# DanHelmy/hdr-realtime-video-pipeline

Hardware: AMD Instinct MI355X
Metric: frames/sec (HDRTVNet++ AGCM+LE+HG fp16 3840x2160 + fused RGB48 post into the pinned host ring); p50 per-frame ms in p50_ms (higher is better)
Workload: dtype f16

## Files before the change

hdr-realtime-video-pipeline_amd/csrc/api.h:

```cpp
#pragma once
#include "../../include/hdrtv_mi355x.h"

#include <algorithm>
#include <array>
#include <cfloat>
#include <chrono>
#include <cmath>
#include <condition_variable>
#include <cstdarg>
#include <cstdio>
#include <cstdlib>
#include <cstring>
#include <map>
#include <mutex>
#include <string>
#include <vector>

#include "launchers.h"

namespace hdrtv_host {

struct PackEntry {
    int dtype;
    int ndim;
// ... 119 lines not shown
    bool asym = true;
    float inv() const { return 1.f / scale; }
    float zoff() const { return asym ? -zero / scale : 128.f; }
    double soff() const { return asym ? 128.0 * (double)scale + (double)zero : 0.0; }
};
struct QLayer {
    size_t wpk8 = 0, scale = 0, shift = 0;
    ActQf q;
    int cin = 0, cout = 0, coutPad = 0, ks = 0, stride = 1;
};
struct QLastLayer { size_t wq = 0, ss = 0; ActQf q; bool on = false; };
struct SftLayer {
    size_t wfrag = 0, bias = 0;
    bool q = false;
    size_t qfrag = 0, qconst = 0;
    float inv[2] = {0, 0}, zoff[2] = {0, 0}, hzoff[2] = {0, 0};
    ActQf fq[4];
};

struct Tensor {
    size_t off = 0;
    int C = 0, H = 0, W = 0, layout = 0;
    size_t bytes() const
    {
        const size_t n = (size_t)C * H * W;
        return layout == 2 || layout == 3 ? n * 4 : (layout == 4 || layout == 5 ? n : n * 2);
    }
};

struct F32Layer {
    size_t w = 0, b = 0, bn_s = 0, bn_t = 0;
    int cin = 0, cout = 0, cot = 32, ks = 1;
    bool bn = false;
};

struct RingSlot {
    uint16_t *host = nullptr, *dev = nullptr;
    hipEvent_t ev = nullptr;
    int state = 0;
    bool landed = false;
};

}

struct hdrtv_ctx {
    int device = 0;
    int n_cu = 256, dev_ncu = 256;
    bool has_hg = false;
    bool fp32 = false;
    std::map<std::string, hdrtv_host::F32Layer> conv32f;
    std::string err;
    mutable std::mutex err_mu;
    hdrtv_host::Arena wts;
    std::map<std::string, hdrtv_host::ConvLayer> conv;
    std::map<std::string, hdrtv_host::C3Layer> c3;
    std::map<std::string, hdrtv_host::ConvI8Layer> conv8;
    float mask_r = 0.75f;
    int cond_mode = 0;
    bool hg_i8 = false;
    float hg_q0_inv = 0.f, hg_q0_zero = 0.f;
    std::map<std::string, hdrtv_host::SftLayer> sft;
    bool hr_i8 = false;
    std::map<std::string, hdrtv_host::QLayer> q32, q8;
    hdrtv_host::QLastLayer q_trunk6, q_tail2;
    bool trunk_q8 = false, tail_q8 = false, agcm_q8 = false;
    size_t tq_frag = 0, tq_const = 0, tl_frag = 0, tl_const = 0, ag_frag = 0, ag_P = 0, ag_Q = 0;
    hdrtv_host::ActQf tq_q[6], tl_q[2], ag_q[3];
    FakeQ cls_q[6] = {}, lin_q[6] = {};
    std::map<std::string, size_t> f32v;
    size_t zeros_off = 0;
    size_t dump_off = 0;
    size_t trunk_wfrag = 0, trunk_bias = 0;
    size_t tail_wfrag = 0, tail_bias = 0;
    size_t hgf_wfrag = 0, hg_w10a = 0;
    int H = 0, W = 0;
    hdrtv_host::Arena ws;
    int lanes = 1;
    std::vector<unsigned char *> lane_ws;
    std::map<std::string, hdrtv_host::Tensor> t;
    int launches = 0;
    double macs = 0.0;
    bool prof_on = false;
    std::vector<hipEvent_t> prof_ev;
    struct ProfEntry { std::string layer, kernel; double macs, bytes; float ms; const int *cnt; int cnt_total; };
    bool taps_partial = false, taps_replayable = false;
    hipStream_t taps_stream = nullptr;
    std::vector<ProfEntry> prof;
    int lb_key[4] = {0, 0, 0, 0};
    LetterboxParams lb{};
    void *lb_dev = nullptr;
    size_t lb_cap = 0;
    float *pq_bnd = nullptr;
    std::map<std::array<int, 4>, int4 *> ps_tabs;
    double *mt_dev = nullptr;
    size_t mt_cap = 0;
    std::vector<hdrtv_host::RingSlot> ring;
    int ring_next = 0, ring_H = 0, ring_W = 0, ring_waiters = 0;
    std::mutex ring_mu;
    std::condition_variable ring_cv;
    std::map<std::string, int> var;
};

namespace hdrtv_host {

int fail(hdrtv_ctx *c, int code, const char *fmt, ...);
bool variant_allowed(const std::string &name, int value);
void variants_init(hdrtv_ctx *c);

#define HIPCHK(c, expr)                                                                         \
    do {                                                                                        \
        hipError_t e_ = (expr);                                                                 \
        if (e_ != hipSuccess) return hdrtv_host::fail(c, HDRTV_EHIP, "%s failed: %s", #expr, hipGetErrorString(e_)); \
    } while (0)

bool build_weights(hdrtv_ctx *c, const Pack &hr, const Pack *hg);
bool build_weights_f32(hdrtv_ctx *c, const Pack &hr, const Pack *hg);

struct Shapes {
    int H, W, h4, w4;
    int ch[6], cw[6];
    int H1, W1, H2, W2, H3, W3;
    int Hp, Wp;
};
Shapes shapes_for(int H, int W);
Tensor &ws_add(hdrtv_ctx *c, const std::string &name, int C, int H, int W, int layout);
int do_reserve(hdrtv_ctx *c, int H, int W);
void free_workspaces(hdrtv_ctx *c);
template <typename T>
T *wsp(hdrtv_ctx *c, unsigned char *base, const std::string &name)
{
    auto it = c->t.find(name);
    if (it == c->t.end()) { fprintf(stderr, "hdrtv: internal error, no workspace tensor %s\n", name.c_str()); abort(); }
    return reinterpret_cast<T *>(base + it->second.off);
}
template <typename T>
const T *wtp(hdrtv_ctx *c, size_t off) { return reinterpret_cast<const T *>(c->wts.dev + off); }

struct HgLayer {
    const char *name;
    int cout, cin, skip_cin;
    int ks, ps;
    int mode, act;
    int level;
    const char *in, *skip, *out;
    const char *bn;
    const char *consumer, *shares;
    int out_c() const { return ps ? ps : cout; }
    int out_level() const { return level + (mode == ST_POOL ? 1 : 0) - (ps ? 1 : 0); }
};
inline constexpr HgLayer hg_layers[] = {
    {"conv2", 128, 64, 0, 3, 0, ST_NHWC, ACT_RELU, 1, "p1", nullptr, "conv2", "conv2.1", "conv3_1.0", "conv9"},
    {"conv3_1", 256, 128, 0, 3, 0, ST_POOL, ACT_RELU, 1, "conv2", nullptr, "p3", "conv3_1.1", "conv3_2.0", nullptr},
    {"conv3_2", 256, 256, 0, 3, 0, ST_NHWC, ACT_RELU, 2, "p3", nullptr, "conv3_2", "conv3_2.1", "conv4_1.0", "conv8"},
    {"conv4_1", 512, 256, 0, 3, 0, ST_POOL, ACT_RELU, 2, "conv3_2", nullptr, "p4", "conv4_1.1", "conv4_2.0", nullptr},
    {"conv4_2", 512, 512, 0, 3, 0, ST_NHWC, ACT_RELU, 3, "p4", nullptr, "conv4_2", "conv4_2.1", "conv5_1.0", "conv7"},
    {"conv5_1", 512, 512, 0, 3, 0, ST_POOL, ACT_RELU, 3, "conv4_2", nullptr, "p5", "conv5_1.1", "conv5_2.0", nullptr},
    {"conv5_2", 512, 512, 0, 3, 0, ST_NHWC, ACT_RELU, 4, "p5", nullptr, "conv5_2", "conv5_2.1", "conv_code1.0", "conv6"},
    {"conv_code1", 512, 512, 0, 3, 0, ST_POOL, ACT_RELU, 4, "conv5_2", nullptr, "pc", "conv_code1.1", "conv_code2.0", nullptr},
    {"conv_code2", 512, 512, 0, 3, 0, ST_NHWC, ACT_RELU, 5, "pc", nullptr, "conv_code2", "conv_code2.1", "Up_conv1.0", nullptr},
    {"Up_conv1", 2048, 512, 0, 3, 512, ST_PS, ACT_RELU, 5, "conv_code2", nullptr, "up1", "", "conv6", nullptr},
    {"conv6", 512, 1024, 512, 1, 0, ST_NHWC, ACT_NONE, 4, "up1", "conv5_2", "conv6", "", "Up_conv2.0", nullptr},
    {"Up_conv2", 2048, 512, 0, 3, 512, ST_PS, ACT_RELU, 4, "conv6", nullptr, "up2", "", "conv7", nullptr},
    {"conv7", 256, 1024, 512, 1, 0, ST_NHWC, ACT_NONE, 3, "up2", "conv4_2", "conv7", "", "Up_conv3.0", nullptr},
    {"Up_conv3", 1024, 256, 0, 3, 256, ST_PS, ACT_RELU, 3, "conv7", nullptr, "up3", "", "conv8", nullptr},
    {"conv8", 128, 512, 256, 1, 0, ST_NHWC, ACT_NONE, 2, "up3", "conv3_2", "conv8", "", "Up_conv4.0", nullptr},
    {"Up_conv4", 512, 128, 0, 3, 128, ST_PS, ACT_RELU, 2, "conv8", nullptr, "up4", "", "conv9", nullptr},
    {"conv9", 64, 256, 128, 1, 0, ST_NHWC, ACT_NONE, 1, "up4", "conv2", "conv9", "", "Up_conv5.0", nullptr},
    {"Up_conv5", 256, 64, 0, 3, 64, ST_PS_DOT3, ACT_RELU, 1, "conv9", nullptr, nullptr, "", nullptr, nullptr},
};

struct Seq {
    hdrtv_ctx *c;
    hipStream_t s;
    unsigned char *ws;
    int rc = HDRTV_OK;
    const f16 *tail_w = nullptr;
    const float *tail_b = nullptr, *tail_s = nullptr;
    f16 *tail_out = nullptr;
    const int *need_list = nullptr;
    int need_th = 0, need_total = 0;
    bool ok() const { return rc == HDRTV_OK; }
    void mark()
    {
        if (!c->prof_on) return;
        const size_t i = c->prof.size();
        while (c->prof_ev.size() <= i) {
            hipEvent_t ev;
            if (hipEventCreate(&ev) != hipSuccess) { c->prof_on = false; return; }
            c->prof_ev.push_back(ev);
        }
        (void)hipEventRecord(c->prof_ev[i], s);
    }
    void chk(hipError_t e, const char *what, const char *kernel = "", double macs = 0.0, double bytes = 0.0, const int *cnt = nullptr, int cnt_total = 0)
    {
        ++c->launches;
        c->macs += macs;
        if (e != hipSuccess && rc == HDRTV_OK) rc = fail(c, HDRTV_EHIP, "launch %s failed: %s", what, hipGetErrorString(e));
        if (c->prof_on) {
            c->prof.push_back({what, kernel, macs, bytes, 0.f, cnt, cnt_total});
            mark();
        }
    }
    void conv(const std::string &key, const f16 *src0, int c0, const f16 *src1, int c1, int Hi, int Wi, int act, int mode, f16 *dst, int dstC, int Hd, int Wd, const f16 *res1 = nullptr, const f16 *res2 = nullptr, f16 *dst_full = nullptr, f16 *dst_planar = nullptr, const f16 *res_planar = nullptr, const float *dotw = nullptr, float *dst_dot = nullptr, int s0_stride = 0);
    void conv8(const std::string &key, const int8_t *src0, int c0, const int8_t *src1, int c1, int Hi, int Wi, int mode, void *dst, int dstC, int Hd, int Wd, const float *dotw = nullptr, float *dst_dot = nullptr);
    void convq8(const std::string &key, const void *src, bool src_i8, int src_stride, int Hi, int Wi, int act, void *dst, int dstC, const ActQf *oq);
    void c3(const std::string &key, const f16 *in, int H, int W, int act, f16 *out, f16 *out_pool, float pool_q_inv = 0.f, float pool_q_zero = 0.f, const f16 *w2frag = nullptr, float *part2 = nullptr);
    void conv32(const std::string &key, const f16 *src, const f16 *cond, const std::string &sft_key, int H, int W, int act, int mode, f16 *dst, int dstC, int Hd, int Wd, const f16 *res1 = nullptr, const f16 *res2 = nullptr, f16 *dst_planar = nullptr, const f16 *res_planar = nullptr, const f16 *c3_img = nullptr, const std::string &c3_key = "");
    template <typename T>
    T *wsp(const std::string &name) const { return hdrtv_host::wsp<T>(c, ws, name); }
    void *stamp_buf() const
    {
#ifdef HDRTV_STAMP
        static const int stamp_launch = [] { const char *e = getenv("HDRTV_STAMP_LAUNCH"); return e ? atoi(e) : -1; }();
        return (stamp_launch >= 0 && c->launches == stamp_launch) ? (void *)wsp<f16>("dbg.stamps") : nullptr;
#else
        return nullptr;
#endif
    }
    static int prw_rows(int prw_mode, int Ho, int Wo, int cout, int n_cu)
    {
        if (prw_mode != 1) return prw_mode == 0 ? 0 : (prw_mode == 3 ? 8 : 16);
        const long tx = (Wo + 15) / 16, n = n_cu;
        auto cost = [&](long tiles, double rel) { return (double)(((tiles + n - 1) / n) * n) / (double)tiles * rel; };
        const double c16 = cost(tx * ((Ho + 15) / 16) * (cout / 256), 1.0);
        const double c8 = cost(tx * ((Ho + 7) / 8) * (cout / 256), 1.09);
        const double cp = cost(tx * ((Ho + 15) / 16) * (cout / 128), 1.22);
        if (cp <= c16 && cp <= c8) return 0;
        return c8 < c16 ? 8 : 16;
    }
    static int prw_tile_rows(const hdrtv_ctx *c, int mode, int cout, int Ho, int Wo)
    {
        const int prw_mode = c->var.at("prw");
        if (prw_mode == 0) return 0;
        if (mode == ST_PS_DOT3) return cout == 256 ? 16 : 0;
        return (cout % 256) ? 0 : prw_rows(prw_mode, Ho, Wo, cout, c->n_cu);
    }
    static FqParam fqp(const ActQf &q) { return FqParam{q.inv(), q.zoff(), q.scale, q.asym ? q.zero : -128.f * q.scale}; }
    const ConvLayer *rows_conv(const std::string &key, FqParam &fq, bool &on) const
    {
        on = false;
        auto it = c->conv.find(key);
        if (it != c->conv.end()) return &it->second;
        if (!c->var.at("le_rows_fq")) return nullptr;
        it = c->conv.find(key + "#fq");
        if (it == c->conv.end()) return nullptr;
        auto iq = c->q32.find(key);
        const ActQf *q = iq != c->q32.end() ? &iq->second.q : nullptr;
        if (!q) { auto i8 = c->q8.find(key); if (i8 != c->q8.end()) q = &i8->second.q; }
        if (!q) return nullptr;
        fq = fqp(*q);
        on = true;
        return &it->second;
    }
    bool rows_sft(const SftLayer &S, FqParam (&fq)[4], bool &on) const
    {
        on = S.q;
        if (S.q && !c->var.at("le_rows_fq")) return false;
        for (int i = 0; i < 4; ++i) fq[i] = fqp(S.fq[i]);
        return true;
    }
    bool rows_on(int H, int W, bool even) const
    {
        if (!c->var.at("le_rows") || (even && ((H | W) & 1))) return false;
        const int nstrips = (W + 59) / 60, nseg = std::max(1, c->n_cu / nstrips);
        return W >= 60 && (H + nseg - 1) / nseg >= c->var.at("le_rows_min");
    }
    RowsConvI8 rows_i8(const QLayer &Q) const
    {
        return RowsConvI8{wtp<int8_t>(c, Q.wpk8), wtp<float>(c, Q.scale), wtp<float>(c, Q.shift), Q.q.inv(), Q.q.zoff()};
    }
    RowsSftI8 rows_i8(const SftLayer &S) const
    {
        return RowsSftI8{wtp<int8_t>(c, S.qfrag), wtp<float>(c, S.qconst), {S.inv[0], S.inv[1]}, {S.zoff[0], S.zoff[1]}, {S.hzoff[0], S.hzoff[1]}};
    }
    void resblock(const std::string &base, const f16 *x, const f16 *cond, int H, int W, f16 *tb, f16 *y, const f16 *extra = nullptr);
};

int run_agcm(hdrtv_ctx *c, Seq &q, const f16 *rgb, const f16 *cond, f16 *agcm_out);
int run_le(hdrtv_ctx *c, Seq &q, const f16 *img, f16 *out_planar);
int run_hg(hdrtv_ctx *c, Seq &q, const f16 *base, void *out, int out_f32, bool complete_taps = false);
size_t hg_need_plan(hdrtv_ctx *c, int Hp, int Wp, HgNeedParams &p);
int run_f32(hdrtv_ctx *c, Seq &q, bool plan, int H, int W, const float *rgb, const float *cond, float *out, float *agcm_out);
int f32_plan(hdrtv_ctx *c, int H, int W);

}
```

hdr-realtime-video-pipeline_amd/csrc/api_graph.hip:

```cpp
#include "api.h"

namespace hdrtv_host {

void Seq::conv(const std::string &key, const f16 *src0, int c0, const f16 *src1, int c1, int Hi, int Wi, int act, int mode, f16 *dst, int dstC, int Hd, int Wd, const f16 *res1, const f16 *res2, f16 *dst_full, f16 *dst_planar, const f16 *res_planar, const float *dotw, float *dst_dot, int s0_stride)
{
    if (!ok()) return;
    auto it = c->conv.find(key);
    if (it == c->conv.end()) { rc = fail(c, HDRTV_ESTATE, "no packed conv %s", key.c_str()); return; }
    const ConvLayer &L = it->second;
    ConvParams p;
    memset(&p, 0, sizeof p);
    p.src0 = src0; p.src1 = src1; p.c0 = c0; p.c1 = c1;
    p.s0_stride = s0_stride ? s0_stride : c0; p.s1_stride = c1;
    p.Hi = Hi; p.Wi = Wi;
    const int pad = L.ks / 2;
    p.Ho = (Hi + 2 * pad - L.ks) / L.stride + 1;
    p.Wo = (Wi + 2 * pad - L.ks) / L.stride + 1;
    p.wpk = wtp<f16>(c, L.wpk); p.scale = wtp<float>(c, L.scale); p.shift = wtp<float>(c, L.shift);
    p.CoutPad = L.coutPad; p.Cout = L.cout; p.act = act; p.mode = mode;
    p.dst = dst; p.dst_full = dst_full; p.dstC = dstC; p.Hd = Hd; p.Wd = Wd;
    p.res1 = res1; p.res2 = res2; p.dst_planar = dst_planar; p.res_planar = res_planar;
    p.dotw = dotw; p.dst_dot = dst_dot;
    if (c0 + c1 != L.cin) { rc = fail(c, HDRTV_ESTATE, "conv %s: channel mismatch", key.c_str()); return; }
    p.zeros = wtp<f16>(c, c->zeros_off);
    p.tail_w = tail_w; p.tail_b = tail_b; p.tail_s = tail_s; p.tail_out = tail_out;
    tail_w = nullptr; tail_b = nullptr; tail_s = nullptr; tail_out = nullptr;
    p.trash = const_cast<char *>(wtp<char>(c, c->dump_off));
    const int *const need = need_list;
    const int need_rows = need_th, need_cells = need_total;
    need_list = nullptr; need_th = 0; need_total = 0;
    const int nt_slow = c->var.at("pglds_nt_slow");
    p.nt_slow = nt_slow == 3 ? (mode == ST_PS) : (nt_slow == 2 ? (L.coutPad >= 512) : nt_slow);
    enum { T16, S2G, PRW, PGLDS, GLDS1, IGEMM } route = IGEMM;
    int prw_th = 0;
    const bool g64 = L.stride == 1 && L.cin_t == 64 && L.bn == 128 && !res1 && !res2 && !dst_full && mode != ST_PLANAR3;
    const bool no_t16 = c->var.at("no_t16") != 0;
    if (!no_t16 && L.ks == 3 && L.stride == 2 && L.cin == 32 && L.coutPad == 32 && !src1 && mode == ST_NHWC && !res1 && !res2)
        route = T16;
    else if (L.ks == 3 && L.stride == 2 && L.cin_t == 64 && L.bn == L.coutPad && (L.coutPad == 64 || L.coutPad == 192))
        route = S2G;
    else if (g64 && L.ks == 3 && L.cout == L.coutPad) {
        prw_th = prw_tile_rows(c, mode, L.coutPad, p.Ho, p.Wo);
        route = prw_th ? PRW : PGLDS;
    } else if (g64 && L.ks == 1 && mode == ST_NHWC && (c0 + c1) >= 128 && L.coutPad <= 512 && (act == ACT_RELU || act == ACT_NONE))
        route = GLDS1;
    if (p.tail_w && route != S2G) { rc = fail(c, HDRTV_ESTATE, "conv %s: a fused CondNet tail was requested but the layer does not run on conv3x3s2_preg", key.c_str()); return; }
    const char *epi = mode == ST_POOL ? "pool" : (mode == ST_PS ? "ps" : (mode == ST_PS_DOT3 ? "ps_dot3" : "nhwc"));
    char tag[64];
    hipError_t e;
    bool list_taken = false;
    switch (route) {
    case T16: snprintf(tag, sizeof tag, "conv_t16<32,3,2>"); e = conv_t16_launch(p, s, c->n_cu); break;
    case S2G:
        snprintf(tag, sizeof tag, p.tail_w ? "conv3x3s2_preg<%d>+tail" : "conv3x3s2_preg<%d>", L.coutPad);
        e = conv3x3s2_preg_launch(p, c->n_cu, s);
        break;
    case PRW:
        if (need && need_rows == prw_th) p.tile_list = need;
        snprintf(tag, sizeof tag, "%s<%s>", prw_th == 8 ? "conv_prw8" : "conv_prw", epi);
        e = conv_prw_launch(p, prw_th, c->n_cu, s, &list_taken);
        break;
    case PGLDS: snprintf(tag, sizeof tag, "conv_pglds<%s>", epi); e = conv_pglds_launch(p, c->n_cu, s); break;
    case GLDS1: snprintf(tag, sizeof tag, "conv_glds1"); e = conv_glds1_launch(p, s, c->n_cu, c->var.at("glds1_old") != 0); break;
    default:
        snprintf(tag, sizeof tag, "conv_igemm<%d,%d,%d,%d>", L.cin_t, L.bn, L.ks, L.stride);
        e = conv_igemm_launch(p, L.cin_t, L.bn, L.ks, L.stride, s);
    }
    double macs = (double)p.Ho * p.Wo * L.cin * L.ks * L.ks * L.cout;
    double bytes = 2.0 * Hi * Wi * L.cin + 2.0 * L.ks * L.ks * L.cin * L.coutPad;
    if (p.tail_w) {
        macs += (double)p.Ho * p.Wo * (p.tail_s ? 64 * 16 : 64 * 64 + 64 * 16);
        bytes -= 2.0 * p.Ho * p.Wo * (64 - 16);
    }
    const double outel = mode == ST_POOL ? (double)Hd * Wd * L.cout + (dst_full ? (double)p.Ho * p.Wo * L.cout : 0.0)
                                          : (mode == ST_PLANAR3 ? 3.0 * Hd * Wd
                                                                : (mode == ST_PS_DOT3 ? 8.0 * Hd * Wd : (double)p.Ho * p.Wo * L.cout));
    bytes += 2.0 * outel * (1 + (res1 ? 1 : 0) + (res2 ? 1 : 0) + (res_planar ? 1 : 0));
    chk(e, key.c_str(), tag, macs, bytes, list_taken ? p.tile_list : nullptr, need_cells);
}


void Seq::conv8(const std::string &key, const int8_t *src0, int c0, const int8_t *src1, int c1, int Hi, int Wi, int mode, void *dst, int dstC, int Hd, int Wd, const float *dotw, float *dst_dot)
{
    if (!ok()) return;
    auto it = c->conv8.find(key);
    if (it == c->conv8.end()) { rc = fail(c, HDRTV_ESTATE, "no packed int8 conv %s", key.c_str()); return; }
    const ConvI8Layer &L = it->second;
    if (c0 + c1 != L.cin) { rc = fail(c, HDRTV_ESTATE, "conv %s: channel mismatch", key.c_str()); return; }
    ConvI8Params p;
    memset(&p, 0, sizeof p);
    p.src0 = src0; p.src1 = src1; p.c0 = c0; p.c1 = c1; p.Hi = Hi; p.Wi = Wi; p.Ho = Hi; p.Wo = Wi;
    p.wpk = wtp<int8_t>(c, L.wpk); p.scale = wtp<float>(c, L.scale); p.shift = wtp<float>(c, L.shift);
    p.Cout = L.cout; p.mode = mode; p.out_f16 = L.out_f16; p.dst = dst; p.dstC = dstC; p.Hd = Hd; p.Wd = Wd;
    p.padline = wtp<int8_t>(c, L.padline);
    p.delta = L.has_delta ? wtp<float>(c, L.delta) : nullptr;
    p.delta_acc = L.has_delta ? wtp<int>(c, L.delta_acc) : nullptr;
    p.lo_clamp = L.lo_clamp;
    p.trash = const_cast<char *>(wtp<char>(c, c->dump_off));
    p.dotw = dotw; p.dst_dot = dst_dot;
    char tag[64];
    if (L.ks == 3) snprintf(tag, sizeof tag, "conv_pglds_i8<%s%s>", mode == ST_POOL ? "pool" : (mode == ST_PS ? "ps" : (mode == ST_PS_DOT3 ? "ps_dot3" : "nhwc")), c0 == 64 ? ",c64" : "");
    else snprintf(tag, sizeof tag, "conv1x1_i8%s", L.out_f16 ? "<f16>" : "");
    const double macs = (double)Hi * Wi * L.cin * L.ks * L.ks * L.cout_real;
    const double outel = mode == ST_POOL ? (double)Hd * Wd * L.cout_real : (double)Hi * Wi * L.cout_real;
    const double bytes = (double)Hi * Wi * L.cin + (double)L.ks * L.ks * L.cin * L.cout +
                         (mode == ST_PS_DOT3 ? 16.0 * Hd * Wd : outel * (L.out_f16 ? 2.0 : 1.0));
    const int prw_mode = c->var.at("prw");
    int prw_th = prw_mode != 0 && L.ks == 3 && c0 != 64 && (L.cout % 256) == 0 && mode != ST_PS_DOT3 && !L.out_f16
                     ? prw_rows(prw_mode, Hi, Wi, L.cout, c->n_cu) : 0;
    const int i8_mode = c->var.at("prw_i8");
    if (i8_mode == 0 || (i8_mode == 1 && prw_th != 8)) prw_th = 0;
    const bool prw = prw_th != 0;
    if (prw) snprintf(tag, sizeof tag, "conv_prw%s_i8<%s>", prw_th == 8 ? "8" : "", mode == ST_POOL ? "pool" : (mode == ST_PS ? "ps" : "nhwc"));
    chk(L.ks == 3 ? (prw ? conv_prw_i8_launch(p, prw_th, c->n_cu, s) : conv_pglds_i8_launch(p, c->n_cu, s)) : conv1x1_i8_launch(p, s),
        key.c_str(), tag, macs, bytes);
}


void Seq::convq8(const std::string &key, const void *src, bool src_i8, int src_stride, int Hi, int Wi, int act, void *dst, int dstC, const ActQf *oq)
{
    if (!ok()) return;
    auto it = c->q8.find(key);
    if (it == c->q8.end()) { rc = fail(c, HDRTV_ESTATE, "no packed W8A8 conv %s", key.c_str()); return; }
    const QLayer &L = it->second;
    ConvQ8Params p;
    memset(&p, 0, sizeof p);
    p.src = src; p.src_i8 = src_i8 ? 1 : 0; p.Cin = L.cin; p.src_stride = src_stride; p.Hi = Hi; p.Wi = Wi;
    p.ks = L.ks; p.stride = L.stride;
    const int pad = L.ks / 2;
    p.Ho = (Hi + 2 * pad - L.ks) / L.stride + 1; p.Wo = (Wi + 2 * pad - L.ks) / L.stride + 1;
    p.wpk8 = wtp<int8_t>(c, L.wpk8); p.scale = wtp<float>(c, L.scale); p.shift = wtp<float>(c, L.shift);
    p.CoutPad = L.coutPad; p.Cout = L.cout; p.act = act; p.q_inv = L.q.inv(); p.q_zoff = L.q.zoff();
    p.dst = dst; p.dst_i8 = oq ? 1 : 0; p.dstC = dstC;
    if (oq) { p.oq_inv = oq->inv(); p.oq_zoff = oq->zoff(); }
    char tag[64];
    snprintf(tag, sizeof tag, "conv_q8<%d,%d,%d>", L.cin, L.ks, L.stride);
    const double macs = (double)p.Ho * p.Wo * L.cin * L.ks * L.ks * L.cout;
    const double bytes = (double)Hi * Wi * L.cin * (src_i8 ? 1.0 : 2.0) + (double)L.ks * L.ks * L.cin * L.coutPad +
                         (double)p.Ho * p.Wo * L.cout * (oq ? 1.0 : 2.0);
    chk(conv_q8_launch(p, s, c->n_cu), key.c_str(), tag, macs, bytes);
}


void Seq::c3(const std::string &key, const f16 *in, int H, int W, int act, f16 *out, f16 *out_pool, float pool_q_inv, float pool_q_zero, const f16 *w2frag, float *part2)
{
    if (!ok()) return;
    const C3Layer &L = c->c3.at(key);
    chk(conv_c3_launch(in, H, W, wtp<f16>(c, L.wfrag), wtp<float>(c, L.scale), wtp<float>(c, L.shift), L.cout, act, out,
                       out_pool, c->n_cu, s, pool_q_inv, pool_q_zero, w2frag, part2), key.c_str(),
        part2 ? "conv_c3<64,dot3>" : (L.cout == 64 ? "conv_c3<64>" : "conv_c3<32>"), (double)H * W * (27 * L.cout + (part2 ? 192 : 0)),
        (double)H * W * (6.0 + (out ? 2.0 * L.cout : 0.0) + (out_pool ? (pool_q_inv > 0.f ? 0.25 : 0.5) * L.cout : 0.0) + (part2 ? 16.0 : 0.0)));
}


void Seq::conv32(const std::string &key, const f16 *src, const f16 *cond, const std::string &sft_key, int H, int W, int act, int mode, f16 *dst, int dstC, int Hd, int Wd, const f16 *res1, const f16 *res2, f16 *dst_planar, const f16 *res_planar, const f16 *c3_img, const std::string &c3_key)
{
    if (!ok()) return;
    auto it = c->conv.find(key);
    auto iq = c->q32.find(key);
    if (it == c->conv.end() && iq == c->q32.end()) { rc = fail(c, HDRTV_ESTATE, "no packed conv %s", key.c_str()); return; }
    const bool i8 = iq != c->q32.end();
    ConvLayer L;
    Conv32Params p;
    memset(&p, 0, sizeof p);
    if (i8) {
        const QLayer &Q = iq->second;
        L.cout = Q.cout; L.coutPad = Q.coutPad;
        p.wpk8 = wtp<int8_t>(c, Q.wpk8); p.scale = wtp<float>(c, Q.scale); p.shift = wtp<float>(c, Q.shift);
        p.q_inv = Q.q.inv(); p.q_zoff = Q.q.zoff();
    } else {
        L = it->second;
        p.wpk = wtp<f16>(c, L.wpk); p.scale = wtp<float>(c, L.scale); p.shift = wtp<float>(c, L.shift);
    }
    p.src = src; p.cond = cond; p.H = H; p.W = W;
    bool sq = false;
    if (cond) {
        const SftLayer &S = c->sft.at(sft_key);
        p.sft_wfrag = wtp<f16>(c, S.wfrag); p.sft_bias = wtp<float>(c, S.bias);
        if (S.q) {
            sq = true;
            p.sq_wfrag = wtp<int8_t>(c, S.qfrag); p.sq_const = wtp<float>(c, S.qconst);
            for (int b = 0; b < 2; ++b) { p.sq_inv[b] = S.inv[b]; p.sq_zoff[b] = S.zoff[b]; p.sq_hzoff[b] = S.hzoff[b]; }
        }
    }
    p.CoutPad = L.coutPad; p.Cout = L.cout; p.act = act; p.mode = mode;
    p.dst = dst; p.dstC = dstC; p.Hd = Hd; p.Wd = Wd; p.res1 = res1; p.res2 = res2;
    p.dst_planar = dst_planar; p.res_planar = res_planar; p.zeros = wtp<f16>(c, c->zeros_off);
    p.dump = reinterpret_cast<f16 *>(stamp_buf());
    const double npx = (double)H * W;
    const double macs = npx * 32 * 9 * L.cout + (cond ? npx * 2 * (16 * 16 + 16 * 32) : 0.0) + (c3_img ? npx * 27 * 32 : 0.0);
    const double outb = mode == ST_PLANAR3 ? 6.0 * npx : 2.0 * npx * L.cout;
    const double bytes = npx * ((c3_img ? 6 : 64) + (cond ? 32 : 0)) + outb * (1 + (res1 ? 1 : 0) + (res2 ? 1 : 0) + (res_planar ? 1 : 0)) +
                         (i8 ? 1.0 : 2.0) * 9 * 32 * L.coutPad;
    p.trash = const_cast<char *>(wtp<char>(c, c->dump_off));
    if (c3_img) {
        const C3Layer &L3 = c->c3.at(c3_key);
        p.c3_img = c3_img; p.c3_wfrag = wtp<f16>(c, L3.wfrag);
    }
    const bool old_sched = c->var.at("conv32_old") != 0;
    const bool one_barrier = L.coutPad == 32 && !old_sched;
    char tag[48];
    snprintf(tag, sizeof tag, "conv32%c<%d,%s%s%s>", one_barrier ? 's' : 'p', L.coutPad / 32, c3_img ? "c3+" : "", cond ? (sq ? "sft-i8" : "sft") : "plain", i8 ? ",i8" : "");
    if (c3_img && !one_barrier) { rc = fail(c, HDRTV_ESTATE, "conv_first fusion needs the one-barrier schedule"); return; }
    chk(one_barrier ? conv32s_launch(p, c->n_cu, s, c->var.at("conv32_nosplit") != 0) : conv32p_launch(p, c->n_cu, s, c->var.at("conv32_nw")), key.c_str(), tag, macs, bytes);
}


void Seq::resblock(const std::string &base, const f16 *x, const f16 *cond, int H, int W, f16 *tb, f16 *y, const f16 *extra)
{
    const bool rows = ok() && !extra && rows_on(H, W, false);
    if (rows && c->var.at("le_rows_i8")) {
        auto q1 = c->q32.find(base + ".conv1"), q2 = c->q32.find(base + ".conv2");
        const SftLayer &S1 = c->sft.at(base + ".sft1"), &S2 = c->sft.at(base + ".sft2");
        if (q1 != c->q32.end() && q2 != c->q32.end() && S1.q && S2.q && q1->second.coutPad == 32 && q2->second.coutPad == 32) {
            RowsRbI8Params p;
            memset(&p, 0, sizeof p);
            p.x = x; p.cond = cond; p.c1 = rows_i8(q1->second); p.c2 = rows_i8(q2->second); p.s1 = rows_i8(S1); p.s2 = rows_i8(S2);
            p.slope1 = act_slope(ACT_RELU);
            p.dst = y; p.trash = const_cast<char *>(wtp<char>(c, c->dump_off)); p.H = H; p.W = W;
            const double npx = (double)H * W;
            chk(le_rb_rows_i8_launch(p, c->n_cu, s), base.c_str(), "le_rb_rows<i8>",
                npx * (2.0 * 32 * 9 * 32 + 4.0 * (16 * 16 + 16 * 32)), npx * (64 + 32 + 64) + 2.0 * 9 * 32 * 32);
            return;
        }
    }
    if (rows) {
        RowsRbParams p;
        memset(&p, 0, sizeof p);
        bool q1, q2, qs1, qs2;
        const ConvLayer *L1 = rows_conv(base + ".conv1", p.fq_c1, q1), *L2 = rows_conv(base + ".conv2", p.fq_c2, q2);
        const SftLayer &S1 = c->sft.at(base + ".sft1"), &S2 = c->sft.at(base + ".sft2");
        if (L1 && L2 && rows_sft(S1, p.fq_s1, qs1) && rows_sft(S2, p.fq_s2, qs2)) {
            p.fq = (q1 ? 1 : 0) | (q2 ? 2 : 0) | (qs1 ? 4 : 0) | (qs2 ? 8 : 0);
            p.x = x; p.cond = cond; p.H = H; p.W = W; p.dst = y;
// ... 256 lines not shown
            q.conv32("LE.HR_conv1", f0a, cond1, "LE.SFT_layer1", H, W, ACT_RELU, ST_NHWC, fea0, 32, H, W);
        } else {
            const bool fuse = !c->var.at("no_c3fuse") && !c->var.at("conv32_old") && c->q32.find("LE.HR_conv1") == c->q32.end();
            if (fuse) {
                q.conv32("LE.HR_conv1", f0a, cond1, "LE.SFT_layer1", H, W, ACT_RELU, ST_NHWC, fea0, 32, H, W, nullptr, nullptr, nullptr, nullptr,
                         img, "le.conv_first");
            } else {
                q.c3("le.conv_first", img, H, W, ACT_RELU, f0a, nullptr);
                q.conv32("LE.HR_conv1", f0a, cond1, "LE.SFT_layer1", H, W, ACT_RELU, ST_NHWC, fea0, 32, H, W);
            }
        }
    }
    f16 *fea1a = q.wsp<f16>("le.fea1a"), *fea1 = q.wsp<f16>("le.fea1"), *l1b = q.wsp<f16>("le.l1b");
    auto down = [&](const char *key, const f16 *src, int Hi, int Wi, f16 *dst, int Ho, int Wo) {
        if (isq8(key)) q.convq8(key, src, false, 32, Hi, Wi, ACT_RELU, dst, 32, nullptr);
        else q.conv(key, src, 32, nullptr, 0, Hi, Wi, ACT_RELU, ST_NHWC, dst, 32, Ho, Wo);
    };
    if (!head_fused) down("LE.down_conv1", fea0, H, W, fea1a, s.H1, s.W1);
    q.resblock("LE.recon_trunk1.0", fea1a, cond2, s.H1, s.W1, l1b, fea1);
    f16 *fea2a = q.wsp<f16>("le.fea2a"), *fea2 = q.wsp<f16>("le.fea2"), *l2b = q.wsp<f16>("le.l2b");
    down("LE.down_conv2", fea1, s.H1, s.W1, fea2a, s.H2, s.W2);
    q.resblock("LE.recon_trunk2.0", fea2a, cond3, s.H2, s.W2, l2b, fea2);
    f16 *fea3 = q.wsp<f16>("le.fea3"), *l3b = q.wsp<f16>("le.l3b"), *t3x = q.wsp<f16>("le.t3x"), *t3y = q.wsp<f16>("le.t3y");
    down("LE.down_conv3", fea2, s.H2, s.W2, fea3, s.H3, s.W3);
    q.resblock("LE.recon_trunk3.0", fea3, cond4, s.H3, s.W3, l3b, t3x);
    q.resblock("LE.recon_trunk3.1", t3x, cond4, s.H3, s.W3, l3b, t3y);
    q.resblock("LE.recon_trunk3.2", t3y, cond4, s.H3, s.W3, l3b, t3x);
    q.resblock("LE.recon_trunk3.3", t3x, cond4, s.H3, s.W3, l3b, t3y, fea3);
    f16 *up1 = q.wsp<f16>("le.up1"), *t4 = q.wsp<f16>("le.t4");
    q.conv32("LE.up_conv1.0", t3y, nullptr, "", s.H3, s.W3, ACT_RELU, ST_PS, up1, 32, s.H2, s.W2, fea2);
    q.resblock("LE.recon_trunk4.0", up1, cond3, s.H2, s.W2, l2b, t4);
    f16 *up2 = q.wsp<f16>("le.up2"), *t5 = q.wsp<f16>("le.t5");
    q.conv32("LE.up_conv2.0", t4, nullptr, "", s.H2, s.W2, ACT_RELU, ST_PS, up2, 32, s.H1, s.W1, fea1);
    q.resblock("LE.recon_trunk5.0", up2, cond2, s.H1, s.W1, l1b, t5);
    if (q.ok() && rows && c->var.at("le_rows_i8")) {
        auto qu = c->q32.find("LE.up_conv3.0"), qh = c->q32.find("LE.HR_conv2"), ql = c->q32.find("LE.conv_last");
        const SftLayer &S2 = c->sft.at("LE.SFT_layer2");
        if (qu != c->q32.end() && qh != c->q32.end() && ql != c->q32.end() && S2.q && qu->second.coutPad == 128 &&
            qh->second.coutPad == 32 && ql->second.coutPad == 32) {
            RowsTailI8Params p;
            memset(&p, 0, sizeof p);
            p.u = t5; p.fea0 = fea0; p.cond = cond1; p.res_planar = img; p.dst_planar = out_planar; p.H = H; p.W = W;
            p.up = q.rows_i8(qu->second); p.hr = q.rows_i8(qh->second); p.last = q.rows_i8(ql->second); p.s = q.rows_i8(S2);
            p.slope_relu = act_slope(ACT_RELU);
            p.trash = const_cast<char *>(wtp<char>(c, c->dump_off));
            const double npx = (double)H * W;
            q.chk(le_tail_rows_i8_launch(p, c->n_cu, q.s), "LE.tail", "le_tail_rows<i8>",
                  npx * (32.0 * 9 * 128 / 4 + 2.0 * (16 * 16 + 16 * 32) + 32.0 * 9 * 32 + 32.0 * 9 * 3), npx * (16 + 64 + 32 + 6 + 6) + 9.0 * 32 * (128 + 32 + 32));
            return q.rc;
        }
    }
    if (q.ok() && rows) {
        RowsTailParams p;
        memset(&p, 0, sizeof p);
        bool qu, qh, ql, qs;
        const ConvLayer *Lu = q.rows_conv("LE.up_conv3.0", p.fq_u, qu), *Lh = q.rows_conv("LE.HR_conv2", p.fq_y, qh),
                        *Ll = q.rows_conv("LE.conv_last", p.fq_z, ql);
        const SftLayer &S2 = c->sft.at("LE.SFT_layer2");
        if (Lu && Lh && Ll && q.rows_sft(S2, p.fq_s, qs)) {
            p.fq = (qu ? 1 : 0) | (qh ? 2 : 0) | (ql ? 4 : 0) | (qs ? 8 : 0);
            p.u = t5; p.fea0 = fea0; p.cond = cond1; p.res_planar = img; p.dst_planar = out_planar; p.H = H; p.W = W;
            p.w_up = wtp<f16>(c, Lu->wpk); p.b_up = wtp<float>(c, Lu->shift);
            p.sft_wfrag = wtp<f16>(c, S2.wfrag); p.sft_bias = wtp<float>(c, S2.bias);
            p.w_hr = wtp<f16>(c, Lh->wpk); p.b_hr = wtp<float>(c, Lh->shift); p.w_last = wtp<f16>(c, Ll->wpk); p.b_last = wtp<float>(c, Ll->shift);
            p.trash = const_cast<char *>(wtp<char>(c, c->dump_off));
            p.dump = q.stamp_buf();
            const double npx = (double)H * W;
            q.chk(le_tail_rows_launch(p, c->n_cu, q.s), "LE.tail", p.fq ? "le_tail_rows<fq>" : "le_tail_rows",
                  npx * (32.0 * 9 * 128 / 4 + 2.0 * (16 * 16 + 16 * 32) + 32.0 * 9 * 32 + 32.0 * 9 * 3), npx * (16 + 64 + 32 + 6 + 6) + 2.0 * 9 * 32 * (128 + 32 + 32));
            return q.rc;
        }
    }
    q.conv32("LE.up_conv3.0", t5, nullptr, "", s.H1, s.W1, ACT_RELU, ST_PS, up3, 32, H, W, fea0);
    q.conv32("LE.HR_conv2", up3, cond1, "LE.SFT_layer2", H, W, ACT_RELU, ST_NHWC, f0b, 32, H, W);
    q.conv32("LE.conv_last", f0b, nullptr, "", H, W, ACT_NONE, ST_PLANAR3, nullptr, 0, H, W, nullptr, nullptr, out_planar, img);
    return q.rc;
}

size_t hg_need_plan(hdrtv_ctx *c, int Hp, int Wp, HgNeedParams &p)
{
    memset(&p, 0, sizeof p);
    p.Hp = Hp; p.Wp = Wp;
    constexpr int n_layers = (int)(sizeof hg_layers / sizeof hg_layers[0]);
    static_assert(n_layers <= HG_NEED_MAX_LAYERS && n_layers + 2 <= HG_NEED_MAX_TENSORS, "hg_need's tables are too small");
    constexpr int max_level = [] { int m = 0; for (const HgLayer &L : hg_layers) m = L.level > m ? L.level : m; return m; }();
    static_assert(max_level < HG_NEED_LEVELS, "hg_need's unit tables have too few levels");
    memcpy(p.lu, hg_need_unit_log2[c->var.at("hg_sparse") == 1 ? 1 : 2], sizeof p.lu);
    auto ncell = [&](int level) { return (((Hp >> level) + 15) / 16) * (((Wp >> level) + 15) / 16); };
    auto nwords = [&](int level) {
        size_t m = 0;
        for (const auto &tab : hg_need_unit_log2) {
            const int u = 1 << tab[level], rows = std::max(((Hp >> level) + u - 1) / u, ((Hp >> level) + 7) / 8);
            m = std::max(m, (size_t)rows * ((((Wp >> level) + u - 1) / u + 63) / 64));
        }
        return m;
    };
    const char *names[HG_NEED_MAX_TENSORS];
    int level[HG_NEED_MAX_TENSORS], nt = 0;
    auto tensor = [&](const char *name, int lev) {
        if (!name) name = "part";
        for (int i = 0; i < nt; ++i)
            if (!strcmp(names[i], name)) return i;
        names[nt] = name; level[nt] = lev;
        return nt++;
    };
    for (int i = 0; i < n_layers; ++i) {
        const HgLayer &L = hg_layers[i];
        HgNeedLayer &N = p.L[i];
        N.level = L.level; N.ks = L.ks;
        N.mode = L.mode == ST_POOL ? 1 : (L.ps ? 2 : 0);
        N.in = tensor(L.in, L.level);
        N.skip = L.skip ? tensor(L.skip, L.level) : -1;
        N.out = tensor(L.out, L.out_level());
        N.th = L.ks == 3 && Seq::prw_tile_rows(c, L.mode, L.cout, Hp >> L.level, Wp >> L.level) == 8 ? 8 : 16;
    }
    p.n_layers = n_layers;
    bool seen[HG_NEED_MAX_TENSORS] = {};
    for (int i = n_layers - 1; i >= 0; --i) {
        HgNeedLayer &N = p.L[i];
        N.in_first = !seen[N.in];
        seen[N.in] = true;
        if (N.skip >= 0) { N.skip_first = !seen[N.skip]; seen[N.skip] = true; }
    }
    size_t off = 0;
    auto take = [&](size_t bytes) { const size_t o = off; off = (off + bytes + 15) & ~(size_t)15; return (int)o; };
    p.flags_off = take((size_t)ncell(0));
    take((size_t)ncell(0));
    for (int t = 0; t < nt; ++t)
        if (strcmp(names[t], "part")) take((size_t)ncell(level[t]));
    for (int i = 0; i < n_layers; ++i) p.L[i].list_off = take(4 * (2 * (size_t)ncell(p.L[i].level) + 4));
    size_t scratch = 0;
    for (int t = 0; t < nt; ++t) {
        p.map_off[t] = take(8 * nwords(level[t]));
        scratch = std::max(scratch, nwords(level[t]));
        if (!strcmp(names[t], "part")) p.flags_map = t;
    }
    for (int i = 0; i < n_layers; ++i) {
        p.L[i].out_chained = i + 1 < n_layers ? p.L[i + 1].in == p.L[i].out : p.L[i].out == p.flags_map;
        p.L[i].in_chained = i > 0 && p.L[i - 1].out == p.L[i].in;
    }
    p.scratch_words = (int)scratch;
    p.kbits_off = take(8 * scratch);
    p.tbits_off = take(8 * scratch);
    return off;
}

int run_hg(hdrtv_ctx *c, Seq &q, const f16 *base, void *out, int out_f32, bool complete_taps)
{
    const Shapes s = shapes_for(c->H, c->W);
    const int Hp = s.Hp, Wp = s.Wp;
    f16 *img = q.wsp<f16>("hg.img");
    uint8_t *mask = q.wsp<uint8_t>("hg.mask");
    const bool sparse = !complete_taps && c->var.at("hg_sparse") != 0 && !c->hg_i8 && !c->var.at("final_recompute");
    HgNeedParams np;
    if (sparse) {
        hg_need_plan(c, Hp, Wp, np);
        np.base = q.wsp<unsigned char>("hg.need");
    }
    if (q.ws == c->lane_ws[0] && !complete_taps) {
        hipStreamCaptureStatus cap = hipStreamCaptureStatusNone;
        c->taps_partial = sparse;
        c->taps_replayable = sparse && hipStreamIsCapturing(q.s, &cap) == hipSuccess && cap != hipStreamCaptureStatusNone;
        c->taps_stream = q.s;
    }
    if (!complete_taps)
        q.chk(hg_prep_launch(base, s.H, s.W, Hp, Wp, img, mask, c->mask_r, 0.1f, q.s, sparse ? np.base + np.flags_off : nullptr), "hg_prep",
              "hg_prep", 0.0, 13.0 * Hp * Wp);
    if (sparse) q.chk(hg_need_launch(np, q.s), "hg_need", "hg_need", 0.0, 0.0);
    float *part = q.wsp<float>("hg.part");
    const bool light = !c->var.at("final_recompute");
    float *part2 = light ? q.wsp<float>("hg.part2") : nullptr;
    const f16 *w2frag = light ? wtp<f16>(c, c->hgf_wfrag) + 6 * 64 * 8 : nullptr;
    constexpr int n_layers = (int)(sizeof hg_layers / sizeof hg_layers[0]);
    const char *tn[3 * n_layers];
    void *tp[3 * n_layers];
    int nt = 0;
    auto tensor = [&](const char *name) -> void * {
        if (!name) return nullptr;
        for (int i = 0; i < nt; ++i)
            if (!strcmp(tn[i], name)) return tp[i];
        char key[32];
        snprintf(key, sizeof key, "%s%s", c->hg_i8 ? "hg8." : "hg.", name);
        tn[nt] = name;
        tp[nt] = q.wsp<void>(key);
        return tp[nt++];
    };
    q.c3("hg.conv1", img, Hp, Wp, ACT_RELU, nullptr, (f16 *)tensor(hg_layers[0].in), c->hg_q0_inv, c->hg_q0_zero, w2frag, part2);
    char key[32];
    for (const HgLayer &L : hg_layers) {
        snprintf(key, sizeof key, "hg.%s", L.name);
        if (sparse) {
            const HgNeedLayer &N = np.L[&L - hg_layers];
            q.need_list = reinterpret_cast<const int *>(np.base + N.list_off);
            q.need_th = N.th;
            q.need_total = (((Hp >> L.level) + N.th - 1) / N.th) * (((Wp >> L.level) + 15) / 16);
        }
        const int c1 = L.skip_cin, c0 = L.cin - c1, Hi = Hp >> L.level, Wi = Wp >> L.level;
        const int Ho = Hp >> L.out_level(), Wo = Wp >> L.out_level();
        const bool dot3 = L.mode == ST_PS_DOT3;
        const float *dotw = dot3 ? wtp<float>(c, c->hg_w10a) : nullptr;
        float *dst_dot = dot3 ? part : nullptr;
        if (c->hg_i8)
            q.conv8(key, (const int8_t *)tensor(L.in), c0, (const int8_t *)tensor(L.skip), c1, Hi, Wi, L.mode, tensor(L.out), L.out_c(), Ho, Wo, dotw, dst_dot);
        else
            q.conv(key, (const f16 *)tensor(L.in), c0, (const f16 *)tensor(L.skip), c1, Hi, Wi, L.act, L.mode, (f16 *)tensor(L.out), L.out_c(), Ho, Wo,
                   nullptr, nullptr, nullptr, nullptr, nullptr, dotw, dst_dot);
    }
    if (!q.ok() || complete_taps) return q.rc;
    const C3Layer &L1 = c->c3.at("hg.conv1");
    HgFinalFusedArgs fa;
    fa.img = img; fa.mask = mask; fa.part = part; fa.wfrag = wtp<f16>(c, c->hgf_wfrag);
    fa.scale = wtp<float>(c, L1.scale); fa.shift = wtp<float>(c, L1.shift);
    fa.b10 = wtp<float>(c, c->f32v.at("hg.b10"));
    fa.wl = wtp<float>(c, c->f32v.at("hg.wl")); fa.bl = wtp<float>(c, c->f32v.at("hg.bl"));
    fa.out = out; fa.out_f32 = out_f32; fa.H = s.H; fa.W = s.W; fa.Hp = Hp; fa.Wp = Wp;
    if (light)
        q.chk(hg_final_light_launch(fa, part2, q.s), "hg_final", "hg_final_light", (double)s.H * s.W * 6 * 3,
              (double)s.H * s.W * (6 + 1 + 32 + 3 * (out_f32 ? 4 : 2)));
#ifdef HDRTV_AB
    else
        q.chk(hg_final_fused_launch(fa, c->n_cu, q.s), "hg_final", "hg_final_fused", (double)Hp * Wp * (128 * 3 + 6 * 3),
              (double)s.H * s.W * (6 + 1 + 16 + 3 * (out_f32 ? 4 : 2)));
#endif
    return q.rc;
}

}
```

hdr-realtime-video-pipeline_amd/csrc/conv1x1_glds.hip:

```cpp
#include <cstdlib>

#include "launchers.h"

namespace {

constexpr int TH = 16, TW = 16, NPIX = TH * TW;
constexpr int CT = 64, PIXB = CT * 2;
constexpr int A_PIECES_PER_WAVE = 4, A_BYTES = 8 * A_PIECES_PER_WAVE * 1024;
constexpr int BN = 128;
constexpr int B_BYTES = BN * PIXB;
constexpr int B_PIECES_PER_WAVE = 2;
constexpr int SMEM = 3 * A_BYTES + 3 * B_BYTES;
constexpr int OUT_ROWB = BN * 2 + 16;
static_assert(NPIX * OUT_ROWB <= SMEM, "epilogue tile must fit");

__device__ __forceinline__ int swz64(int row) { return (row >> 1) & 7; }


#ifdef HDRTV_AB
__global__ __launch_bounds__(512) void conv_glds1_kernel(ConvParams p)
{
    extern __shared__ __attribute__((aligned(16))) char smem[];
    char *sA = smem;
    char *sB = smem + 3 * A_BYTES;
// ... 58 lines not shown
    for (int i = 0; i < 2; ++i)
#pragma unroll
        for (int j = 0; j < 2; ++j)
#pragma unroll
            for (int k = 0; k < 16; ++k) acc[i][j][k] = 0.f;

    issue_A(0, 0);
    issue_B(0, 0);
    if (nchunk > 1) {
        issue_A(1, 1);
        issue_B(1, 1);
        asm volatile("s_waitcnt vmcnt(6)" ::: "memory");
    } else {
        asm volatile("s_waitcnt vmcnt(0)" ::: "memory");
    }
    __builtin_amdgcn_s_barrier();
    int slot = 0;
#pragma unroll 1
    for (int cc = 0; cc < nchunk; ++cc) {
        const bool pf = cc + 2 < nchunk;
        const int s2 = slot == 0 ? 2 : slot - 1;
        if (pf) { issue_A(cc + 2, s2); issue_B(cc + 2, s2); }
        const char *a = sA + slot * A_BYTES;
        const char *b = sB + slot * B_BYTES;
#pragma unroll
        for (int ks = 0; ks < CT / 16; ++ks) {
            const int chunk = ks * 2 + lh;
            f16x8 wf[2], xf[2];
#pragma unroll
            for (int i = 0; i < 2; ++i)
                wf[i] = *reinterpret_cast<const f16x8 *>(b + wrow[i] * PIXB + ((chunk ^ swz64(wrow[i])) << 4));
#pragma unroll
            for (int j = 0; j < 2; ++j)
                xf[j] = *reinterpret_cast<const f16x8 *>(a + hp_base[j] * PIXB + ((chunk ^ swz64(hx_base[j])) << 4));
#pragma unroll
            for (int i = 0; i < 2; ++i)
#pragma unroll
                for (int j = 0; j < 2; ++j)
                    acc[i][j] = __builtin_amdgcn_mfma_f32_32x32x16_f16(wf[i], xf[j], acc[i][j], 0, 0, 0);
        }
        if (pf) asm volatile("s_waitcnt vmcnt(6)" ::: "memory");
        else asm volatile("s_waitcnt vmcnt(0)" ::: "memory");
        __builtin_amdgcn_s_barrier();
        slot = slot == 2 ? 0 : slot + 1;
    }

    const float aslope = act_slope(p.act);
    char *so = smem;
#pragma unroll
    for (int i = 0; i < 2; ++i) {
#pragma unroll
        for (int qd = 0; qd < 4; ++qd) {
            const int cl = (wc * 2 + i) * 32 + 8 * qd + 4 * lh;
            const float4 sc = *reinterpret_cast<const float4 *>(p.scale + n0 + cl);
            const float4 sh = *reinterpret_cast<const float4 *>(p.shift + n0 + cl);
#pragma unroll
            for (int j = 0; j < 2; ++j) {
                const int q = (wp * 2 + j) * 32 + l31;
                f16x4 o;
                o[0] = (f16)act_fast(acc[i][j][4 * qd + 0] * sc.x + sh.x, aslope);
                o[1] = (f16)act_fast(acc[i][j][4 * qd + 1] * sc.y + sh.y, aslope);
                o[2] = (f16)act_fast(acc[i][j][4 * qd + 2] * sc.z + sh.z, aslope);
                o[3] = (f16)act_fast(acc[i][j][4 * qd + 3] * sc.w + sh.w, aslope);
                *reinterpret_cast<f16x4 *>(so + q * OUT_ROWB + cl * 2) = o;
            }
        }
    }
    __syncthreads();
    constexpr int CPP = BN / 8;
    for (int e = tid; e < NPIX * CPP; e += 512) {
        const int q = e / CPP, c8 = e % CPP;
        const int oy = oy0 + q / TW, ox = ox0 + q % TW;
        const int ch = n0 + c8 * 8;
        if (oy < p.Ho && ox < p.Wo && ch < p.Cout)
            *reinterpret_cast<f16x8 *>(p.dst + ((size_t)oy * p.Wo + ox) * p.dstC + ch) =
                *reinterpret_cast<const f16x8 *>(so + q * OUT_ROWB + c8 * 16);
    }
}
#endif

constexpr int P_NST = 8;
constexpr int P_SP = 144;
constexpr int P_MAXC = 512;

__global__ __launch_bounds__(512) void conv_glds1p_kernel(ConvParams p)
{
    extern __shared__ __attribute__((aligned(16))) char smem[];
    char *sA = smem;
    char *sB = smem + 3 * A_BYTES;
    const int tid = threadIdx.x, lane = tid & 63;
    const int wave = __builtin_amdgcn_readfirstlane(tid >> 6);
    const int l31 = lane & 31, lh = lane >> 5;

    const int ntn = p.CoutPad / BN;
    const int total = p.tiles_x * p.tiles_y * ntn;
    int t_first, t_step, ntile;
    {
        const int G = gridDim.x, b = blockIdx.x, xcd = b & 7, slot = b >> 3;
        const int nslots = (G - xcd + 7) >> 3;
        const int q = total >> 3, r = total & 7;
        const int base = xcd < r ? xcd * (q + 1) : r * (q + 1) + (xcd - r) * q;
        const int len = q + (xcd < r ? 1 : 0);
        t_first = base + slot;
        t_step = nslots;
        ntile = slot < len ? (len - slot + nslots - 1) / nslots : 0;
    }
    if (ntile == 0) return;
    struct Tile { int n0, oy0, ox0; };
    auto decode = [&](int t) {
        Tile o;
        const int nt_i = t % ntn, sp = t / ntn;
        const int ty = sp / p.tiles_x, tx = sp - ty * p.tiles_x;
        o.n0 = nt_i * BN; o.oy0 = ty * TH; o.ox0 = tx * TW;
        return o;
    };
    const int nchunk = (p.c0 + p.c1) / CT, nchunk0 = p.c0 / CT;

    const int l_row = lane >> 3, l_slot = lane & 7;
    auto issue = [&](const Tile &T, int cc, int slot) {
        const f16 *src;
        int cs, coff;
        if (cc < nchunk0) { src = p.src0; cs = p.s0_stride; coff = cc * CT; }
        else { src = p.src1; cs = p.s1_stride; coff = (cc - nchunk0) * CT; }
        const dma_rsrc_t ra = dma_rsrc(src, (unsigned)p.Hi * (unsigned)p.Wi * (unsigned)cs * 2u);
#pragma unroll
        for (int it = 0; it < A_PIECES_PER_WAVE; ++it) {
            const int piece = wave + it * 8;
            const int hp = piece * 8 + l_row;
            const int hy = hp / TW, hx = hp - hy * TW;
            const int iy = T.oy0 + hy, ix = T.ox0 + hx;
            const bool ok = (iy < p.Hi) & (ix < p.Wi);
            const unsigned off = ((unsigned)(iy * p.Wi + ix) * (unsigned)cs + (unsigned)(coff + ((l_slot ^ swz64(hx)) << 3))) * 2u;
            dma16(ra, sA + slot * A_BYTES + piece * 1024, ok ? off : DMA_OOB);
        }
        const dma_rsrc_t rb = dma_rsrc(p.wpk, (unsigned)nchunk * (unsigned)p.CoutPad * (unsigned)(CT * 2));
        const unsigned so = (unsigned)(cc * p.CoutPad + T.n0) * (unsigned)(CT * 2);
#pragma unroll
        for (int k = 0; k < B_PIECES_PER_WAVE; ++k) {
            const int piece = wave * B_PIECES_PER_WAVE + k;
            const int n = piece * 8 + l_row;
            dma16(rb, sB + slot * B_BYTES + piece * 1024, (unsigned)(n * CT + ((l_slot ^ swz64(n)) << 3)) * 2u, so);
        }
    };

    const int wc = wave & 1, wp = wave >> 1;
    int hp_base[2], hx_base[2], wrow[2];
#pragma unroll
    for (int j = 0; j < 2; ++j) {
        const int q = (wp * 2 + j) * 32 + l31;
        hp_base[j] = q;
        hx_base[j] = q % TW;
        wrow[j] = (wc * 2 + j) * 32 + l31;
    }
    f32x16 acc[2][2];
#pragma unroll
    for (int i = 0; i < 2; ++i)
#pragma unroll
        for (int j = 0; j < 2; ++j)
#pragma unroll
            for (int k = 0; k < 16; ++k) acc[i][j][k] = 0.f;
    const float act_lb = p.act == ACT_RELU ? 0.f : -__builtin_inff();
    char *trash = reinterpret_cast<char *>(p.trash) + lane * 16;
    __shared__ __attribute__((aligned(16))) float s_ss[2 * P_MAXC];
    for (int e = tid; e < p.CoutPad; e += 512) { s_ss[e] = p.scale[e]; s_ss[P_MAXC + e] = p.shift[e]; }
    __syncthreads();

    Tile cur = decode(t_first), nxt = cur;
    issue(cur, 0, 0);
    issue(cur, 1, 1);
    asm volatile("s_waitcnt vmcnt(6)" ::: "memory");
    __builtin_amdgcn_s_barrier();
    int slot = 0;
    for (int k = 0; k < ntile; ++k) {
        const bool has_next = k + 1 < ntile;
        if (has_next) nxt = decode(t_first + (k + 1) * t_step);
#pragma unroll 1
        for (int cc = 0; cc < nchunk; ++cc) {
            const int s2 = slot == 0 ? 2 : slot - 1;
            bool pf = true;
            if (cc + 2 < nchunk) issue(cur, cc + 2, s2);
            else if (has_next) issue(nxt, cc + 2 - nchunk, s2);
            else pf = false;
            const char *a = sA + slot * A_BYTES;
            const char *b = sB + slot * B_BYTES;
#pragma unroll
            for (int ks = 0; ks < CT / 16; ++ks) {
                const int chunk = ks * 2 + lh;
                f16x8 wf[2], xf[2];
#pragma unroll
                for (int i = 0; i < 2; ++i)
                    wf[i] = *reinterpret_cast<const f16x8 *>(b + wrow[i] * PIXB + ((chunk ^ swz64(wrow[i])) << 4));
#pragma unroll
                for (int j = 0; j < 2; ++j)
                    xf[j] = *reinterpret_cast<const f16x8 *>(a + hp_base[j] * PIXB + ((chunk ^ swz64(hx_base[j])) << 4));
#pragma unroll
                for (int i = 0; i < 2; ++i)
#pragma unroll
                    for (int j = 0; j < 2; ++j)
                        acc[i][j] = __builtin_amdgcn_mfma_f32_32x32x16_f16(wf[i], xf[j], acc[i][j], 0, 0, 0);
            }
            if (!pf) asm volatile("s_waitcnt vmcnt(0)" ::: "memory");
            else if (cc == 0 && k > 0) asm volatile("s_waitcnt vmcnt(%0)" ::"n"(6 + P_NST) : "memory");
            else asm volatile("s_waitcnt vmcnt(6)" ::: "memory");
            __builtin_amdgcn_s_barrier();
            if (cc + 1 < nchunk) slot = slot == 2 ? 0 : slot + 1;
        }
        char *stg = wave < 6 ? sA + slot * A_BYTES + wave * (32 * P_SP) : sB + slot * B_BYTES + (wave - 6) * (32 * P_SP);
        const int s_row = lane >> 3, s_chunk = lane & 7;
        const int chb = cur.n0 + wc * 64 + s_chunk * 8;
#pragma unroll
        for (int j = 0; j < 2; ++j) {
#pragma unroll
            for (int i = 0; i < 2; ++i)
#pragma unroll
                for (int qd = 0; qd < 4; ++qd) {
                    const int cl = (wc * 2 + i) * 32 + 8 * qd + 4 * lh;
                    const float4 sc = *reinterpret_cast<const float4 *>(s_ss + cur.n0 + cl);
                    const float4 sh = *reinterpret_cast<const float4 *>(s_ss + P_MAXC + cur.n0 + cl);
                    f16x4 o;
                    o[0] = (f16)fmaxf(acc[i][j][4 * qd + 0] * sc.x + sh.x, act_lb);
                    o[1] = (f16)fmaxf(acc[i][j][4 * qd + 1] * sc.y + sh.y, act_lb);
                    o[2] = (f16)fmaxf(acc[i][j][4 * qd + 2] * sc.z + sh.z, act_lb);
                    o[3] = (f16)fmaxf(acc[i][j][4 * qd + 3] * sc.w + sh.w, act_lb);
                    *reinterpret_cast<f16x4 *>(stg + l31 * P_SP + (i * 32 + 8 * qd + 4 * lh) * 2) = o;
#pragma unroll
                    for (int r = 0; r < 4; ++r) acc[i][j][4 * qd + r] = 0.f;
                }
#pragma unroll
            for (int rr = 0; rr < 4; ++rr) {
                const int px = rr * 8 + s_row;
                const f16x8 v = *reinterpret_cast<const f16x8 *>(stg + px * P_SP + s_chunk * 16);
                const int oy = cur.oy0 + (wp * 2 + j) * 2 + (px >> 4), ox = cur.ox0 + (px & 15);
                const bool ok = oy < p.Ho && ox < p.Wo && chb < p.Cout;
                f16 *d = ok ? p.dst + ((size_t)oy * p.Wo + ox) * p.dstC + chb : reinterpret_cast<f16 *>(trash);
                *reinterpret_cast<f16x8 *>(d) = v;
            }
        }
        asm volatile("s_waitcnt lgkmcnt(0)" ::: "memory");
        __builtin_amdgcn_s_barrier();
        slot = slot == 2 ? 0 : slot + 1;
        cur = nxt;
    }
}

}

hipError_t conv_glds1_launch(ConvParams p, hipStream_t stream, int n_cu, bool old_form)
{
    if ((p.c0 % CT) || (p.c1 % CT) || p.c0 + p.c1 < CT || (p.CoutPad % BN) || p.res1 || p.res2 || p.dst_full ||
        p.mode != ST_NHWC || !p.zeros)
        return hipErrorInvalidValue;
#ifdef HDRTV_AB
    static DevOnce attr_once;
    if (attr_once.need()) {
        hipError_t e = hipFuncSetAttribute(reinterpret_cast<const void *>(conv_glds1_kernel),
                                           hipFuncAttributeMaxDynamicSharedMemorySize, SMEM);
        if (e != hipSuccess) return e;
        attr_once.done();
    }
#endif
    p.tiles_x = (p.Wo + TW - 1) / TW;
    p.tiles_y = (p.Ho + TH - 1) / TH;
    const int grid = p.tiles_x * p.tiles_y * (p.CoutPad / BN);
    const int nchunk = (p.c0 + p.c1) / CT;
    if (!old_form && n_cu >= 8 && nchunk >= 2 && p.trash && p.CoutPad <= P_MAXC && (p.act == ACT_RELU || p.act == ACT_NONE)) {
        static DevOnce attr_p;
        if (attr_p.need()) {
            hipError_t e = hipFuncSetAttribute(reinterpret_cast<const void *>(conv_glds1p_kernel),
                                               hipFuncAttributeMaxDynamicSharedMemorySize, SMEM);
            if (e != hipSuccess) return e;
            attr_p.done();
        }
        hipLaunchKernelGGL(conv_glds1p_kernel, dim3(grid < n_cu ? grid : n_cu), dim3(512), SMEM, stream, p);
        return hipGetLastError();
    }
#ifdef HDRTV_AB
    hipLaunchKernelGGL(conv_glds1_kernel, dim3(grid), dim3(512), SMEM, stream, p);
    return hipGetLastError();
#else
    return hipErrorNotSupported;
#endif
}
```

hdr-realtime-video-pipeline_amd/csrc/conv3x3_pglds.hip:

```cpp
#include "launchers.h"

namespace {

constexpr int TH = 16, TW = 16, HW = 18, NPIX = HW * HW;
constexpr int CT = 64, PIXB = CT * 2;
constexpr int BN = 128;
constexpr int A_PIECES_PER_WAVE = 6, A_BYTES = 8 * A_PIECES_PER_WAVE * 1024;
constexpr int B_BYTES = BN * PIXB, B_PIECES_PER_WAVE = 2;
constexpr int SS_OFF = 2 * A_BYTES + 3 * B_BYTES;
constexpr int DOTW_OFF = SS_OFF + 2048;
constexpr int SMEM = DOTW_OFF + 1024;

template <int MODE> struct NStores { static constexpr int N = MODE == ST_POOL ? 2 : (MODE == ST_PS_DOT3 ? 1 : 8); };

typedef __amdgpu_buffer_rsrc_t rsrc_t;
__device__ __forceinline__ rsrc_t make_rsrc(const void *base, unsigned bytes)
{
    return __builtin_amdgcn_make_buffer_rsrc(const_cast<void *>(base), (short)0, (int)bytes, 0x00020000);
}
__device__ __forceinline__ void bdma16(rsrc_t r, void *lds, unsigned voff, unsigned soff)
{
    __builtin_amdgcn_raw_ptr_buffer_load_lds(r, (__attribute__((address_space(3))) void *)lds, 16, voff, soff, 0, 0);
}
constexpr unsigned OOB = 0x80000000u;

template <int N> __device__ __forceinline__ void wait_vm()
{
    asm volatile("s_waitcnt vmcnt(%0)" ::"n"(N) : "memory");
}
template <int N> __device__ __forceinline__ void wait_tap()
{
    asm volatile("s_waitcnt vmcnt(%0) lgkmcnt(0)" ::"n"(N) : "memory");
}

struct Tile { int n0, oy0, ox0; };

template <int MODE>
__global__ __launch_bounds__(512) void conv_pglds_kernel(ConvParams p)
{
    extern __shared__ __attribute__((aligned(16))) char smem[];
    char *sA = smem;
    char *sB = smem + 2 * A_BYTES;

    const int tid = threadIdx.x, lane = tid & 63;
    const int wave = __builtin_amdgcn_readfirstlane(tid >> 6);
    const int l15 = lane & 15, kg = lane >> 4;

    const int ntn = p.CoutPad / BN;
    const int total = p.tiles_x * p.tiles_y * ntn;
    int t_first, t_step, ntile;
    {
        const int G = gridDim.x, b = blockIdx.x, xcd = b & 7, slot = b >> 3;
        const int nslots = (G - xcd + 7) >> 3;
        const int q = total >> 3, r = total & 7;
        const int base = xcd < r ? xcd * (q + 1) : r * (q + 1) + (xcd - r) * q;
        const int len = q + (xcd < r ? 1 : 0);
        t_first = base + slot;
        t_step = nslots;
        ntile = slot < len ? (len - slot + nslots - 1) / nslots : 0;
    }
    if (ntile == 0) return;
    auto decode = [&](int t) {
        Tile o;
        const int nsp = p.tiles_x * p.tiles_y;
        const int nt_i = p.nt_slow ? t / nsp : t % ntn, sp = p.nt_slow ? t - nt_i * nsp : t / ntn;
        const int ty = sp / p.tiles_x, tx = sp - ty * p.tiles_x;
        o.n0 = nt_i * BN; o.oy0 = ty * TH; o.ox0 = tx * TW;
        return o;
    };

    const int nchunk = (p.c0 + p.c1) / CT, nchunk0 = p.c0 / CT;
    const int nit = nchunk * 9;

    const int l_row = lane >> 3, l_slot = lane & 7;
    auto issue_A = [&](int cc, int buf, const Tile &T) {
        const f16 *src;
        int cs, coff;
        if (cc < nchunk0) { src = p.src0; cs = p.s0_stride; coff = cc * CT; }
        else { src = p.src1; cs = p.s1_stride; coff = (cc - nchunk0) * CT; }
        const rsrc_t rs = make_rsrc(src, (unsigned)p.Hi * (unsigned)p.Wi * (unsigned)cs * 2u);
#pragma unroll
        for (int it = 0; it < A_PIECES_PER_WAVE; ++it) {
            const int piece = wave + it * 8;
            const int hp = piece * 8 + l_row;
            const int hy = hp / HW, hx = hp - hy * HW;
            const int iy = T.oy0 - 1 + hy, ix = T.ox0 - 1 + hx;
            const bool ok = (hp < NPIX) & ((unsigned)iy < (unsigned)p.Hi) & ((unsigned)ix < (unsigned)p.Wi);
            const unsigned off = ((unsigned)(iy * p.Wi + ix) * (unsigned)cs + (unsigned)(coff + ((l_slot ^ (hx & 7)) << 3))) * 2u;
            bdma16(rs, sA + buf * A_BYTES + piece * 1024, ok ? off : OOB, 0);
        }
    };
    auto issue_B = [&](int it_i, int n0, int slot) {
        const int cc = it_i / 9, tap = it_i - cc * 9;
        const rsrc_t rs = make_rsrc(p.wpk, 9u * (unsigned)nchunk * (unsigned)p.CoutPad * (unsigned)PIXB);
        const unsigned so = (unsigned)((tap * nchunk + cc) * p.CoutPad + n0) * (unsigned)PIXB;
#pragma unroll
        for (int k = 0; k < B_PIECES_PER_WAVE; ++k) {
            const int piece = wave * B_PIECES_PER_WAVE + k;
            const int n = piece * 8 + l_row;
            bdma16(rs, sB + slot * B_BYTES + piece * 1024, (unsigned)(n * CT + ((l_slot ^ (n & 7)) << 3)) * 2u, so);
        }
    };
    auto issue_SS = [&](int n0, int slot) {
        const char *sc = reinterpret_cast<const char *>(p.scale), *sh = reinterpret_cast<const char *>(p.shift);
        const char *lo = sc < sh ? sc : sh;
        const rsrc_t rs = make_rsrc(lo, 0xffffffffu);
        bdma16(rs, smem + SS_OFF + slot * 1024, (unsigned)((lane < 32 ? sc : sh) - lo) + (unsigned)(lane & 31) * 16u, (unsigned)n0 * 4u);
    };

    if constexpr (MODE == ST_PS_DOT3) {
        if (tid < 24) {
            const int kgq = tid & 3, o = (tid >> 2) % 3, half = tid / 12;
            f16x8 hi, lo;
#pragma unroll
            for (int e = 0; e < 8; ++e) {
                const float w = p.dotw[o * 64 + half * 32 + (e < 4 ? 4 * kgq + e : 16 + 4 * kgq + e - 4)];
                hi[e] = (f16)w;
                lo[e] = (f16)((w - (float)hi[e]) * 1024.f);
            }
            *reinterpret_cast<f16x8 *>(smem + DOTW_OFF + tid * 32) = hi;
            *reinterpret_cast<f16x8 *>(smem + DOTW_OFF + tid * 32 + 16) = lo;
        }
        __syncthreads();
    }

    const int wc = wave & 1, wp = wave >> 1;
    f32x4 acc[4][4];
#pragma unroll
    for (int i = 0; i < 4; ++i)
#pragma unroll
        for (int j = 0; j < 4; ++j) acc[i][j] = f32x4{0.f, 0.f, 0.f, 0.f};
    const float act_lb = p.act == ACT_RELU ? 0.f : -__builtin_inff();
    const int kw = l15 & 7;
    const int b_lane = (wc * 64 + l15) * PIXB;
    const int a_lane = (wp * 4 * HW + l15) * PIXB;

    Tile cur = decode(t_first), nxt = cur;
    issue_A(0, 0, cur);
    issue_SS(cur.n0, 0);
    issue_B(0, cur.n0, 0);
    issue_B(1, cur.n0, 1);
    issue_B(2, cur.n0, 2);
    wait_vm<4>();
    __builtin_amdgcn_s_barrier();

    int gch = 0;
    for (int k = 0; k < ntile; ++k) {
        const bool has_next = k + 1 < ntile;
        if (has_next) nxt = decode(t_first + (k + 1) * t_step);
        for (int cc = 0; cc < nchunk; ++cc, ++gch) {
            const char *a = sA + (gch & 1) * A_BYTES;
            const bool last_chunk = cc + 1 == nchunk;
            const bool pfA = !last_chunk || has_next;
#pragma unroll
            for (int tap = 0; tap < 9; ++tap) {
                const int it_i = cc * 9 + tap;
                bool pfB = true;
                if (tap == 0 && cc == 0) {}
                else if (it_i + 2 < nit) issue_B(it_i + 2, cur.n0, (tap + 2) % 3);
                else if (has_next) issue_B(it_i + 2 - nit, nxt.n0, (tap + 2) % 3);
                else pfB = false;
                if (tap == 6 && pfA) {
                    if (!last_chunk) issue_A(cc + 1, (gch + 1) & 1, cur);
                    else { issue_A(0, (gch + 1) & 1, nxt); issue_SS(nxt.n0, (k + 1) & 1); }
                }

                const char *bw = sB + (tap % 3) * B_BYTES + b_lane;
                const char *ax = a + a_lane + ((tap / 3) * HW + tap % 3) * PIXB;
                const int kx = (l15 + tap % 3) & 7;
                f16x8 wf[2][4], xf[2][4];
                auto ldw = [&](int ks, int i) {
                    wf[ks][i] = *reinterpret_cast<const f16x8 *>(bw + i * 16 * PIXB + (((ks * 4 + kg) ^ kw) << 4));
                };
                auto ldx = [&](int ks, int j) {
                    xf[ks][j] = *reinterpret_cast<const f16x8 *>(ax + j * HW * PIXB + (((ks * 4 + kg) ^ kx) << 4));
                };
#pragma unroll
                for (int i = 0; i < 4; ++i) { ldw(0, i); ldx(0, i); }
                __builtin_amdgcn_sched_barrier(0);
#pragma unroll
                for (int g = 0; g < 8; ++g) {
                    acc[g >> 2][g & 3] = __builtin_amdgcn_mfma_f32_16x16x32_f16(wf[0][g >> 2], xf[0][g & 3], acc[g >> 2][g & 3], 0, 0, 0);
                    __builtin_amdgcn_sched_barrier(0);
                    if (g == 0) ldw(1, 0); else if (g < 5) ldx(1, g - 1); else ldw(1, g - 4);
                    __builtin_amdgcn_sched_barrier(0);
                }
#pragma unroll
                for (int m = 8; m < 16; ++m)
                    acc[m >> 2][m & 3] = __builtin_amdgcn_mfma_f32_16x16x32_f16(wf[0][m >> 2], xf[0][m & 3], acc[m >> 2][m & 3], 0, 0, 0);
                __builtin_amdgcn_sched_barrier(0);
#pragma unroll
                for (int m = 0; m < 16; ++m)
                    acc[m >> 2][m & 3] = __builtin_amdgcn_mfma_f32_16x16x32_f16(wf[1][m >> 2], xf[1][m & 3], acc[m >> 2][m & 3], 0, 0, 0);

                if (!pfB) {
                    wait_tap<0>();
                } else if ((tap == 6 || tap == 7) && pfA) {
                    if (last_chunk) wait_tap<9>();
                    else wait_tap<8>();
                } else if (tap <= 1 && cc == 0 && k > 0) {
                    wait_tap<NStores<MODE>::N + 2>();
                } else {
                    wait_tap<2>();
                }
                __builtin_amdgcn_s_barrier();
            }
        }

        if (has_next) issue_B(2, nxt.n0, 2);
        const float *ss = reinterpret_cast<const float *>(smem + SS_OFF + (k & 1) * 1024);
        char *trash = reinterpret_cast<char *>(p.trash) + lane * 16;
        const int cw = wc * 64 + 4 * kg;
        f16x4 o[4][4];
#pragma unroll
        for (int i = 0; i < 4; ++i) {
            const float4 sc = *reinterpret_cast<const float4 *>(ss + cw + i * 16);
            const float4 sh = *reinterpret_cast<const float4 *>(ss + 128 + cw + i * 16);
#pragma unroll
            for (int j = 0; j < 4; ++j) {
                o[i][j][0] = (f16)fmaxf(acc[i][j][0] * sc.x + sh.x, act_lb);
                o[i][j][1] = (f16)fmaxf(acc[i][j][1] * sc.y + sh.y, act_lb);
                o[i][j][2] = (f16)fmaxf(acc[i][j][2] * sc.z + sh.z, act_lb);
                o[i][j][3] = (f16)fmaxf(acc[i][j][3] * sc.w + sh.w, act_lb);
                acc[i][j] = f32x4{0.f, 0.f, 0.f, 0.f};
            }
        }
        const int ox = cur.ox0 + l15;
        constexpr int SP = 144;
        char *stg = sA + ((gch - 1) & 1) * A_BYTES + wave * (32 * SP);
        const int s_row = lane >> 3, s_chunk = lane & 7;
        if constexpr (MODE == ST_NHWC || MODE == ST_PS) {
            const int cps = p.dstC;
// ... 15 lines not shown
                    f16 *d;
                    if constexpr (MODE == ST_NHWC) {
                        const bool ok = oy < p.Ho && oxx < p.Wo;
                        d = ok ? p.dst + ((size_t)oy * p.Wo + oxx) * p.dstC + cbase : reinterpret_cast<f16 *>(trash);
                    } else {
                        const int Y = 2 * oy + (sub >> 1), X = 2 * oxx + (sub & 1);
                        const bool ok = oy < p.Ho && oxx < p.Wo && Y < p.Hd && X < p.Wd;
                        d = ok ? p.dst + ((size_t)Y * p.Wd + X) * cps + cbase : reinterpret_cast<f16 *>(trash);
                    }
                    *reinterpret_cast<f16x8 *>(d) = v;
                }
            }
        } else if constexpr (MODE == ST_POOL) {
#pragma unroll
            for (int jj = 0; jj < 2; ++jj)
#pragma unroll
                for (int i = 0; i < 4; ++i) {
                    f16x4 m;
#pragma unroll
                    for (int r = 0; r < 4; ++r) m[r] = o[i][2 * jj][r] > o[i][2 * jj + 1][r] ? o[i][2 * jj][r] : o[i][2 * jj + 1][r];
                    *reinterpret_cast<f16x4 *>(stg + (jj * 16 + l15) * SP + (i * 16 + 4 * kg) * 2) = m;
                }
#pragma unroll
            for (int jj = 0; jj < 2; ++jj) {
                f16x8 v = *reinterpret_cast<const f16x8 *>(stg + (jj * 16 + 2 * s_row) * SP + s_chunk * 16);
                const f16x8 v1 = *reinterpret_cast<const f16x8 *>(stg + (jj * 16 + 2 * s_row + 1) * SP + s_chunk * 16);
#pragma unroll
                for (int r = 0; r < 8; ++r) v[r] = v[r] > v1[r] ? v[r] : v1[r];
                const int py = (cur.oy0 >> 1) + wp * 2 + jj, px = (cur.ox0 >> 1) + s_row;
                const bool ok = py < p.Hd && px < p.Wd;
                f16 *d = ok ? p.dst + ((size_t)py * p.Wd + px) * p.dstC + cur.n0 + wc * 64 + s_chunk * 8 : reinterpret_cast<f16 *>(trash);
                *reinterpret_cast<f16x8 *>(d) = v;
            }
        } else {
            const int orow = l15 & 3, qrow = l15 >> 2;
            const f16x8 zero8 = {(f16)0.f, (f16)0.f, (f16)0.f, (f16)0.f, (f16)0.f, (f16)0.f, (f16)0.f, (f16)0.f};
            float4 r = make_float4(0.f, 0.f, 0.f, 0.f);
#pragma unroll
            for (int half = 0; half < 2; ++half) {
                const char *tb = smem + DOTW_OFF + (((half * 3 + (orow < 3 ? orow : 0)) * 4 + kg) << 5);
                f16x8 fh = *reinterpret_cast<const f16x8 *>(tb), fl = *reinterpret_cast<const f16x8 *>(tb + 16);
                if (orow == 3) { fh = zero8; fl = zero8; }
                f32x4 ah = {0.f, 0.f, 0.f, 0.f}, al = {0.f, 0.f, 0.f, 0.f};
#pragma unroll
                for (int jj = 0; jj < 4; ++jj) {
                    const f16x4 o0 = o[2 * half][jj], o1 = o[2 * half + 1][jj];
                    const f16x8 bq = {o0[0], o0[1], o0[2], o0[3], o1[0], o1[1], o1[2], o1[3]};
                    const bool mine = qrow == jj;
                    ah = __builtin_amdgcn_mfma_f32_16x16x32_f16(mine ? fh : zero8, bq, ah, 0, 0, 0);
                    al = __builtin_amdgcn_mfma_f32_16x16x32_f16(mine ? fl : zero8, bq, al, 0, 0, 0);
                }
                constexpr float k = 1.f / 1024.f;
                const float4 v = make_float4(ah[0] + al[0] * k, ah[1] + al[1] * k, ah[2] + al[2] * k, 0.f);
                if (half == 0) r = v;
                else { r.x += v.x; r.y += v.y; r.z += v.z; }
            }
            const int sub = cur.n0 / 64 + wc;
            const int oy = cur.oy0 + wp * 4 + kg;
            const int Y = 2 * oy + (sub >> 1), X = 2 * ox + (sub & 1);
            const bool ok = oy < p.Ho && ox < p.Wo && Y < p.Hd && X < p.Wd;
            float4 *d = ok ? reinterpret_cast<float4 *>(p.dst_dot + ((size_t)Y * p.Wd + X) * 4) : reinterpret_cast<float4 *>(trash);
            *d = make_float4(r.x, r.y, r.z, 0.f);
        }
        cur = nxt;
    }
}

template <int MODE>
hipError_t launch_mode(const ConvParams &p, int grid, hipStream_t stream)
{
    static DevOnce attr_once;
    auto kern = conv_pglds_kernel<MODE>;
    if (attr_once.need()) {
        hipError_t e = hipFuncSetAttribute(reinterpret_cast<const void *>(kern), hipFuncAttributeMaxDynamicSharedMemorySize, SMEM);
        if (e != hipSuccess) return e;
        attr_once.done();
    }
    hipLaunchKernelGGL(kern, dim3(grid), dim3(512), SMEM, stream, p);
    return hipGetLastError();
}

}

hipError_t conv_pglds_launch(ConvParams p, int n_cu, hipStream_t stream)
{
    if ((p.c0 % CT) || (p.c1 % CT) || p.c0 + p.c1 < CT || (p.CoutPad % BN) || p.Cout != p.CoutPad || p.res1 || p.res2 ||
        p.dst_full || !p.zeros || !p.trash || n_cu < 8 || (p.act != ACT_RELU && p.act != ACT_NONE) ||
        (p.mode != ST_NHWC && p.mode != ST_PS && p.mode != ST_POOL && p.mode != ST_PS_DOT3) ||
        (p.mode == ST_PS && (p.dstC % 64)) || (p.mode == ST_PS_DOT3 && (p.dstC != 64 || !p.dotw || !p.dst_dot)))
        return hipErrorInvalidValue;
    p.tiles_x = (p.Wo + TW - 1) / TW;
    p.tiles_y = (p.Ho + TH - 1) / TH;
    const int total = p.tiles_x * p.tiles_y * (p.CoutPad / BN);
    const int grid = total < n_cu ? total : n_cu;
    switch (p.mode) {
    case ST_NHWC: return launch_mode<ST_NHWC>(p, grid, stream);
    case ST_PS: return launch_mode<ST_PS>(p, grid, stream);
    case ST_POOL: return launch_mode<ST_POOL>(p, grid, stream);
    default: return launch_mode<ST_PS_DOT3>(p, grid, stream);
    }
}
```

hdr-realtime-video-pipeline_amd/csrc/hdrtv_api.hip:

```cpp
#include "api.h"
#include "yuv420.h"

using namespace hdrtv_host;
extern "C" {

static int launched(hdrtv_ctx *c, const char *what, hipError_t e)
{
    return e == hipSuccess ? HDRTV_OK : fail(c, HDRTV_EHIP, "%s: %s", what, hipGetErrorString(e));
}

#ifndef HDRTV_BUILD_ID
#define HDRTV_BUILD_ID "unstamped"
#endif
const char *hdrtv_version(void) { return "hdrtv_mi355x 0.1 gfx950 (MFMA f16 implicit-GEMM, hand-written HIP) build " HDRTV_BUILD_ID; }

int hdrtv_create(const void *hr_pack, size_t hr_bytes, const void *hg_pack, size_t hg_bytes, int device_id, hdrtv_ctx **out)
{
    return hdrtv_create_ex(hr_pack, hr_bytes, hg_pack, hg_bytes, device_id, HDRTV_PREC_F16, out);
}

int hdrtv_create_ex(const void *hr_pack, size_t hr_bytes, const void *hg_pack, size_t hg_bytes, int device_id, int precision,
                    hdrtv_ctx **out)
{
    if (!out) return HDRTV_EINVAL;
// ... 637 lines not shown
    {
        std::unique_lock<std::mutex> lk(c->ring_mu);
        if (slot < 0 || slot >= (int)c->ring.size()) return fail(c, HDRTV_EINVAL, "bad ring slot");
        if (c->ring[slot].state == 0) return fail(c, HDRTV_ESTATE, "ring slot %d is already free", slot);
        if (c->ring[slot].state == 2 && !c->ring[slot].landed) {
            const hipEvent_t ev = c->ring[slot].ev;
            if (int rc = ring_sync_slot(c, slot, lk, "release")) return rc;
            if (slot >= (int)c->ring.size() || c->ring[slot].ev != ev) return fail(c, HDRTV_ESTATE, "ring destroyed during release");
        }
        c->ring[slot].state = 0;
        c->ring[slot].landed = false;
    }
    c->ring_cv.notify_all();
    return HDRTV_OK;
}

int hdrtv_ring_destroy(hdrtv_ctx *c)
{
    if (!c) return HDRTV_OK;
    std::unique_lock<std::mutex> lk(c->ring_mu);
    c->ring_cv.wait(lk, [&] { return c->ring_waiters == 0; });
    for (auto &sl : c->ring) {
        if (sl.ev) (void)hipEventDestroy(sl.ev);
        if (sl.host) (void)hipHostFree(sl.host);
        if (sl.dev) (void)hipFree(sl.dev);
    }
    c->ring.clear();
    lk.unlock();
    c->ring_cv.notify_all();
    return HDRTV_OK;
}

int hdrtv_get_tap(hdrtv_ctx *c, const char *name, void **dev_ptr, int *C, int *H, int *W, int *layout)
{
    if (!c || !name) return HDRTV_EINVAL;
    auto it = c->t.find(name);
    if (it == c->t.end() || c->lane_ws.empty()) return fail(c, HDRTV_EINVAL, "no tap named %s", name);
    if (c->taps_partial && !strncmp(name, "hg.", 3) && strcmp(name, "hg.img") && strcmp(name, "hg.mask") && strcmp(name, "hg.need")) {
        HIPCHK(c, hipSetDevice(c->device));
        const int launches = c->launches;
        const double macs = c->macs;
        const bool prof_on = c->prof_on;
        c->prof_on = false;
        Seq q{c, c->taps_stream, c->lane_ws[0]};
        const int rc = run_hg(c, q, nullptr, nullptr, 0, true);
        c->launches = launches; c->macs = macs; c->prof_on = prof_on;
        c->taps_partial = c->taps_replayable;
        if (rc != HDRTV_OK) return rc;
    }
    if (dev_ptr) *dev_ptr = c->lane_ws[0] + it->second.off;
    if (C) *C = it->second.C;
    if (H) *H = it->second.H;
    if (W) *W = it->second.W;
    if (layout) *layout = it->second.layout;
    return HDRTV_OK;
}

int hdrtv_infer_stats(hdrtv_ctx *c, int *launches, double *macs)
{
    if (!c) return HDRTV_EINVAL;
    if (launches) *launches = c->launches;
    if (macs) *macs = c->macs;
    return HDRTV_OK;
}

int hdrtv_profile_enable(hdrtv_ctx *c, int on)
{
    if (!c) return HDRTV_EINVAL;
    c->prof_on = on != 0;
    c->prof.clear();
    return HDRTV_OK;
}

int hdrtv_profile_get(hdrtv_ctx *c, int i, const char **layer, const char **kernel, float *ms, double *macs, double *bytes)
{
    if (!c) return HDRTV_EINVAL;
    const int n = (int)c->prof.size();
    if (i < 0) return n;
    if (i >= n || (size_t)i + 1 >= c->prof_ev.size()) return fail(c, HDRTV_EINVAL, "profile index out of range");
    hdrtv_ctx::ProfEntry &e = c->prof[i];
    HIPCHK(c, hipEventSynchronize(c->prof_ev[i + 1]));
    HIPCHK(c, hipEventElapsedTime(&e.ms, c->prof_ev[i], c->prof_ev[i + 1]));
    double done = 1.0;
    if (e.cnt && e.cnt_total > 0) {
        int n = 0;
        HIPCHK(c, hipMemcpy(&n, e.cnt, sizeof n, hipMemcpyDeviceToHost));
        done = (double)n / (double)e.cnt_total;
    }
    if (layer) *layer = e.layer.c_str();
    if (kernel) *kernel = e.kernel.c_str();
    if (ms) *ms = e.ms;
    if (macs) *macs = e.macs * done;
    if (bytes) *bytes = e.bytes * done;
    return HDRTV_OK;
}

const char *hdrtv_last_error(const hdrtv_ctx *c)
{
    if (!c) return "null context";
    static thread_local std::string copy;
    std::lock_guard<std::mutex> lk(c->err_mu);
    copy = c->err;
    return copy.c_str();
}

}
```

hdr-realtime-video-pipeline_amd/csrc/hg_need.hip:

```cpp
#include "launchers.h"

namespace {

constexpr int NT = 1024, LDS_WORDS = 2304;
using u64 = unsigned long long;

__constant__ u64 k_tile_bits[5] = {~0ull, 0x5555555555555555ull, 0x1111111111111111ull, 0x0101010101010101ull, 0x0001000100010001ull};

struct Map {
    int h, w, nw;
};
__device__ __forceinline__ Map map_of(const HgNeedParams &p, int level)
{
    const int lu = p.lu[level], r = (1 << lu) - 1;
    Map m;
    m.h = ((p.Hp >> level) + r) >> lu;
    m.w = ((p.Wp >> level) + r) >> lu;
    m.nw = (m.w + 63) >> 6;
    return m;
}
__device__ __forceinline__ u64 word(const u64 *b, const Map &m, int y, int wi)
{
    return (unsigned)y < (unsigned)m.h && (unsigned)wi < (unsigned)m.nw ? b[y * m.nw + wi] : 0;
}
__device__ __forceinline__ u64 row_mask(int w, int wi)
{
    const int n = w - 64 * wi;
    return n >= 64 ? ~0ull : (n <= 0 ? 0ull : (1ull << n) - 1);
}
__device__ __forceinline__ u64 spread2(unsigned v)
{
    u64 x = v;
    x = (x | x << 16) & 0x0000FFFF0000FFFFull;
    x = (x | x << 8) & 0x00FF00FF00FF00FFull;
    x = (x | x << 4) & 0x0F0F0F0F0F0F0F0Full;
    x = (x | x << 2) & 0x3333333333333333ull;
    x = (x | x << 1) & 0x5555555555555555ull;
    return x | x << 1;
}
__device__ __forceinline__ unsigned pairs_any(u64 v)
{
    u64 x = (v | v >> 1) & 0x5555555555555555ull;
    x = (x | x >> 1) & 0x3333333333333333ull;
    x = (x | x >> 2) & 0x0F0F0F0F0F0F0F0Full;
    x = (x | x >> 4) & 0x00FF00FF00FF00FFull;
    x = (x | x >> 8) & 0x0000FFFF0000FFFFull;
    x = (x | x >> 16) & 0x00000000FFFFFFFFull;
    return (unsigned)x;
}

__global__ __launch_bounds__(NT) void hg_need_kernel(HgNeedParams p)
{
    __shared__ u64 s_k[LDS_WORDS], s_t[LDS_WORDS], s_n[LDS_WORDS];
    __shared__ int s_wave[NT / 64];
    const int tid = threadIdx.x;
    {
        const Map m = map_of(p, 0);
        const HgNeedLayer &L = p.L[p.n_layers - 1];
        u64 *fb = L.out_chained && m.h * m.nw <= LDS_WORDS ? s_n : reinterpret_cast<u64 *>(p.base + p.map_off[p.flags_map]);
        unsigned char *fl = p.base + p.flags_off;
        constexpr int NW = NT / 64, B = 8;
        const int lane = tid & 63, n0 = m.h * m.nw;
        for (int i0 = tid >> 6; i0 < n0; i0 += B * NW) {
            int at[B];
            unsigned char c[B];
#pragma unroll
            for (int j = 0; j < B; ++j) {
                const int i = i0 + j * NW, y = i / m.nw, x = 64 * (i - y * m.nw) + lane;
                at[j] = i < n0 && x < m.w ? y * m.w + x : -1;
                c[j] = at[j] >= 0 ? fl[at[j]] : 0;
            }
#pragma unroll
            for (int j = 0; j < B; ++j) {
                const u64 v = __ballot(c[j] != 0);
                if (at[j] >= 0) fl[at[j]] = 0;
                if (lane == 0 && i0 + j * NW < n0) fb[i0 + j * NW] = v;
            }
        }
    }
    __syncthreads();
    for (int li = p.n_layers - 1; li >= 0; --li) {
        const HgNeedLayer L = p.L[li];
        const int olev = L.level + (L.mode == 1 ? 1 : 0) - (L.mode == 2 ? 1 : 0);
        const Map mk = map_of(p, L.level), mo = map_of(p, olev);
        const int lu = p.lu[L.level], nk = mk.h * mk.nw;
        const int sh = p.lu[olev] - lu + olev - L.level;
        const int lth = L.th == 8 ? 3 : 4, lbw = 4 - lu;
        const int ty_n = ((p.Hp >> L.level) + L.th - 1) >> lth, tx_n = ((p.Wp >> L.level) + 15) >> 4, nt = ty_n * mk.nw;
        const bool lds = max(nk, nt) <= LDS_WORDS;
        u64 *km = lds ? s_k : reinterpret_cast<u64 *>(p.base + p.kbits_off);
        u64 *tm = lds ? s_t : reinterpret_cast<u64 *>(p.base + p.tbits_off);
        const u64 *om = L.out_chained && mo.h * mo.nw <= LDS_WORDS ? s_n : reinterpret_cast<const u64 *>(p.base + p.map_off[L.out]);
        for (int i = tid; i < nk; i += NT) {
            const int y = i / mk.nw, wi = i - y * mk.nw;
            u64 k;
            if (sh == 0) {
                k = word(om, mo, y, wi);
            } else if (sh > 0) {
                k = spread2((unsigned)(word(om, mo, y >> 1, wi >> 1) >> (32 * (wi & 1))));
            } else {
                k = 0;
                for (int dy = 0; dy < 2; ++dy)
                    k |= (u64)pairs_any(word(om, mo, 2 * y + dy, 2 * wi)) | (u64)pairs_any(word(om, mo, 2 * y + dy, 2 * wi + 1)) << 32;
            }
            km[i] = k & row_mask(mk.w, wi);
        }
        __syncthreads();
        u64 *ig = reinterpret_cast<u64 *>(p.base + p.map_off[L.in]), *im = L.in_chained && nk <= LDS_WORDS ? s_n : ig;
        u64 *sm = L.skip >= 0 ? reinterpret_cast<u64 *>(p.base + p.map_off[L.skip]) : nullptr;
        for (int i = tid; i < nk; i += NT) {
            const int y = i / mk.nw, wi = i - y * mk.nw;
            u64 v = km[i];
            if (L.ks == 3) {
                for (int dy = -1; dy <= 1; ++dy) {
                    const u64 c = word(km, mk, y + dy, wi);
                    v |= c | c << 1 | c >> 1 | word(km, mk, y + dy, wi - 1) >> 63 | word(km, mk, y + dy, wi + 1) << 63;
                }
                v &= row_mask(mk.w, wi);
            }
            im[i] = L.in_first ? v : (ig[i] | v);
            if (sm) sm[i] = L.skip_first ? v : (sm[i] | v);
        }
        const int r_sh = lth - lu;
        for (int i = tid; i < nt; i += NT) {
            const int ty = i / mk.nw, wi = i - ty * mk.nw;
            const int r0 = r_sh >= 0 ? ty << r_sh : ty >> -r_sh, nr = r_sh >= 0 ? 1 << r_sh : 1;
            u64 v = 0;
            for (int r = r0; r < min(r0 + nr, mk.h); ++r) v |= km[r * mk.nw + wi];
            for (int s = 1; s < (1 << lbw); s <<= 1) v |= v >> s;
            tm[i] = v & k_tile_bits[lbw];
        }
        __syncthreads();
        const int per = (nt + NT - 1) / NT, c0 = tid * per, c1 = min(nt, c0 + per);
        int cnt = 0;
        for (int i = c0; i < c1; ++i) cnt += __popcll(tm[i]);
        int incl = cnt;
        for (int d = 1; d < 64; d <<= 1) {
            const int v = __shfl_up(incl, d, 64);
            if ((tid & 63) >= d) incl += v;
        }
        if ((tid & 63) == 63) s_wave[tid >> 6] = incl;
        __syncthreads();
        int o = incl - cnt, total = 0;
        for (int w = 0; w < NT / 64; ++w) {
            const int v = s_wave[w];
            if (w < (tid >> 6)) o += v;
            total += v;
        }
        int *lst = reinterpret_cast<int *>(p.base + L.list_off);
        if (tid == 0) lst[0] = total;
        for (int i = c0; i < c1; ++i) {
            const int ty = i / mk.nw, wi = i - ty * mk.nw;
            for (u64 v = tm[i]; v; v &= v - 1) lst[1 + o++] = ty * tx_n + ((64 * wi + __ffsll(v) - 1) >> lbw);
        }
    }
}

}

hipError_t hg_need_launch(const HgNeedParams &p, hipStream_t s)
{
    if (!p.base || p.n_layers < 1 || p.n_layers > HG_NEED_MAX_LAYERS) return hipErrorInvalidValue;
    for (int i = 0; i < p.n_layers; ++i) {
        const HgNeedLayer &L = p.L[i];
        const int olev = L.level + (L.mode == 1 ? 1 : 0) - (L.mode == 2 ? 1 : 0);
        if (L.level < 0 || L.level >= HG_NEED_LEVELS || olev < 0 || olev >= HG_NEED_LEVELS) return hipErrorInvalidValue;
        const int sh = p.lu[olev] - p.lu[L.level] + olev - L.level;
        if (p.lu[L.level] < 0 || p.lu[L.level] > 4 || sh < -1 || sh > 1 || (L.th != 8 && L.th != 16)) return hipErrorInvalidValue;
    }
    if (p.lu[0] != 4) return hipErrorInvalidValue;
    hipLaunchKernelGGL(hg_need_kernel, dim3(1), dim3(NT), 0, s, p);
    return hipGetLastError();
}
```

hdr-realtime-video-pipeline_amd/csrc/launchers.h:

```cpp
#pragma once
#include "common.h"

struct DevOnce {
    unsigned char set[64] = {};
    static int cur() { int d = 0; return hipGetDevice(&d) == hipSuccess && d >= 0 && d < 64 ? d : 0; }
    bool need() const { return !set[cur()]; }
    void done() { set[cur()] = 1; }
};

hipError_t conv_igemm_launch(ConvParams p, int cin_t, int bn, int ks, int stride, hipStream_t stream);
hipError_t conv_glds1_launch(ConvParams p, hipStream_t stream, int n_cu = 0, bool old_form = false);
hipError_t conv_pglds_launch(ConvParams p, int n_cu, hipStream_t stream);
hipError_t conv_prw_launch(ConvParams p, int th, int n_cu, hipStream_t stream, bool *list_taken = nullptr);
hipError_t conv_pglds_i8_launch(ConvI8Params p, int n_cu, hipStream_t stream);
hipError_t conv_prw_i8_launch(ConvI8Params p, int th, int n_cu, hipStream_t stream);
hipError_t conv1x1_i8_launch(ConvI8Params p, hipStream_t stream);
hipError_t conv32p_launch(Conv32Params p, int n_cu, hipStream_t stream, int nw = 0);
hipError_t conv32s_launch(Conv32Params p, int n_cu, hipStream_t stream, bool nosplit = false);
hipError_t le_rb_rows_launch(RowsRbParams p, int n_cu, hipStream_t stream);
hipError_t le_rb_rows_i8_launch(RowsRbI8Params p, int n_cu, hipStream_t stream);
hipError_t le_tail_rows_i8_launch(RowsTailI8Params p, int n_cu, hipStream_t stream);
hipError_t le_head_rows_i8_launch(RowsHeadI8Params p, int n_cu, hipStream_t stream);
hipError_t le_tail_rows_launch(RowsTailParams p, int n_cu, hipStream_t stream);
hipError_t le_head_rows_launch(RowsHeadParams p, int n_cu, hipStream_t stream);
hipError_t conv_t16_launch(ConvParams p, hipStream_t stream, int n_cu);
hipError_t conv_q8_launch(ConvQ8Params p, hipStream_t stream, int n_cu);
hipError_t conv_q8_multi_launch(ConvQ8MultiParams p, int n_cu, hipStream_t stream);
hipError_t conv3x3s2_preg_launch(ConvParams p, int n_cu, hipStream_t stream);

hipError_t pre_unpack_launch(const uint8_t *bgr, f16 *out, int H, int W, hipStream_t s);
hipError_t cond_resize_launch(const f16 *in, f16 *out, int H, int W, int Ho, int Wo, const float *wx, const int *xmn,
                              const int *xns, const float *wy, const int *ymn, const int *yns, hipStream_t s);
hipError_t pre_fused_launch(const uint8_t *bgr, f16 *out, f16 *cond, int H, int W, int Ho, int Wo, const float *wx, const int *xmn,
                            const int *xns, const float *wy, const int *ymn, const int *yns, int mode, hipStream_t s);
hipError_t post_u8_launch(const void *in, int is_f32, int H, int W, uint8_t *bgr, hipStream_t s);
hipError_t post_rgb48_launch(const void *in, int is_f32, int H, int W, uint16_t *rgb, int pq, float peak, hipStream_t s,
                             const float *pq_bnd = nullptr);

struct FakeQ { int on; float inv, zoff, scale, zero; };
hipError_t cls_block_launch(const void *in, int in_f16, int Ci, int Hi, int Wi, const float *nmean, const float *nrstd,
                            const float *ngamma, const float *nbeta, const float *Wt, const float *bias, int Co, float *out,
                            int Ho, int Wo, float *part, hipStream_t s, const FakeQ *qin = nullptr, const FakeQ *qstat = nullptr,
                            int *nblk = nullptr);
hipError_t cls_stats_launch(const float *part, int C, int nblk, int n, float eps, float *mean, float *rstd, hipStream_t s);
struct AgcmFoldArgs {
    const float *mean5;
    const float *w20, *b20;
    const float *ws[3], *bs[3], *wt[3], *bt[3];
    const float *w1, *b1, *w2, *b2, *w3, *b3;
};
hipError_t agcm_fold_launch(const AgcmFoldArgs &a, f16 *frags, float *biasbuf, hipStream_t s);
hipError_t agcm_mlp_launch(const f16 *in, f16 *out, size_t npix, const f16 *frags, const float *biasbuf, hipStream_t s);

hipError_t conv_c3_launch(const f16 *in, int H, int W, const f16 *wfrag, const float *scale, const float *shift, int cout,
                          int act, f16 *out, f16 *out_pool, int n_cu, hipStream_t s, float pool_q_inv = 0.f, float pool_q_zero = 0.f,
                          const f16 *w2frag = nullptr, float *part2 = nullptr);
hipError_t conv_c3_q8_launch(const f16 *in, int H, int W, const int8_t *wq, const float *scale, const float *shift, float q_inv,
                             float q_zoff, int act, f16 *out, int n_cu, hipStream_t s);
struct QLastArgs {
    const int8_t *wq;
    const float *ss;
    float q_inv, q_zoff;
};
hipError_t le_cond_trunk_launch(const f16 *img, int H, int W, const f16 *wfrag, const float *bias, f16 *cond, f16 *cond1,
                                int n_cu, hipStream_t s, const QLastArgs *q6 = nullptr);
hipError_t cond_tail_launch(const f16 *x, int x_stride, size_t npx, const f16 *wfrag, const float *bias, f16 *out, int n_cu,
                            hipStream_t s, const QLastArgs *q2 = nullptr);
struct TrunkQ8Args {
    const int8_t *wfrag;
    const float *consts;
    float q1_inv, q1_zoff, q4_inv;
    float zoff[5];
};
hipError_t le_cond_trunk_q8_launch(const f16 *img, int H, int W, const TrunkQ8Args &a, f16 *cond, f16 *cond1, int n_cu, hipStream_t s);
hipError_t cond_tail_q8_launch(const int8_t *x, size_t npx, const int8_t *wfrag, const float *consts, float zoff2, f16 *out, int n_cu,
                               hipStream_t s);
hipError_t agcm_mlp_q8_launch(const f16 *in, f16 *out, size_t npix, const int8_t *wfrag, const float *consts, float q1_inv, float q1_zoff,
                              float zoff2, float zoff3, hipStream_t s);
hipError_t planar3_to_q8_launch(const f16 *in, size_t npix, float inv, float zoff, int8_t *out, hipStream_t s);
struct AgcmFoldQ8Args {
    FakeQ q20, qlin[6];
    const float *P, *Q;
    float inv2, inv3;
    float *consts;
};
hipError_t agcm_fold_q8_launch(const AgcmFoldArgs &a, const AgcmFoldQ8Args &q, float *biasbuf, hipStream_t s);
hipError_t hg_prep_launch(const f16 *base, int H, int W, int Hp, int Wp, f16 *img_pad, uint8_t *mask, float r, float thresh,
                          hipStream_t s, uint8_t *flags = nullptr);
constexpr int HG_NEED_MAX_LAYERS = 24, HG_NEED_MAX_TENSORS = 32, HG_NEED_LEVELS = 6;
constexpr int hg_need_unit_log2[3][HG_NEED_LEVELS] = {{4, 4, 4, 4, 4, 4}, {4, 4, 4, 4, 4, 4}, {4, 2, 1, 0, 0, 0}};
struct HgNeedLayer {
    int level, mode, ks;
    int in, skip, out;
    int in_first, skip_first;
    int out_chained;
    int in_chained;
    int th;
    int list_off;
};
struct HgNeedParams {
    unsigned char *base;
    int Hp, Wp, n_layers;
    int lu[HG_NEED_LEVELS];
    int flags_off;
    int flags_map;
    int kbits_off, tbits_off, scratch_words;
    int map_off[HG_NEED_MAX_TENSORS];
    HgNeedLayer L[HG_NEED_MAX_LAYERS];
};
hipError_t hg_need_launch(const HgNeedParams &p, hipStream_t s);
struct HgFinalFusedArgs {
    const f16 *img;
    const uint8_t *mask;
    const float *part;
    const f16 *wfrag;
    const float *scale, *shift, *b10, *wl, *bl;
    void *out;
    int out_f32, H, W, Hp, Wp;
};
hipError_t hg_final_fused_launch(const HgFinalFusedArgs &a, int n_cu, hipStream_t s);
hipError_t hg_final_light_launch(const HgFinalFusedArgs &a, const float *part2, hipStream_t s);
hipError_t letterbox_launch(const LetterboxParams &p, hipStream_t s);
hipError_t post_scale_launch(const PostScaleParams &p, int is_f32, int pq, hipStream_t s);
hipError_t post_ycbcr10_launch(const Ycbcr10Params &p, int is_f32, int pq, hipStream_t s);
hipError_t rgb48_to_ycbcr10_launch(const Ycbcr10Params &p, hipStream_t s);
hipError_t metrics_launch(const MetricsParams &p, hipStream_t s);
int metrics_blocks(int H, int W);

hipError_t conv_f32_launch(const F32ConvParams &p, int ks, int stride, int n_cu, hipStream_t s);
bool conv_f32_on_mfma(const F32ConvParams &p, int ks, int n_cu);
hipError_t ew_f32_launch(int op, const float *a, const float *b, const float *c, float *y, size_t n, hipStream_t s);
hipError_t avgpool3s2_leaky_f32_launch(const float *x, float *y, int C, int H, int W, float slope, hipStream_t s);
hipError_t instnorm_f32_launch(float *x, const float *gamma, const float *beta, int C, int n, float eps, hipStream_t s);
hipError_t plane_mean_f32_launch(const float *x, float *y, int C, int n, hipStream_t s);
hipError_t gfm_heads_f32_launch(const F32GfmParams &p, hipStream_t s);
hipError_t maxpool2_f32_launch(const float *x, float *y, int C, int H, int W, hipStream_t s);
hipError_t window_f32_launch(const float *x, float *y, int C, int H, int W, int Ho, int Wo, int mode, hipStream_t s);
hipError_t hg_mask_f32_launch(const float *base, float *mask, size_t npix, float r, hipStream_t s);
hipError_t hg_blend_f32_launch(const float *t, const float *img, const float *mask, float *out, int H, int W, int Hp, int Wp,
                               hipStream_t s);
hipError_t pre_f32_launch(const uint8_t *bgr, float *rgb, float *cond, int H, int W, int Ho, int Wo, const float *wx,
                          const int *xmn, const int *xns, const float *wy, const int *ymn, const int *yns, int mode, hipStream_t s);
```

hdr-realtime-video-pipeline_amd/csrc/le_hg_misc.hip:

```cpp
#include "launchers.h"

namespace {

constexpr int C3_TH = 8, C3_TW = 32;
constexpr int C3_HH = C3_TH + 2, C3_HW = C3_TW + 2;
constexpr int C3_PW = C3_HW + 2;
constexpr int C3_NP = (C3_HH * C3_HW + 255) / 256;

__device__ __forceinline__ f16x8 c3_frag(const f16x4 *s_px, int row, int ky, int l31, int lh)
{
    const f16x4 *q = s_px + (row + ky) * C3_PW + l31 + 2 * lh;
    const f16x4 a = q[0], b = q[1];
    return f16x8{a[0], a[1], a[2], a[3], b[0], b[1], b[2], b[3]};
}

struct C3Pre { f16 v[C3_NP][3]; bool ok[C3_NP]; };
__device__ __forceinline__ void c3_fetch(C3Pre &pre, const f16 *__restrict__ in, int H, int W, int oy0, int ox0, int tid)
{
#pragma unroll
    for (int i = 0; i < C3_NP; ++i) {
        const int e = tid + 256 * i;
        const int r = e / C3_HW, q = e % C3_HW;
        const int iy = oy0 - 1 + r, ix = ox0 - 1 + q;
        const bool ok = e < C3_HH * C3_HW && iy >= 0 && iy < H && ix >= 0 && ix < W;
        const size_t o = ok ? (size_t)iy * W + ix : 0;
        pre.ok[i] = ok;
#pragma unroll
        for (int c = 0; c < 3; ++c) {
            pre.v[i][c] = in[(size_t)c * H * W + o];
            if (!ok) pre.v[i][c] = (f16)0.f;
        }
    }
}
__device__ __forceinline__ void c3_stage(const C3Pre &pre, f16x4 *s_px, int tid)
{
#pragma unroll
    for (int i = 0; i < C3_NP; ++i) {
        const int e = tid + 256 * i;
        if (e < C3_HH * C3_HW) s_px[(e / C3_HW) * C3_PW + e % C3_HW] = f16x4{pre.v[i][0], pre.v[i][1], pre.v[i][2], (f16)1.f};
    }
}

template <int COUT, bool DOT = false>
__global__ __launch_bounds__(256) void conv_c3_kernel(const f16 *__restrict__ in, int H, int W, const f16 *__restrict__ wfrag,
                                                      const float *__restrict__ scale, const float *__restrict__ shift,
                                                      int act, f16 *__restrict__ out, f16 *__restrict__ out_pool, float pool_q_inv,
                                                      float pool_q_zero, const f16 *__restrict__ w2frag = nullptr,
                                                      float *__restrict__ part2 = nullptr)
{
    static_assert(!DOT || COUT == 64, "the fused conv10 half belongs to HG.conv1");
    constexpr int MT = COUT / 32;
    constexpr int ROWB = COUT * 2 + 16;
    __shared__ __attribute__((aligned(16))) f16x4 s_px_all[(DOT ? 2 : 1) * C3_HH * C3_PW];
    f16x4 *s_px = s_px_all;
    __shared__ __attribute__((aligned(16))) char s_out[C3_TH * C3_TW * ROWB];
    __shared__ __attribute__((aligned(16))) float s_ss[2 * COUT];
    const int tid = threadIdx.x, lane = tid & 63, wave = tid >> 6, l31 = lane & 31, lh = lane >> 5;
    const int tiles_x = (W + C3_TW - 1) / C3_TW, ntiles = tiles_x * ((H + C3_TH - 1) / C3_TH);
    if (tid < COUT) { s_ss[tid] = scale[tid]; s_ss[COUT + tid] = shift[tid]; }
    __shared__ __attribute__((aligned(16))) f16x8 s_w2[DOT ? 4 * 64 : 1];
    if constexpr (DOT) s_w2[tid] = reinterpret_cast<const f16x8 *>(w2frag)[tid];
    f16x8 wf[MT][3];
#pragma unroll
    for (int i = 0; i < MT; ++i)
#pragma unroll
        for (int ky = 0; ky < 3; ++ky) wf[i][ky] = reinterpret_cast<const f16x8 *>(wfrag)[(i * 3 + ky) * 64 + lane];
    for (int e = tid; e < C3_HH * 2 * (DOT ? 2 : 1); e += 256)
        s_px_all[(e / (C3_HH * 2)) * (C3_HH * C3_PW) + ((e % (C3_HH * 2)) >> 1) * C3_PW + C3_HW + (e & 1)] = f16x4{(f16)0.f, (f16)0.f, (f16)0.f, (f16)0.f};
    C3Pre pre;
    auto fetch = [&](int t) { c3_fetch(pre, in, H, W, (t / tiles_x) * C3_TH, (t % tiles_x) * C3_TW, tid); };
    const float aslope = act_slope(act);
    int t = blockIdx.x;
    if (t < ntiles) fetch(t);
    int pbuf = 0;
    if constexpr (DOT) {
        if (t < ntiles) c3_stage(pre, s_px_all, tid);
        if (t + (int)gridDim.x < ntiles) fetch(t + gridDim.x);
    }
    for (; t < ntiles; t += gridDim.x) {
    const int ox0 = (t % tiles_x) * C3_TW, oy0 = (t / tiles_x) * C3_TH;
    if constexpr (DOT) {
        __syncthreads();
        s_px = s_px_all + pbuf * (C3_HH * C3_PW);
        if (t + (int)gridDim.x < ntiles) c3_stage(pre, s_px_all + (pbuf ^ 1) * (C3_HH * C3_PW), tid);
        if (t + 2 * (int)gridDim.x < ntiles) fetch(t + 2 * gridDim.x);
        pbuf ^= 1;
    } else {
        __syncthreads();
        c3_stage(pre, s_px, tid);
        __syncthreads();
        if (t + (int)gridDim.x < ntiles) fetch(t + gridDim.x);
    }
    f32x16 acc[MT][2];
    auto dot_row = [&](int j) __attribute__((always_inline)) {
        const int q = (2 * wave + j) * C3_TW + l31;
        f16x8 bf[4];
#pragma unroll
        for (int i = 0; i < MT; ++i)
#pragma unroll
            for (int qd = 0; qd < 4; ++qd) {
                const int cl = i * 32 + 8 * qd + 4 * lh;
                const float4 sc = *reinterpret_cast<const float4 *>(s_ss + cl);
                const float4 sh = *reinterpret_cast<const float4 *>(s_ss + COUT + cl);
                f16x4 o;
                o[0] = (f16)act_fast(acc[i][j][4 * qd + 0] * sc.x + sh.x, aslope);
                o[1] = (f16)act_fast(acc[i][j][4 * qd + 1] * sc.y + sh.y, aslope);
                o[2] = (f16)act_fast(acc[i][j][4 * qd + 2] * sc.z + sh.z, aslope);
                o[3] = (f16)act_fast(acc[i][j][4 * qd + 3] * sc.w + sh.w, aslope);
                *reinterpret_cast<f16x4 *>(s_out + q * ROWB + cl * 2) = o;
#pragma unroll
                for (int k = 0; k < 4; ++k) bf[2 * i + (qd >> 1)][4 * (qd & 1) + k] = o[k];
            }
        f32x16 o3;
#pragma unroll
        for (int k = 0; k < 16; ++k) o3[k] = 0.f;
#pragma unroll
        for (int s4 = 0; s4 < 4; ++s4) o3 = __builtin_amdgcn_mfma_f32_32x32x16_f16(s_w2[s4 * 64 + lane], bf[s4], o3, 0, 0, 0);
        const int y = oy0 + 2 * wave + j, x = ox0 + l31;
        if (lh == 0 && y < H && x < W) *reinterpret_cast<float4 *>(part2 + ((size_t)y * W + x) * 4) = make_float4(o3[0], o3[1], o3[2], 0.f);
    };
#pragma unroll
    for (int j = 0; j < 2; ++j) {
        const int row = 2 * wave + j;
        f16x8 xf[3];
#pragma unroll
        for (int ky = 0; ky < 3; ++ky) xf[ky] = c3_frag(s_px, row, ky, l31, lh);
#pragma unroll
        for (int i = 0; i < MT; ++i) {
#pragma unroll
            for (int k = 0; k < 16; ++k) acc[i][j][k] = 0.f;
#pragma unroll
            for (int ky = 0; ky < 3; ++ky) acc[i][j] = __builtin_amdgcn_mfma_f32_32x32x16_f16(wf[i][ky], xf[ky], acc[i][j], 0, 0, 0);
        }
        if constexpr (DOT) {
            dot_row(j);
            __builtin_amdgcn_sched_barrier(0);
        }
    }
    if constexpr (!DOT) {
#pragma unroll
        for (int i = 0; i < MT; ++i)
#pragma unroll
            for (int qd = 0; qd < 4; ++qd) {
                const int cl = i * 32 + 8 * qd + 4 * lh;
                const float4 sc = *reinterpret_cast<const float4 *>(s_ss + cl);
                const float4 sh = *reinterpret_cast<const float4 *>(s_ss + COUT + cl);
#pragma unroll
                for (int j = 0; j < 2; ++j) {
                    const int q = (2 * wave + j) * C3_TW + l31;
                    f16x4 o;
                    o[0] = (f16)act_fast(acc[i][j][4 * qd + 0] * sc.x + sh.x, aslope);
                    o[1] = (f16)act_fast(acc[i][j][4 * qd + 1] * sc.y + sh.y, aslope);
                    o[2] = (f16)act_fast(acc[i][j][4 * qd + 2] * sc.z + sh.z, aslope);
                    o[3] = (f16)act_fast(acc[i][j][4 * qd + 3] * sc.w + sh.w, aslope);
                    *reinterpret_cast<f16x4 *>(s_out + q * ROWB + cl * 2) = o;
                }
            }
    }
    constexpr int CPP = COUT / 8;
    if constexpr (DOT) {
        const int Hq = H / 2, Wq = W / 2;
#pragma unroll
        for (int it = 0; it < 2; ++it) {
            const int e = lane + 64 * it;
            const int px = e / CPP, c8 = e % CPP;
            const int oy = oy0 / 2 + wave, ox = ox0 / 2 + px;
            const int q00 = 2 * wave * C3_TW + 2 * px;
            f16x8 v = *reinterpret_cast<const f16x8 *>(s_out + q00 * ROWB + c8 * 16);
            const f16x8 v1 = *reinterpret_cast<const f16x8 *>(s_out + (q00 + 1) * ROWB + c8 * 16);
            const f16x8 v2 = *reinterpret_cast<const f16x8 *>(s_out + (q00 + C3_TW) * ROWB + c8 * 16);
            const f16x8 v3 = *reinterpret_cast<const f16x8 *>(s_out + (q00 + C3_TW + 1) * ROWB + c8 * 16);
#pragma unroll
            for (int k = 0; k < 8; ++k) {
                const f16 m = v[k] > v1[k] ? v[k] : v1[k];
                const f16 m2 = v2[k] > v3[k] ? v2[k] : v3[k];
                v[k] = m > m2 ? m : m2;
            }
            if (oy < Hq && ox < Wq) {
                if (pool_q_inv > 0.f) {
                    unsigned lo = 0, hi = 0;
                    const float z128 = pool_q_zero + 128.f;
                    lo = __builtin_amdgcn_cvt_pk_u8_f32((float)v[0] * pool_q_inv + z128, 0, lo);
                    lo = __builtin_amdgcn_cvt_pk_u8_f32((float)v[1] * pool_q_inv + z128, 1, lo);
                    lo = __builtin_amdgcn_cvt_pk_u8_f32((float)v[2] * pool_q_inv + z128, 2, lo);
                    lo = __builtin_amdgcn_cvt_pk_u8_f32((float)v[3] * pool_q_inv + z128, 3, lo);
                    hi = __builtin_amdgcn_cvt_pk_u8_f32((float)v[4] * pool_q_inv + z128, 0, hi);
                    hi = __builtin_amdgcn_cvt_pk_u8_f32((float)v[5] * pool_q_inv + z128, 1, hi);
                    hi = __builtin_amdgcn_cvt_pk_u8_f32((float)v[6] * pool_q_inv + z128, 2, hi);
                    hi = __builtin_amdgcn_cvt_pk_u8_f32((float)v[7] * pool_q_inv + z128, 3, hi);
                    lo ^= 0x80808080u; hi ^= 0x80808080u;
                    *reinterpret_cast<uint2 *>(reinterpret_cast<int8_t *>(out_pool) + ((size_t)oy * Wq + ox) * COUT + c8 * 8) = make_uint2(lo, hi);
                } else {
                    *reinterpret_cast<f16x8 *>(out_pool + ((size_t)oy * Wq + ox) * COUT + c8 * 8) = v;
                }
            }
        }
        continue;
    }
    __syncthreads();
    for (int e = tid; e < C3_TH * C3_TW * CPP; e += 256) {
        const int q = e / CPP, c8 = e % CPP;
        const int oy = oy0 + q / C3_TW, ox = ox0 + q % C3_TW;
        if (out && oy < H && ox < W)
            *reinterpret_cast<f16x8 *>(out + ((size_t)oy * W + ox) * COUT + c8 * 8) =
                *reinterpret_cast<const f16x8 *>(s_out + q * ROWB + c8 * 16);
    }
    if (out_pool) {
        const int Hp = H / 2, Wp = W / 2;
        for (int e = tid; e < (C3_TH / 2) * (C3_TW / 2) * CPP; e += 256) {
            const int pq = e / CPP, c8 = e % CPP;
            const int py = pq / (C3_TW / 2), px = pq % (C3_TW / 2);
            const int oy = oy0 / 2 + py, ox = ox0 / 2 + px;
            if (oy < Hp && ox < Wp) {
                const int q00 = 2 * py * C3_TW + 2 * px;
                f16x8 v = *reinterpret_cast<const f16x8 *>(s_out + q00 * ROWB + c8 * 16);
                const f16x8 v1 = *reinterpret_cast<const f16x8 *>(s_out + (q00 + 1) * ROWB + c8 * 16);
                const f16x8 v2 = *reinterpret_cast<const f16x8 *>(s_out + (q00 + C3_TW) * ROWB + c8 * 16);
                const f16x8 v3 = *reinterpret_cast<const f16x8 *>(s_out + (q00 + C3_TW + 1) * ROWB + c8 * 16);
#pragma unroll
                for (int k = 0; k < 8; ++k) {
                    const f16 m = v[k] > v1[k] ? v[k] : v1[k];
                    const f16 m2 = v2[k] > v3[k] ? v2[k] : v3[k];
                    v[k] = m > m2 ? m : m2;
                }
                if (pool_q_inv > 0.f) {
                    unsigned lo = 0, hi = 0;
                    const float z128 = pool_q_zero + 128.f;
                    lo = __builtin_amdgcn_cvt_pk_u8_f32((float)v[0] * pool_q_inv + z128, 0, lo);
                    lo = __builtin_amdgcn_cvt_pk_u8_f32((float)v[1] * pool_q_inv + z128, 1, lo);
                    lo = __builtin_amdgcn_cvt_pk_u8_f32((float)v[2] * pool_q_inv + z128, 2, lo);
                    lo = __builtin_amdgcn_cvt_pk_u8_f32((float)v[3] * pool_q_inv + z128, 3, lo);
                    hi = __builtin_amdgcn_cvt_pk_u8_f32((float)v[4] * pool_q_inv + z128, 0, hi);
                    hi = __builtin_amdgcn_cvt_pk_u8_f32((float)v[5] * pool_q_inv + z128, 1, hi);
                    hi = __builtin_amdgcn_cvt_pk_u8_f32((float)v[6] * pool_q_inv + z128, 2, hi);
                    hi = __builtin_amdgcn_cvt_pk_u8_f32((float)v[7] * pool_q_inv + z128, 3, hi);
                    lo ^= 0x80808080u; hi ^= 0x80808080u;
                    *reinterpret_cast<uint2 *>(reinterpret_cast<int8_t *>(out_pool) + ((size_t)oy * Wp + ox) * COUT + c8 * 8) = make_uint2(lo, hi);
                } else {
                    *reinterpret_cast<f16x8 *>(out_pool + ((size_t)oy * Wp + ox) * COUT + c8 * 8) = v;
                }
            }
        }
    }
    }
}

__global__ __launch_bounds__(256) void conv_c3_q8_kernel(const f16 *__restrict__ in, int H, int W, const i32x4 *__restrict__ wq,
                                                         const float *__restrict__ scale, const float *__restrict__ shift,
                                                         float q_inv, float q_zoff, int act, f16 *__restrict__ out)
{
    constexpr int COUT = 32, ROWB = COUT * 2 + 16;
    __shared__ __attribute__((aligned(16))) int s_px[C3_HH * C3_PW];
    __shared__ __attribute__((aligned(16))) char s_out[C3_TH * C3_TW * ROWB];
    __shared__ __attribute__((aligned(16))) float s_ss[17 * COUT];
    const int tid = threadIdx.x, lane = tid & 63, wave = tid >> 6, l31 = lane & 31, lh = lane >> 5;
    const int tiles_x = (W + C3_TW - 1) / C3_TW, ntiles = tiles_x * ((H + C3_TH - 1) / C3_TH);
    for (int e = tid; e < 17 * COUT; e += 256) s_ss[e] = e < COUT ? scale[e] : shift[e - COUT];
    const i32x4 w0 = wq[lane], w1 = wq[64 + lane];
    for (int e = tid; e < C3_HH * 2; e += 256) s_px[(e >> 1) * C3_PW + C3_HW + (e & 1)] = 0;
    C3Pre pre;
    auto fetch = [&](int t) { c3_fetch(pre, in, H, W, (t / tiles_x) * C3_TH, (t % tiles_x) * C3_TW, tid); };
    const float aslope = act_slope(act);
    int t = blockIdx.x;
    if (t < ntiles) fetch(t);
    for (; t < ntiles; t += gridDim.x) {
        const int ox0 = (t % tiles_x) * C3_TW, oy0 = (t / tiles_x) * C3_TH;
        __syncthreads();
#pragma unroll
        for (int i = 0; i < C3_NP; ++i) {
            const int e = tid + 256 * i;
            if (e < C3_HH * C3_HW)
                s_px[(e / C3_HW) * C3_PW + e % C3_HW] =
                    pre.ok[i] ? (int)quant4((float)pre.v[i][0], (float)pre.v[i][1], (float)pre.v[i][2], 0.f, q_inv, q_zoff) : 0;
        }
        __syncthreads();
        if (t + (int)gridDim.x < ntiles) fetch(t + gridDim.x);
#pragma unroll
        for (int j = 0; j < 2; ++j) {
            const int row = 2 * wave + j;
// ... 161 lines not shown
            }
        }
    }
    }
}
#endif

struct HgFinalLightParams {
    const f16 *img;
    const uint8_t *mask;
    const float *part, *part2;
    const float *b10, *wl, *bl;
    void *out;
    int out_f32, H, W, Hp, Wp;
};

__global__ __launch_bounds__(256) void hg_final_light_kernel(HgFinalLightParams p)
{
    const int nx = (p.W + 3) >> 2;
    const size_t total = (size_t)p.H * nx, plane_i = (size_t)p.Hp * p.Wp, plane_o = (size_t)p.H * p.W;
    float b10[3], wl[18], bl[3];
#pragma unroll
    for (int k = 0; k < 3; ++k) { b10[k] = p.b10[k]; bl[k] = p.bl[k]; }
#pragma unroll
    for (int k = 0; k < 18; ++k) wl[k] = p.wl[k];
    for (size_t e = (size_t)blockIdx.x * 256 + threadIdx.x; e < total; e += (size_t)gridDim.x * 256) {
        const int y = (int)(e / nx), x0 = (int)(e - (size_t)y * nx) * 4;
        const size_t pix = (size_t)y * p.Wp + x0;
        const uint32_t m4 = *reinterpret_cast<const uint32_t *>(p.mask + pix);
        float4 pt[4], p2[4];
#pragma unroll
        for (int k = 0; k < 4; ++k) {
            pt[k] = p2[k] = make_float4(0.f, 0.f, 0.f, 0.f);
            if ((m4 >> (8 * k)) & 0xff) { pt[k] = reinterpret_cast<const float4 *>(p.part)[pix + k]; p2[k] = reinterpret_cast<const float4 *>(p.part2)[pix + k]; }
        }
        f16x4 iv[3];
#pragma unroll
        for (int ch = 0; ch < 3; ++ch) iv[ch] = *reinterpret_cast<const f16x4 *>(p.img + ch * plane_i + pix);
        float res[3][4];
#pragma unroll
        for (int k = 0; k < 4; ++k) {
            const float c10[3] = {(float)(f16)(p2[k].x + pt[k].x + b10[0]), (float)(f16)(p2[k].y + pt[k].y + b10[1]),
                                  (float)(f16)(p2[k].z + pt[k].z + b10[2])};
            const float im[3] = {(float)iv[0][k], (float)iv[1][k], (float)iv[2][k]};
            const float m = (float)((m4 >> (8 * k)) & 0xff);
#pragma unroll
            for (int ch = 0; ch < 3; ++ch) {
                float v = bl[ch];
#pragma unroll
                for (int t = 0; t < 3; ++t) v += wl[ch * 6 + t] * c10[t] + wl[ch * 6 + 3 + t] * im[t];
                v = (float)(f16)v;
                res[ch][k] = m != 0.f ? m * v + im[ch] : im[ch];
            }
        }
        const size_t oo = (size_t)y * p.W + x0;
        const bool vec = (p.W & 3) == 0;
#pragma unroll
        for (int ch = 0; ch < 3; ++ch) {
            if (p.out_f32) {
                float *d = reinterpret_cast<float *>(p.out) + ch * plane_o + oo;
                if (vec) *reinterpret_cast<float4 *>(d) = make_float4(res[ch][0], res[ch][1], res[ch][2], res[ch][3]);
                else for (int k = 0; k < 4 && x0 + k < p.W; ++k) d[k] = res[ch][k];
            } else {
                f16 *d = reinterpret_cast<f16 *>(p.out) + ch * plane_o + oo;
                if (vec) *reinterpret_cast<f16x4 *>(d) = f16x4{(f16)res[ch][0], (f16)res[ch][1], (f16)res[ch][2], (f16)res[ch][3]};
                else for (int k = 0; k < 4 && x0 + k < p.W; ++k) d[k] = (f16)res[ch][k];
            }
        }
    }
}

inline int grid_for(size_t n, int per_block)
{
    size_t g = (n + per_block - 1) / per_block;
    if (g > 4096) g = 4096;
    if (g < 1) g = 1;
    return (int)g;
}

}

hipError_t conv_c3_launch(const f16 *in, int H, int W, const f16 *wfrag, const float *scale, const float *shift, int cout,
                          int act, f16 *out, f16 *out_pool, int n_cu, hipStream_t s, float pool_q_inv, float pool_q_zero,
                          const f16 *w2frag, float *part2)
{
    if ((w2frag != nullptr) != (part2 != nullptr) || (part2 && (cout != 64 || out || !out_pool))) return hipErrorInvalidValue;
    const int ntiles = ((W + C3_TW - 1) / C3_TW) * ((H + C3_TH - 1) / C3_TH);
    static int occ[3] = {0, 0, 0};
    int &per_cu = occ[part2 ? 2 : (cout == 64)];
    if (per_cu == 0) {
        int nb = 0;
        const hipError_t e = cout == 32 ? hipOccupancyMaxActiveBlocksPerMultiprocessor(&nb, conv_c3_kernel<32>, 256, 0)
                           : part2 ? hipOccupancyMaxActiveBlocksPerMultiprocessor(&nb, conv_c3_kernel<64, true>, 256, 0)
                                   : hipOccupancyMaxActiveBlocksPerMultiprocessor(&nb, conv_c3_kernel<64>, 256, 0);
        per_cu = (e == hipSuccess && nb >= 1) ? nb : 2;
    }
    const dim3 grid(ntiles < per_cu * n_cu ? ntiles : per_cu * n_cu);
    if (cout == 32)
        hipLaunchKernelGGL(conv_c3_kernel<32>, grid, dim3(256), 0, s, in, H, W, wfrag, scale, shift, act, out, out_pool, pool_q_inv, pool_q_zero,
                           (const f16 *)nullptr, (float *)nullptr);
    else if (cout == 64 && part2)
        hipLaunchKernelGGL((conv_c3_kernel<64, true>), grid, dim3(256), 0, s, in, H, W, wfrag, scale, shift, act, out, out_pool, pool_q_inv, pool_q_zero,
                           w2frag, part2);
    else if (cout == 64)
        hipLaunchKernelGGL(conv_c3_kernel<64>, grid, dim3(256), 0, s, in, H, W, wfrag, scale, shift, act, out, out_pool, pool_q_inv, pool_q_zero,
                           (const f16 *)nullptr, (float *)nullptr);
    else
        return hipErrorInvalidValue;
    return hipGetLastError();
}

hipError_t conv_c3_q8_launch(const f16 *in, int H, int W, const int8_t *wq, const float *scale, const float *shift, float q_inv,
                             float q_zoff, int act, f16 *out, int n_cu, hipStream_t s)
{
    const int ntiles = ((W + C3_TW - 1) / C3_TW) * ((H + C3_TH - 1) / C3_TH);
    static int per_cu = 0;
    if (per_cu == 0) {
        int nb = 0;
        per_cu = (hipOccupancyMaxActiveBlocksPerMultiprocessor(&nb, conv_c3_q8_kernel, 256, 0) == hipSuccess && nb >= 1) ? nb : 2;
    }
    const dim3 grid(ntiles < per_cu * n_cu ? ntiles : per_cu * n_cu);
    hipLaunchKernelGGL(conv_c3_q8_kernel, grid, dim3(256), 0, s, in, H, W, reinterpret_cast<const i32x4 *>(wq), scale, shift, q_inv, q_zoff,
                       act, out);
    return hipGetLastError();
}

hipError_t hg_prep_launch(const f16 *base, int H, int W, int Hp, int Wp, f16 *img_pad, uint8_t *mask, float r, float thresh,
                          hipStream_t s, uint8_t *flags)
{
    hipLaunchKernelGGL(hg_prep_kernel, dim3(grid_for((size_t)Hp * Wp, 256)), dim3(256), 0, s, base, H, W, Hp, Wp, img_pad,
                       mask, r, thresh, flags);
    return hipGetLastError();
}

hipError_t hg_final_light_launch(const HgFinalFusedArgs &a, const float *part2, hipStream_t s)
{
    if (!part2 || (a.Wp & 31) || a.W > a.Wp || a.H > a.Hp) return hipErrorInvalidValue;
    HgFinalLightParams p;
    p.img = a.img; p.mask = a.mask; p.part = a.part; p.part2 = part2; p.b10 = a.b10; p.wl = a.wl; p.bl = a.bl;
    p.out = a.out; p.out_f32 = a.out_f32; p.H = a.H; p.W = a.W; p.Hp = a.Hp; p.Wp = a.Wp;
    hipLaunchKernelGGL(hg_final_light_kernel, dim3(grid_for((size_t)a.H * ((a.W + 3) / 4), 256)), dim3(256), 0, s, p);
    return hipGetLastError();
}

#ifdef HDRTV_AB
hipError_t hg_final_fused_launch(const HgFinalFusedArgs &a, int n_cu, hipStream_t s)
{
    HgFinalFusedParams p;
    p.img = a.img; p.mask = a.mask; p.part = a.part; p.wfrag = a.wfrag; p.scale = a.scale; p.shift = a.shift;
    p.b10 = a.b10; p.wl = a.wl; p.bl = a.bl; p.out = a.out; p.out_f32 = a.out_f32; p.H = a.H; p.W = a.W; p.Hp = a.Hp; p.Wp = a.Wp;
    const int ntiles = ((a.W + C3_TW - 1) / C3_TW) * ((a.H + C3_TH - 1) / C3_TH);
    static int per_cu = 0;
    if (per_cu == 0) {
        int nb = 0;
        if (hipOccupancyMaxActiveBlocksPerMultiprocessor(&nb, hg_final_fused_kernel, 256, 0) != hipSuccess || nb < 1) nb = 3;
        per_cu = nb;
    }
    const int grid = ntiles < per_cu * n_cu ? ntiles : per_cu * n_cu;
    hipLaunchKernelGGL(hg_final_fused_kernel, dim3(grid), dim3(256), 0, s, p);
    return hipGetLastError();
}
#endif
```

hdr-realtime-video-pipeline_amd/hdrtv_mi355x/lib.py:

```python
from __future__ import annotations

import ctypes as C
import os
from typing import NamedTuple

_PKG = os.path.dirname(os.path.abspath(__file__))
LIB_PATH = os.path.join(os.path.dirname(_PKG), "lib", "libhdrtv_mi355x.so")
LIB_PATH_AB = os.path.join(os.path.dirname(_PKG), "lib", "libhdrtv_mi355x_ab.so")

OK, EINVAL, EWEIGHTS, EHIP, ENOMEM, ESTATE = 0, -1, -2, -3, -4, -5
F16, F32 = 0, 1
PREC_F16, PREC_F32 = 0, 1
YUV_I420, YUV_NV12 = 0, 1
YCC_P010, YCC_YUV420P10, YCC_YUV422P10 = 0, 1, 2
SITING_LEFT, SITING_TOPLEFT = 0, 1

_VP, _I, _SZ = C.c_void_p, C.c_int, C.c_size_t
SYMBOLS = [
    ("hdrtv_version", C.c_char_p, []),
    ("hdrtv_create", _I, [_VP, _SZ, _VP, _SZ, _I, C.POINTER(_VP)]),
    ("hdrtv_create_ex", _I, [_VP, _SZ, _VP, _SZ, _I, _I, C.POINTER(_VP)]),
    ("hdrtv_destroy", _I, [_VP]),
    ("hdrtv_has_hg", _I, [_VP]),
    ("hdrtv_set_hg_mask_r", _I, [_VP, C.c_float]),
    ("hdrtv_set_cond_mode", _I, [_VP, _I]),
    ("hdrtv_reserve", _I, [_VP, _I, _I]),
    ("hdrtv_preprocess", _I, [_VP, _VP, _VP, _I, _I, _VP, _VP]),
    ("hdrtv_infer", _I, [_VP, _VP, _VP, _VP, _I, _I, _VP, _I, _VP]),
    ("hdrtv_set_lanes", _I, [_VP, _I]),
    ("hdrtv_get_lanes", _I, [_VP]),
    ("hdrtv_infer_lane", _I, [_VP, _I, _VP, _VP, _VP, _I, _I, _VP, _I, _VP]),
    ("hdrtv_post_u8", _I, [_VP, _VP, _VP, _I, _I, _I, _VP]),
    ("hdrtv_post_rgb48", _I, [_VP, _VP, _VP, _I, _I, _I, _VP]),
    ("hdrtv_post_pq_rgb48", _I, [_VP, _VP, _VP, _I, _I, _I, C.c_float, _VP]),
    ("hdrtv_post_rgb48_scaled", _I, [_VP, _VP, _VP, _I, _I, _I, _I, C.c_float, _VP, _I, _I]),
    ("hdrtv_post_ycbcr10", _I, [_VP, _VP, _VP, _I, _I, _I, _I, C.c_float, _I, _I, _VP, _I, _VP, _VP, _I]),
    ("hdrtv_rgb48_to_ycbcr10", _I, [_VP, _VP, _VP, _I, _I, _I, _I, _VP, _I, _VP, _VP, _I]),
    ("hdrtv_ycbcr10_bytes", C.c_int64, [_I, _I, _I]),
    ("hdrtv_letterbox_u8", _I, [_VP, _VP, _VP, _I, _I, _VP, _I, _I]),
    ("hdrtv_yuv420_to_bgr_u8", _I, [_VP, _VP, _VP, _I, _VP, _VP, _I, _I, _I, _I, _I, _I, _VP]),
    ("hdrtv_preprocess_yuv420", _I, [_VP, _VP, _VP, _I, _VP, _VP, _I, _I, _I, _I, _I, _I, _VP, _VP]),
    ("hdrtv_metrics", _I, [_VP, _VP, _VP, _VP, _I, _I, _I, C.c_float, C.POINTER(C.c_double)]),
    ("hdrtv_ring_create", _I, [_VP, _I, _I, _I]),
    ("hdrtv_ring_acquire", _I, [_VP, _I, C.POINTER(_VP), C.POINTER(_VP)]),
    ("hdrtv_ring_commit", _I, [_VP, _I, _VP]),
    ("hdrtv_ring_commit_bytes", _I, [_VP, _I, _VP, _SZ]),
    ("hdrtv_ring_wait", _I, [_VP, _I]),
    ("hdrtv_ring_release", _I, [_VP, _I]),
    ("hdrtv_ring_destroy", _I, [_VP]),
    ("hdrtv_get_tap", _I, [_VP, C.c_char_p, C.POINTER(_VP), C.POINTER(_I), C.POINTER(_I), C.POINTER(_I), C.POINTER(_I)]),
    ("hdrtv_infer_stats", _I, [_VP, C.POINTER(_I), C.POINTER(C.c_double)]),
    ("hdrtv_profile_enable", _I, [_VP, _I]),
    ("hdrtv_profile_get", _I, [_VP, _I, C.POINTER(C.c_char_p), C.POINTER(C.c_char_p), C.POINTER(C.c_float),
                               C.POINTER(C.c_double), C.POINTER(C.c_double)]),
    ("hdrtv_set_variant", _I, [_VP, C.c_char_p, _I]),
    ("hdrtv_get_variant", _I, [_VP, C.c_char_p, C.POINTER(_I)]),
    ("hdrtv_last_error", C.c_char_p, [_VP]),
]

YCC_FORMATS = {"p010le": YCC_P010, "yuv420p10le": YCC_YUV420P10, "yuv422p10le": YCC_YUV422P10}
YCC_SITINGS = {"left": SITING_LEFT, "topleft": SITING_TOPLEFT}
OUT_PIX_FMTS = ("rgb48le",) + tuple(YCC_FORMATS)


def check_out_format(pix_fmt, siting="left"):
    pix_fmt, siting = str(pix_fmt).lower(), str(siting).lower()
    if pix_fmt not in OUT_PIX_FMTS:
        raise ValueError(f"out_pix_fmt must be one of {list(OUT_PIX_FMTS)}")
    if siting not in YCC_SITINGS:
        raise ValueError(f"out_siting must be one of {sorted(YCC_SITINGS)}")
    if pix_fmt == "yuv422p10le" and siting != "left":
        raise ValueError("4:2:2 chroma is horizontally co-sited: out_siting must be 'left'")
    return pix_fmt, siting


class OutputFormat(NamedTuple):
    pix_fmt: str
    siting: str
    h: int
    w: int

    @property
    def is_rgb48(self):
        return self.pix_fmt == "rgb48le"

    @property
    def nbytes(self):
        return self.h * self.w * (6 if self.is_rgb48 else 4 if self.pix_fmt == "yuv422p10le" else 3)

    @property
    def shape(self):
        return (self.h, self.w, 3) if self.is_rgb48 else (self.nbytes // 2,)

    def at(self, h, w):
        return self if (h, w) == (self.h, self.w) else output_format(self.pix_fmt, self.siting, h, w)

    def planes(self, ptr):
        if self.is_rgb48:
            raise ValueError("rgb48le has no Y'CbCr planes")
        fmt, sit, h, w = YCC_FORMATS[self.pix_fmt], YCC_SITINGS[self.siting], self.h, self.w
        u = ptr + h * w * 2
        if fmt == YCC_P010:
            return fmt, sit, ptr, 2 * w, u, None, 2 * w
        ch = h if fmt == YCC_YUV422P10 else h // 2
        return fmt, sit, ptr, 2 * w, u, u + ch * w, w


def output_format(pix_fmt, siting, h, w):
    pix_fmt, siting = check_out_format(pix_fmt, siting)
    h, w = int(h), int(w)
    if pix_fmt != "rgb48le" and (h <= 0 or w <= 0 or w % 2 or (pix_fmt != "yuv422p10le" and h % 2)):
        raise ValueError(f"{pix_fmt} needs an even width{'' if pix_fmt == 'yuv422p10le' else ' and height'} (got {w}x{h})")
    return OutputFormat(pix_fmt, siting, h, w)


def out_frame_bytes(pix_fmt, h, w):
    return output_format(pix_fmt, "left", h, w).nbytes


def ycbcr10_planes(ptr, h, w, pix_fmt, siting="left"):
    return output_format(pix_fmt, siting, h, w).planes(ptr)


_libs = {}


def load(ab=False):
    path = LIB_PATH_AB if ab else LIB_PATH
    if path in _libs:
        return _libs[path]
    if not os.path.exists(path):
        raise RuntimeError(
            f"{path} not found: the MI355X HIP extension is not built and there is no "
            "fallback path (run __graft_entry__.build())")
    import torch
    lib = C.CDLL(path)
    for name, res, args in SYMBOLS:
# ... 28 lines not shown
```

hdr-realtime-video-pipeline_amd/hdrtv_mi355x/processor.py:

```python
from __future__ import annotations

import ctypes as C
import os
import time

import numpy as np
import torch

from . import lib as _L
from . import weights as _W


def _split_composite(state):
    if not any(k.startswith("base.") for k in state):
        return state, None
    hr = {k[5:]: v for k, v in state.items() if k.startswith("base.")}
    hg = {k[3:]: v for k, v in state.items() if k.startswith("hg.")}
    return hr, (hg or None)


def _load_state(path_or_state, what):
    if isinstance(path_or_state, dict):
        return path_or_state
    path = str(path_or_state)
# ... 512 lines not shown

    def tap(self, name):
        p, c, h, w, lay = C.c_void_p(), C.c_int(), C.c_int(), C.c_int(), C.c_int()
        self._chk(self._lib.hdrtv_get_tap(self._ctx, name.encode(), C.byref(p), C.byref(c), C.byref(h), C.byref(w),
                                          C.byref(lay)), "hdrtv_get_tap")
        n = c.value * h.value * w.value
        torch.cuda.synchronize(self.device)
        if lay.value in (0, 1):
            buf = torch.empty(n, dtype=torch.float16, device=self.device)
        elif lay.value == 4:
            buf = torch.empty(n, dtype=torch.uint8, device=self.device)
        elif lay.value == 5:
            buf = torch.empty(n, dtype=torch.int8, device=self.device)
        else:
            buf = torch.empty(n, dtype=torch.float32, device=self.device)
        _hip_memcpy_d2d(buf.data_ptr(), p.value, buf.numel() * buf.element_size())
        torch.cuda.synchronize(self.device)
        if lay.value in (0, 5):
            return buf.view(h.value, w.value, c.value).permute(2, 0, 1).float().cpu()
        return buf.view(c.value, h.value, w.value).float().cpu()

    def _tap_device(self, name):
        p, c, h, w, lay = C.c_void_p(), C.c_int(), C.c_int(), C.c_int(), C.c_int()
        self._chk(self._lib.hdrtv_get_tap(self._ctx, name.encode(), C.byref(p), C.byref(c), C.byref(h), C.byref(w),
                                          C.byref(lay)), "hdrtv_get_tap")
        dt = {0: torch.float16, 1: torch.float16, 4: torch.uint8, 5: torch.int8}.get(lay.value, torch.float32)
        buf = torch.empty(c.value * h.value * w.value, dtype=dt, device=self.device)
        torch.cuda.synchronize(self.device)
        _hip_memcpy_d2d(buf.data_ptr(), p.value, buf.numel() * buf.element_size())
        torch.cuda.synchronize(self.device)
        return buf

    @torch.inference_mode()
    def calibrate_hg_w8a8(self, frames):
        if self._hg_state_fp is None:
            raise RuntimeError("calibrate_hg_w8a8 needs a model loaded with floating-point HG weights")
        members = {"p1": ("hg.p1",), "conv2+up4": ("hg.conv2", "hg.up4"), "p3": ("hg.p3",), "conv3_2+up3": ("hg.conv3_2", "hg.up3"), "p4": ("hg.p4",),
                   "conv4_2+up2": ("hg.conv4_2", "hg.up2"), "p5": ("hg.p5",), "conv5_2+up1": ("hg.conv5_2", "hg.up1"),
                   "pc": ("hg.pc",), "conv_code2": ("hg.conv_code2",), "conv6": ("hg.conv6",), "conv7": ("hg.conv7",),
                   "conv8": ("hg.conv8",), "conv9": ("hg.conv9",)}
        assert list(members) == list(_W.HG_W8A8_GROUPS)
        ranges = {g: [0.0, 0.0] for g in members}
        for f in frames:
            self.infer(self.preprocess(f))
            for g, taps in members.items():
                for t in taps:
                    v = self._tap_device(t)
                    ranges[g][0] = min(ranges[g][0], float(v.amin()))
                    ranges[g][1] = max(ranges[g][1], float(v.amax()))
        return {g: (lo, hi) for g, (lo, hi) in ranges.items()}

    def hg_w8a8_checkpoint(self, ranges):
        if self._hg_state_fp is None:
            raise RuntimeError("hg_w8a8_checkpoint needs a model loaded with floating-point HG weights")
        return _W.hg_w8a8_state(self._hg_state_fp, ranges)

    def set_hg_mask_r(self, r=0.75):
        self._chk(self._lib.hdrtv_set_hg_mask_r(self._ctx, float(r)), "hdrtv_set_hg_mask_r")
        self._graphs.clear()

    def set_variant(self, name, value):
        self._chk(self._lib.hdrtv_set_variant(self._ctx, name.encode(), int(value)), "hdrtv_set_variant")
        self._graphs.clear()

    def get_variant(self, name):
        v = C.c_int()
        self._chk(self._lib.hdrtv_get_variant(self._ctx, name.encode(), C.byref(v)), "hdrtv_get_variant")
        return v.value

    def profile_enable(self, on=True):
        self._chk(self._lib.hdrtv_profile_enable(self._ctx, 1 if on else 0), "hdrtv_profile_enable")
        self._profiling = bool(on)

    def profile_read(self):
        n = self._lib.hdrtv_profile_get(self._ctx, -1, None, None, None, None, None)
        out = []
        for i in range(max(n, 0)):
            layer, kern, ms, macs, nbytes = C.c_char_p(), C.c_char_p(), C.c_float(), C.c_double(), C.c_double()
            self._chk(self._lib.hdrtv_profile_get(self._ctx, i, C.byref(layer), C.byref(kern), C.byref(ms),
                                                  C.byref(macs), C.byref(nbytes)), "hdrtv_profile_get")
            out.append((layer.value.decode(), kern.value.decode(), ms.value, macs.value, nbytes.value))
        return out

    def execution_summary(self, profile=None):
        return summarize_profile(profile if profile is not None else self.profile_read())

    def infer_stats(self):
        n, m = C.c_int(), C.c_double()
        self._lib.hdrtv_infer_stats(self._ctx, C.byref(n), C.byref(m))
        return n.value, m.value

    def close(self):
        if getattr(self, "_ctx", None) and self._ctx.value:
            self._lib.hdrtv_destroy(self._ctx)
            self._ctx = C.c_void_p()

    def __del__(self):
        try:
            self.close()
        except Exception:
            pass


def _arch_hr():
    from . import arch
    return arch.hr_params()


_hip = None


YUV_LAYOUTS = {"i420": _L.YUV_I420, "yuv420p": _L.YUV_I420, "nv12": _L.YUV_NV12}


def _yuv_frame_hw(frame):
    if frame.ndim != 2 or frame.dtype != np.uint8 or frame.shape[0] % 3:
        raise ValueError("a 4:2:0 frame must be uint8 [H*3//2, W]")
    h, w = frame.shape[0] // 3 * 2, frame.shape[1]
    if h % 2 or w % 2 or h <= 0:
        raise ValueError(f"4:2:0 frames have even sizes (got {w}x{h})")
    return h, w


def _yuv_planes(ptr, h, w, layout, matrix, full_range):
    code = YUV_LAYOUTS.get(str(layout).lower())
    if code is None:
        raise ValueError(f"layout must be one of {sorted(YUV_LAYOUTS)}")
    u = ptr + h * w
    if code == _L.YUV_NV12:
        return ptr, w, u, None, w, code, int(matrix), int(bool(full_range))
    return ptr, w, u, u + (h // 2) * (w // 2), w // 2, code, int(matrix), int(bool(full_range))


def _hip_memcpy_d2d(dst, src, nbytes):
    global _hip
    if _hip is None:
        _hip = C.CDLL("libamdhip64.so")
        _hip.hipMemcpy.argtypes = [C.c_void_p, C.c_void_p, C.c_size_t, C.c_int]
        _hip.hipMemcpy.restype = C.c_int
    rc = _hip.hipMemcpy(dst, src, nbytes, 3)
    if rc != 0:
        raise RuntimeError(f"hipMemcpy failed: {rc}")
```

include/hdrtv_mi355x.h:

```cpp
#ifndef HDRTV_MI355X_H
#define HDRTV_MI355X_H

#include <stddef.h>
#include <stdint.h>

#ifdef __cplusplus
extern "C" {
#endif

#define HDRTV_OK 0
#define HDRTV_EINVAL (-1)
#define HDRTV_EWEIGHTS (-2)
#define HDRTV_EHIP (-3)
#define HDRTV_ENOMEM (-4)
#define HDRTV_ESTATE (-5)

typedef struct hdrtv_ctx hdrtv_ctx;

#define HDRTV_F16 0
#define HDRTV_F32 1

const char *hdrtv_version(void);

int hdrtv_create(const void *hr_pack, size_t hr_bytes, const void *hg_pack, size_t hg_bytes,
                 int device_id, hdrtv_ctx **out);

#define HDRTV_PREC_F16 0
#define HDRTV_PREC_F32 1
int hdrtv_create_ex(const void *hr_pack, size_t hr_bytes, const void *hg_pack, size_t hg_bytes,
                    int device_id, int precision, hdrtv_ctx **out);
int hdrtv_destroy(hdrtv_ctx *ctx);

int hdrtv_has_hg(const hdrtv_ctx *ctx);

int hdrtv_set_cond_mode(hdrtv_ctx *ctx, int mode);

int hdrtv_set_hg_mask_r(hdrtv_ctx *ctx, float r);

int hdrtv_reserve(hdrtv_ctx *ctx, int H, int W);

int hdrtv_preprocess(hdrtv_ctx *ctx, void *stream, const uint8_t *dev_bgr_hwc, int H, int W,
                     void *dev_rgb_chw, void *dev_cond);

int hdrtv_infer(hdrtv_ctx *ctx, void *stream, const void *dev_rgb_chw, const void *dev_cond, int H,
                int W, void *dev_out, int out_dtype, void *dev_agcm_out);

int hdrtv_set_lanes(hdrtv_ctx *ctx, int lanes);
int hdrtv_get_lanes(const hdrtv_ctx *ctx);
int hdrtv_infer_lane(hdrtv_ctx *ctx, int lane, void *stream, const void *dev_rgb_chw, const void *dev_cond, int H,
                     int W, void *dev_out, int out_dtype, void *dev_agcm_out);

int hdrtv_post_u8(hdrtv_ctx *ctx, void *stream, const void *dev_out, int dtype, int H, int W,
                  uint8_t *dev_bgr_hwc);

int hdrtv_post_rgb48(hdrtv_ctx *ctx, void *stream, const void *dev_out, int dtype, int H, int W,
                     uint16_t *dst);

int hdrtv_post_pq_rgb48(hdrtv_ctx *ctx, void *stream, const void *dev_out, int dtype, int H, int W,
                        float peak_nits, uint16_t *dst);

int hdrtv_post_rgb48_scaled(hdrtv_ctx *ctx, void *stream, const void *dev_out, int dtype, int H, int W,
                            int pq, float peak_nits, uint16_t *dst, int dH, int dW);

#define HDRTV_YCC_P010 0
#define HDRTV_YCC_YUV420P10 1
#define HDRTV_YCC_YUV422P10 2
#define HDRTV_SITING_LEFT 0
#define HDRTV_SITING_TOPLEFT 1
int hdrtv_post_ycbcr10(hdrtv_ctx *ctx, void *stream, const void *dev_out, int dtype, int H, int W, int pq, float peak_nits,
                       int fmt, int siting, uint16_t *dst_y, int y_pitch, uint16_t *dst_u, uint16_t *dst_v, int c_pitch);
int hdrtv_rgb48_to_ycbcr10(hdrtv_ctx *ctx, void *stream, const uint16_t *src_rgb48, int H, int W, int fmt, int siting,
                           uint16_t *dst_y, int y_pitch, uint16_t *dst_u, uint16_t *dst_v, int c_pitch);
int64_t hdrtv_ycbcr10_bytes(int fmt, int H, int W);

int hdrtv_letterbox_u8(hdrtv_ctx *ctx, void *stream, const uint8_t *dev_src_bgr, int sh, int sw,
                       uint8_t *dev_dst_bgr, int dh, int dw);

#define HDRTV_YUV_I420 0
#define HDRTV_YUV_NV12 1
int hdrtv_yuv420_to_bgr_u8(hdrtv_ctx *ctx, void *stream, const uint8_t *dev_y, int y_pitch,
                           const uint8_t *dev_u, const uint8_t *dev_v, int c_pitch, int layout,
                           int matrix, int full_range, int H, int W, uint8_t *dev_bgr_hwc);
int hdrtv_preprocess_yuv420(hdrtv_ctx *ctx, void *stream, const uint8_t *dev_y, int y_pitch,
                            const uint8_t *dev_u, const uint8_t *dev_v, int c_pitch, int layout,
                            int matrix, int full_range, int H, int W, void *dev_rgb_chw, void *dev_cond);

int hdrtv_metrics(hdrtv_ctx *ctx, void *stream, const void *dev_a, const void *dev_b, int dtype, int H, int W,
                  float peak_nits, double *out3);

int hdrtv_ring_create(hdrtv_ctx *ctx, int slots, int H, int W);
int hdrtv_ring_acquire(hdrtv_ctx *ctx, int timeout_ms, uint16_t **host_ptr, uint16_t **dev_ptr);
int hdrtv_ring_commit(hdrtv_ctx *ctx, int slot, void *stream);
int hdrtv_ring_commit_bytes(hdrtv_ctx *ctx, int slot, void *stream, size_t bytes);
int hdrtv_ring_wait(hdrtv_ctx *ctx, int slot);
int hdrtv_ring_release(hdrtv_ctx *ctx, int slot);
int hdrtv_ring_destroy(hdrtv_ctx *ctx);

int hdrtv_get_tap(hdrtv_ctx *ctx, const char *name, void **dev_ptr, int *C, int *H, int *W,
                  int *layout);
int hdrtv_infer_stats(hdrtv_ctx *ctx, int *launches, double *macs);

int hdrtv_profile_enable(hdrtv_ctx *ctx, int on);
int hdrtv_profile_get(hdrtv_ctx *ctx, int i, const char **layer, const char **kernel, float *ms, double *macs,
                      double *bytes);

int hdrtv_set_variant(hdrtv_ctx *ctx, const char *name, int value);
int hdrtv_get_variant(hdrtv_ctx *ctx, const char *name, int *value);

const char *hdrtv_last_error(const hdrtv_ctx *ctx);

#ifdef __cplusplus
}
#endif
#endif
```

Before: 137.5.

## Extend sparse tile lists to HG conv1, pglds and glds1 convolutions

New measurement: 146.9, median of 6. +6.8%, better.

```diff
diff --git a/hdr-realtime-video-pipeline_amd/csrc/api.h b/hdr-realtime-video-pipeline_amd/csrc/api.h
--- a/hdr-realtime-video-pipeline_amd/csrc/api.h
+++ b/hdr-realtime-video-pipeline_amd/csrc/api.h
@@ -225,7 +225,7 @@
     double macs = 0.0;
     bool prof_on = false;
     std::vector<hipEvent_t> prof_ev;
-    struct ProfEntry { std::string layer, kernel; double macs, bytes; float ms; const int *cnt; int cnt_total; };
+    struct ProfEntry { std::string layer, kernel; double macs, bytes; float ms; const int *cnt; int cnt_total; bool cnt_scales; };
     bool taps_partial = false, taps_replayable = false;
     hipStream_t taps_stream = nullptr;
     std::vector<ProfEntry> prof;
@@ -334,20 +334,20 @@
         }
         (void)hipEventRecord(c->prof_ev[i], s);
     }
-    void chk(hipError_t e, const char *what, const char *kernel = "", double macs = 0.0, double bytes = 0.0, const int *cnt = nullptr, int cnt_total = 0)
+    void chk(hipError_t e, const char *what, const char *kernel = "", double macs = 0.0, double bytes = 0.0, const int *cnt = nullptr, int cnt_total = 0, bool cnt_scales = true)
     {
         ++c->launches;
         c->macs += macs;
         if (e != hipSuccess && rc == HDRTV_OK) rc = fail(c, HDRTV_EHIP, "launch %s failed: %s", what, hipGetErrorString(e));
         if (c->prof_on) {
-            c->prof.push_back({what, kernel, macs, bytes, 0.f, cnt, cnt_total});
+            c->prof.push_back({what, kernel, macs, bytes, 0.f, cnt, cnt_total, cnt_scales});
             mark();
         }
     }
     void conv(const std::string &key, const f16 *src0, int c0, const f16 *src1, int c1, int Hi, int Wi, int act, int mode, f16 *dst, int dstC, int Hd, int Wd, const f16 *res1 = nullptr, const f16 *res2 = nullptr, f16 *dst_full = nullptr, f16 *dst_planar = nullptr, const f16 *res_planar = nullptr, const float *dotw = nullptr, float *dst_dot = nullptr, int s0_stride = 0);
     void conv8(const std::string &key, const int8_t *src0, int c0, const int8_t *src1, int c1, int Hi, int Wi, int mode, void *dst, int dstC, int Hd, int Wd, const float *dotw = nullptr, float *dst_dot = nullptr);
     void convq8(const std::string &key, const void *src, bool src_i8, int src_stride, int Hi, int Wi, int act, void *dst, int dstC, const ActQf *oq);
-    void c3(const std::string &key, const f16 *in, int H, int W, int act, f16 *out, f16 *out_pool, float pool_q_inv = 0.f, float pool_q_zero = 0.f, const f16 *w2frag = nullptr, float *part2 = nullptr);
+    void c3(const std::string &key, const f16 *in, int H, int W, int act, f16 *out, f16 *out_pool, float pool_q_inv = 0.f, float pool_q_zero = 0.f, const f16 *w2frag = nullptr, float *part2 = nullptr, const int *need = nullptr, int need_tiles = 0);
     void conv32(const std::string &key, const f16 *src, const f16 *cond, const std::string &sft_key, int H, int W, int act, int mode, f16 *dst, int dstC, int Hd, int Wd, const f16 *res1 = nullptr, const f16 *res2 = nullptr, f16 *dst_planar = nullptr, const f16 *res_planar = nullptr, const f16 *c3_img = nullptr, const std::string &c3_key = "");
     template <typename T>
     T *wsp(const std::string &name) const { return hdrtv_host::wsp<T>(c, ws, name); }
diff --git a/hdr-realtime-video-pipeline_amd/csrc/api_graph.hip b/hdr-realtime-video-pipeline_amd/csrc/api_graph.hip
--- a/hdr-realtime-video-pipeline_amd/csrc/api_graph.hip
+++ b/hdr-realtime-video-pipeline_amd/csrc/api_graph.hip
@@ -60,8 +60,16 @@
         snprintf(tag, sizeof tag, "%s<%s>", prw_th == 8 ? "conv_prw8" : "conv_prw", epi);
         e = conv_prw_launch(p, prw_th, c->n_cu, s, &list_taken);
         break;
-    case PGLDS: snprintf(tag, sizeof tag, "conv_pglds<%s>", epi); e = conv_pglds_launch(p, c->n_cu, s); break;
-    case GLDS1: snprintf(tag, sizeof tag, "conv_glds1"); e = conv_glds1_launch(p, s, c->n_cu, c->var.at("glds1_old") != 0); break;
+    case PGLDS:
+        if (need && need_rows == 16) p.tile_list = need;
+        snprintf(tag, sizeof tag, "conv_pglds<%s>", epi);
+        e = conv_pglds_launch(p, c->n_cu, s, &list_taken);
+        break;
+    case GLDS1:
+        if (need && need_rows == 16) p.tile_list = need;
+        snprintf(tag, sizeof tag, "conv_glds1");
+        e = conv_glds1_launch(p, s, c->n_cu, c->var.at("glds1_old") != 0, &list_taken);
+        break;
     default:
         snprintf(tag, sizeof tag, "conv_igemm<%d,%d,%d,%d>", L.cin_t, L.bn, L.ks, L.stride);
         e = conv_igemm_launch(p, L.cin_t, L.bn, L.ks, L.stride, s);
@@ -76,7 +84,7 @@
                                           : (mode == ST_PLANAR3 ? 3.0 * Hd * Wd
                                                                 : (mode == ST_PS_DOT3 ? 8.0 * Hd * Wd : (double)p.Ho * p.Wo * L.cout));
     bytes += 2.0 * outel * (1 + (res1 ? 1 : 0) + (res2 ? 1 : 0) + (res_planar ? 1 : 0));
-    chk(e, key.c_str(), tag, macs, bytes, list_taken ? p.tile_list : nullptr, need_cells);
+    chk(e, key.c_str(), tag, macs, bytes, list_taken ? p.tile_list : nullptr, need_cells, route == PRW);
 }
 
 
@@ -142,14 +150,17 @@
 }
 
 
-void Seq::c3(const std::string &key, const f16 *in, int H, int W, int act, f16 *out, f16 *out_pool, float pool_q_inv, float pool_q_zero, const f16 *w2frag, float *part2)
+void Seq::c3(const std::string &key, const f16 *in, int H, int W, int act, f16 *out, f16 *out_pool, float pool_q_inv, float pool_q_zero, const f16 *w2frag, float *part2, const int *need, int need_tiles)
 {
     if (!ok()) return;
     const C3Layer &L = c->c3.at(key);
-    chk(conv_c3_launch(in, H, W, wtp<f16>(c, L.wfrag), wtp<float>(c, L.scale), wtp<float>(c, L.shift), L.cout, act, out,
-                       out_pool, c->n_cu, s, pool_q_inv, pool_q_zero, w2frag, part2), key.c_str(),
+    bool list_taken = false;
+    const hipError_t e = conv_c3_launch(in, H, W, wtp<f16>(c, L.wfrag), wtp<float>(c, L.scale), wtp<float>(c, L.shift), L.cout, act, out,
+                                        out_pool, c->n_cu, s, pool_q_inv, pool_q_zero, w2frag, part2, need, &list_taken);
+    chk(e, key.c_str(),
         part2 ? "conv_c3<64,dot3>" : (L.cout == 64 ? "conv_c3<64>" : "conv_c3<32>"), (double)H * W * (27 * L.cout + (part2 ? 192 : 0)),
-        (double)H * W * (6.0 + (out ? 2.0 * L.cout : 0.0) + (out_pool ? (pool_q_inv > 0.f ? 0.25 : 0.5) * L.cout : 0.0) + (part2 ? 16.0 : 0.0)));
+        (double)H * W * (6.0 + (out ? 2.0 * L.cout : 0.0) + (out_pool ? (pool_q_inv > 0.f ? 0.25 : 0.5) * L.cout : 0.0) + (part2 ? 16.0 : 0.0)),
+        list_taken ? need : nullptr, need_tiles, false);
 }
 
 
@@ -572,7 +583,7 @@
     memset(&p, 0, sizeof p);
     p.Hp = Hp; p.Wp = Wp;
     constexpr int n_layers = (int)(sizeof hg_layers / sizeof hg_layers[0]);
-    static_assert(n_layers <= HG_NEED_MAX_LAYERS && n_layers + 2 <= HG_NEED_MAX_TENSORS, "hg_need's tables are too small");
+    static_assert(n_layers + 1 <= HG_NEED_MAX_LAYERS && n_layers + 3 <= HG_NEED_MAX_TENSORS, "hg_need's tables are too small");
     constexpr int max_level = [] { int m = 0; for (const HgLayer &L : hg_layers) m = L.level > m ? L.level : m; return m; }();
     static_assert(max_level < HG_NEED_LEVELS, "hg_need's unit tables have too few levels");
     memcpy(p.lu, hg_need_unit_log2[c->var.at("hg_sparse") == 1 ? 1 : 2], sizeof p.lu);
@@ -596,17 +607,26 @@
     };
     for (int i = 0; i < n_layers; ++i) {
         const HgLayer &L = hg_layers[i];
-        HgNeedLayer &N = p.L[i];
-        N.level = L.level; N.ks = L.ks;
+        HgNeedLayer &N = p.L[i + 1];
+        N.level = L.level; N.ks = L.ks; N.tw = 16;
         N.mode = L.mode == ST_POOL ? 1 : (L.ps ? 2 : 0);
         N.in = tensor(L.in, L.level);
         N.skip = L.skip ? tensor(L.skip, L.level) : -1;
         N.out = tensor(L.out, L.out_level());
         N.th = L.ks == 3 && Seq::prw_tile_rows(c, L.mode, L.cout, Hp >> L.level, Wp >> L.level) == 8 ? 8 : 16;
     }
-    p.n_layers = n_layers;
+    const int nt_table = nt;
+    {
+        HgNeedLayer &N = p.L[0];
+        N.level = 0; N.ks = 3; N.mode = 1;
+        N.out = tensor(hg_layers[0].in, 1);
+        N.in = tensor("img", 0);
+        N.skip = -1;
+        N.th = 8; N.tw = 32;
+    }
+    p.n_layers = n_layers + 1;
     bool seen[HG_NEED_MAX_TENSORS] = {};
-    for (int i = n_layers - 1; i >= 0; --i) {
+    for (int i = p.n_layers - 1; i >= 0; --i) {
         HgNeedLayer &N = p.L[i];
         N.in_first = !seen[N.in];
         seen[N.in] = true;
@@ -616,22 +636,24 @@
     auto take = [&](size_t bytes) { const size_t o = off; off = (off + bytes + 15) & ~(size_t)15; return (int)o; };
     p.flags_off = take((size_t)ncell(0));
     take((size_t)ncell(0));
-    for (int t = 0; t < nt; ++t)
+    for (int t = 0; t < nt_table; ++t)
         if (strcmp(names[t], "part")) take((size_t)ncell(level[t]));
-    for (int i = 0; i < n_layers; ++i) p.L[i].list_off = take(4 * (2 * (size_t)ncell(p.L[i].level) + 4));
+    for (int i = 1; i <= n_layers; ++i) p.L[i].list_off = take(4 * (2 * (size_t)ncell(p.L[i].level) + 4));
     size_t scratch = 0;
-    for (int t = 0; t < nt; ++t) {
+    for (int t = 0; t < nt; ++t) scratch = std::max(scratch, nwords(level[t]));
+    for (int t = 0; t < nt_table; ++t) {
         p.map_off[t] = take(8 * nwords(level[t]));
-        scratch = std::max(scratch, nwords(level[t]));
         if (!strcmp(names[t], "part")) p.flags_map = t;
     }
-    for (int i = 0; i < n_layers; ++i) {
-        p.L[i].out_chained = i + 1 < n_layers ? p.L[i + 1].in == p.L[i].out : p.L[i].out == p.flags_map;
+    for (int i = 0; i < p.n_layers; ++i) {
+        p.L[i].out_chained = i + 1 < p.n_layers ? p.L[i + 1].in == p.L[i].out : p.L[i].out == p.flags_map;
         p.L[i].in_chained = i > 0 && p.L[i - 1].out == p.L[i].in;
     }
     p.scratch_words = (int)scratch;
     p.kbits_off = take(8 * scratch);
     p.tbits_off = take(8 * scratch);
+    p.L[0].list_off = take(4 * (2 * (size_t)ncell(0) + 4));
+    p.map_off[nt_table] = take(8 * nwords(0));
     return off;
 }
 
@@ -675,12 +697,14 @@
         tp[nt] = q.wsp<void>(key);
         return tp[nt++];
     };
-    q.c3("hg.conv1", img, Hp, Wp, ACT_RELU, nullptr, (f16 *)tensor(hg_layers[0].in), c->hg_q0_inv, c->hg_q0_zero, w2frag, part2);
+    const bool c1_list = sparse && light;
+    q.c3("hg.conv1", img, Hp, Wp, ACT_RELU, nullptr, (f16 *)tensor(hg_layers[0].in), c->hg_q0_inv, c->hg_q0_zero, w2frag, part2,
+         c1_list ? reinterpret_cast<const int *>(np.base + np.L[0].list_off) : nullptr, c1_list ? ((Hp + 7) / 8) * ((Wp + 31) / 32) : 0);
     char key[32];
     for (const HgLayer &L : hg_layers) {
         snprintf(key, sizeof key, "hg.%s", L.name);
         if (sparse) {
-            const HgNeedLayer &N = np.L[&L - hg_layers];
+            const HgNeedLayer &N = np.L[&L - hg_layers + 1];
             q.need_list = reinterpret_cast<const int *>(np.base + N.list_off);
             q.need_th = N.th;
             q.need_total = (((Hp >> L.level) + N.th - 1) / N.th) * (((Wp >> L.level) + 15) / 16);
diff --git a/hdr-realtime-video-pipeline_amd/csrc/conv1x1_glds.hip b/hdr-realtime-video-pipeline_amd/csrc/conv1x1_glds.hip
--- a/hdr-realtime-video-pipeline_amd/csrc/conv1x1_glds.hip
+++ b/hdr-realtime-video-pipeline_amd/csrc/conv1x1_glds.hip
@@ -164,6 +164,7 @@
 constexpr int P_NST = 8;
 constexpr int P_SP = 144;
 constexpr int P_MAXC = 512;
+constexpr int P_LIST_N = 512;
 
 __global__ __launch_bounds__(512) void conv_glds1p_kernel(ConvParams p)
 {
@@ -174,8 +175,10 @@
     const int wave = __builtin_amdgcn_readfirstlane(tid >> 6);
     const int l31 = lane & 31, lh = lane >> 5;
 
+    const float my_scale = tid < p.CoutPad ? p.scale[tid] : 0.f, my_shift = tid < p.CoutPad ? p.shift[tid] : 0.f;
     const int ntn = p.CoutPad / BN;
-    const int total = p.tiles_x * p.tiles_y * ntn;
+    const int *const lst = p.tile_list;
+    const int total = (lst ? lst[0] : p.tiles_x * p.tiles_y) * ntn;
     int t_first, t_step, ntile;
     {
         const int G = gridDim.x, b = blockIdx.x, xcd = b & 7, slot = b >> 3;
@@ -188,10 +191,16 @@
         ntile = slot < len ? (len - slot + nslots - 1) / nslots : 0;
     }
     if (ntile == 0) return;
+    __shared__ int s_list_mem[P_LIST_N];
+    volatile __attribute__((address_space(3))) int *s_list = (volatile __attribute__((address_space(3))) int *)s_list_mem;
+    if (lst && tid < ntile) s_list[tid] = lst[1 + (t_first + tid * t_step) / ntn];
     struct Tile { int n0, oy0, ox0; };
-    auto decode = [&](int t) {
+    auto decode = [&](int k) {
         Tile o;
-        const int nt_i = t % ntn, sp = t / ntn;
+        const int t = t_first + k * t_step;
+        const int nt_i = t % ntn;
+        int sp = t / ntn;
+        if (lst) sp = __builtin_amdgcn_readfirstlane(s_list[k]);
         const int ty = sp / p.tiles_x, tx = sp - ty * p.tiles_x;
         o.n0 = nt_i * BN; o.oy0 = ty * TH; o.ox0 = tx * TW;
         return o;
@@ -244,10 +253,10 @@
     const float act_lb = p.act == ACT_RELU ? 0.f : -__builtin_inff();
     char *trash = reinterpret_cast<char *>(p.trash) + lane * 16;
     __shared__ __attribute__((aligned(16))) float s_ss[2 * P_MAXC];
-    for (int e = tid; e < p.CoutPad; e += 512) { s_ss[e] = p.scale[e]; s_ss[P_MAXC + e] = p.shift[e]; }
+    if (tid < p.CoutPad) { s_ss[tid] = my_scale; s_ss[P_MAXC + tid] = my_shift; }
     __syncthreads();
 
-    Tile cur = decode(t_first), nxt = cur;
+    Tile cur = decode(0), nxt = cur;
     issue(cur, 0, 0);
     issue(cur, 1, 1);
     asm volatile("s_waitcnt vmcnt(6)" ::: "memory");
@@ -255,7 +264,7 @@
     int slot = 0;
     for (int k = 0; k < ntile; ++k) {
         const bool has_next = k + 1 < ntile;
-        if (has_next) nxt = decode(t_first + (k + 1) * t_step);
+        if (has_next) nxt = decode(k + 1);
 #pragma unroll 1
         for (int cc = 0; cc < nchunk; ++cc) {
             const int s2 = slot == 0 ? 2 : slot - 1;
@@ -327,8 +336,9 @@
 
 }
 
-hipError_t conv_glds1_launch(ConvParams p, hipStream_t stream, int n_cu, bool old_form)
+hipError_t conv_glds1_launch(ConvParams p, hipStream_t stream, int n_cu, bool old_form, bool *list_taken)
 {
+    if (list_taken) *list_taken = false;
     if ((p.c0 % CT) || (p.c1 % CT) || p.c0 + p.c1 < CT || (p.CoutPad % BN) || p.res1 || p.res2 || p.dst_full ||
         p.mode != ST_NHWC || !p.zeros)
         return hipErrorInvalidValue;
@@ -353,9 +363,13 @@
             if (e != hipSuccess) return e;
             attr_p.done();
         }
-        hipLaunchKernelGGL(conv_glds1p_kernel, dim3(grid < n_cu ? grid : n_cu), dim3(512), SMEM, stream, p);
+        const int g = grid < n_cu ? grid : n_cu;
+        if (p.tile_list && g >= 8 && (grid / 8 + 1 + g / 8 - 1) / (g / 8) > P_LIST_N) p.tile_list = nullptr;
+        if (list_taken) *list_taken = p.tile_list != nullptr;
+        hipLaunchKernelGGL(conv_glds1p_kernel, dim3(g), dim3(512), SMEM, stream, p);
         return hipGetLastError();
     }
+    p.tile_list = nullptr;
 #ifdef HDRTV_AB
     hipLaunchKernelGGL(conv_glds1_kernel, dim3(grid), dim3(512), SMEM, stream, p);
     return hipGetLastError();
diff --git a/hdr-realtime-video-pipeline_amd/csrc/conv3x3_pglds.hip b/hdr-realtime-video-pipeline_amd/csrc/conv3x3_pglds.hip
--- a/hdr-realtime-video-pipeline_amd/csrc/conv3x3_pglds.hip
+++ b/hdr-realtime-video-pipeline_amd/csrc/conv3x3_pglds.hip
@@ -9,7 +9,9 @@
 constexpr int B_BYTES = BN * PIXB, B_PIECES_PER_WAVE = 2;
 constexpr int SS_OFF = 2 * A_BYTES + 3 * B_BYTES;
 constexpr int DOTW_OFF = SS_OFF + 2048;
-constexpr int SMEM = DOTW_OFF + 1024;
+constexpr int LIST_OFF = DOTW_OFF + 1024;
+constexpr int LIST_N = 512;
+constexpr int SMEM = LIST_OFF + LIST_N * 4;
 
 template <int MODE> struct NStores { static constexpr int N = MODE == ST_POOL ? 2 : (MODE == ST_PS_DOT3 ? 1 : 8); };
 
@@ -47,7 +49,9 @@
     const int l15 = lane & 15, kg = lane >> 4;
 
     const int ntn = p.CoutPad / BN;
-    const int total = p.tiles_x * p.tiles_y * ntn;
+    const int *const lst = p.tile_list;
+    const int nsp = lst ? lst[0] : p.tiles_x * p.tiles_y;
+    const int total = nsp * ntn;
     int t_first, t_step, ntile;
     {
         const int G = gridDim.x, b = blockIdx.x, xcd = b & 7, slot = b >> 3;
@@ -60,10 +64,22 @@
         ntile = slot < len ? (len - slot + nslots - 1) / nslots : 0;
     }
     if (ntile == 0) return;
-    auto decode = [&](int t) {
+    volatile __attribute__((address_space(3))) int *s_list = (volatile __attribute__((address_space(3))) int *)(smem + LIST_OFF);
+    int sp_first = 0;
+    if (lst) {
+        sp_first = lst[1 + (p.nt_slow ? t_first % nsp : t_first / ntn)];
+        if (tid < ntile) {
+            const int t = t_first + tid * t_step;
+            s_list[tid] = lst[1 + (p.nt_slow ? t % nsp : t / ntn)];
+        }
+        asm volatile("s_waitcnt lgkmcnt(0)" ::: "memory");
+    }
+    auto decode = [&](int k) {
         Tile o;
-        const int nsp = p.tiles_x * p.tiles_y;
-        const int nt_i = p.nt_slow ? t / nsp : t % ntn, sp = p.nt_slow ? t - nt_i * nsp : t / ntn;
+        const int t = t_first + k * t_step;
+        const int nt_i = p.nt_slow ? t / nsp : t % ntn;
+        int sp = p.nt_slow ? t - nt_i * nsp : t / ntn;
+        if (lst) sp = k ? __builtin_amdgcn_readfirstlane(s_list[k]) : sp_first;
         const int ty = sp / p.tiles_x, tx = sp - ty * p.tiles_x;
         o.n0 = nt_i * BN; o.oy0 = ty * TH; o.ox0 = tx * TW;
         return o;
@@ -135,7 +151,7 @@
     const int b_lane = (wc * 64 + l15) * PIXB;
     const int a_lane = (wp * 4 * HW + l15) * PIXB;
 
-    Tile cur = decode(t_first), nxt = cur;
+    Tile cur = decode(0), nxt = cur;
     issue_A(0, 0, cur);
     issue_SS(cur.n0, 0);
     issue_B(0, cur.n0, 0);
@@ -147,7 +163,7 @@
     int gch = 0;
     for (int k = 0; k < ntile; ++k) {
         const bool has_next = k + 1 < ntile;
-        if (has_next) nxt = decode(t_first + (k + 1) * t_step);
+        if (has_next) nxt = decode(k + 1);
         for (int cc = 0; cc < nchunk; ++cc, ++gch) {
             const char *a = sA + (gch & 1) * A_BYTES;
             const bool last_chunk = cc + 1 == nchunk;
@@ -329,8 +345,9 @@
 
 }
 
-hipError_t conv_pglds_launch(ConvParams p, int n_cu, hipStream_t stream)
-{
+hipError_t conv_pglds_launch(ConvParams p, int n_cu, hipStream_t stream, bool *list_taken)
+{
+    if (list_taken) *list_taken = false;
     if ((p.c0 % CT) || (p.c1 % CT) || p.c0 + p.c1 < CT || (p.CoutPad % BN) || p.Cout != p.CoutPad || p.res1 || p.res2 ||
         p.dst_full || !p.zeros || !p.trash || n_cu < 8 || (p.act != ACT_RELU && p.act != ACT_NONE) ||
         (p.mode != ST_NHWC && p.mode != ST_PS && p.mode != ST_POOL && p.mode != ST_PS_DOT3) ||
@@ -340,6 +357,8 @@
     p.tiles_y = (p.Ho + TH - 1) / TH;
     const int total = p.tiles_x * p.tiles_y * (p.CoutPad / BN);
     const int grid = total < n_cu ? total : n_cu;
+    if (p.tile_list && grid >= 8 && (total / 8 + 1 + grid / 8 - 1) / (grid / 8) > LIST_N) p.tile_list = nullptr;
+    if (list_taken) *list_taken = p.tile_list != nullptr;
     switch (p.mode) {
     case ST_NHWC: return launch_mode<ST_NHWC>(p, grid, stream);
     case ST_PS: return launch_mode<ST_PS>(p, grid, stream);
diff --git a/hdr-realtime-video-pipeline_amd/csrc/hdrtv_api.hip b/hdr-realtime-video-pipeline_amd/csrc/hdrtv_api.hip
--- a/hdr-realtime-video-pipeline_amd/csrc/hdrtv_api.hip
+++ b/hdr-realtime-video-pipeline_amd/csrc/hdrtv_api.hip
@@ -743,7 +743,7 @@
     HIPCHK(c, hipEventSynchronize(c->prof_ev[i + 1]));
     HIPCHK(c, hipEventElapsedTime(&e.ms, c->prof_ev[i], c->prof_ev[i + 1]));
     double done = 1.0;
-    if (e.cnt && e.cnt_total > 0) {
+    if (e.cnt && e.cnt_total > 0 && e.cnt_scales) {
         int n = 0;
         HIPCHK(c, hipMemcpy(&n, e.cnt, sizeof n, hipMemcpyDeviceToHost));
         done = (double)n / (double)e.cnt_total;
@@ -756,6 +756,23 @@
     return HDRTV_OK;
 }
 
+int hdrtv_profile_tiles(hdrtv_ctx *c, int i, int *executed, int *total)
+{
+    if (!c) return HDRTV_EINVAL;
+    const int n = (int)c->prof.size();
+    if (i < 0 || i >= n || (size_t)i + 1 >= c->prof_ev.size()) return fail(c, HDRTV_EINVAL, "profile index out of range");
+    const hdrtv_ctx::ProfEntry &e = c->prof[i];
+    int done = 0, all = 0;
+    if (e.cnt && e.cnt_total > 0) {
+        HIPCHK(c, hipEventSynchronize(c->prof_ev[i + 1]));
+        HIPCHK(c, hipMemcpy(&done, e.cnt, sizeof done, hipMemcpyDeviceToHost));
+        all = e.cnt_total;
+    }
+    if (executed) *executed = done;
+    if (total) *total = all;
+    return HDRTV_OK;
+}
+
 const char *hdrtv_last_error(const hdrtv_ctx *c)
 {
     if (!c) return "null context";
diff --git a/hdr-realtime-video-pipeline_amd/csrc/hg_need.hip b/hdr-realtime-video-pipeline_amd/csrc/hg_need.hip
--- a/hdr-realtime-video-pipeline_amd/csrc/hg_need.hip
+++ b/hdr-realtime-video-pipeline_amd/csrc/hg_need.hip
@@ -85,8 +85,8 @@
         const Map mk = map_of(p, L.level), mo = map_of(p, olev);
         const int lu = p.lu[L.level], nk = mk.h * mk.nw;
         const int sh = p.lu[olev] - lu + olev - L.level;
-        const int lth = L.th == 8 ? 3 : 4, lbw = 4 - lu;
-        const int ty_n = ((p.Hp >> L.level) + L.th - 1) >> lth, tx_n = ((p.Wp >> L.level) + 15) >> 4, nt = ty_n * mk.nw;
+        const int lth = L.th == 8 ? 3 : 4, ltw = L.tw == 32 ? 5 : 4, lbw = ltw - lu;
+        const int ty_n = ((p.Hp >> L.level) + L.th - 1) >> lth, tx_n = ((p.Wp >> L.level) + (1 << ltw) - 1) >> ltw, nt = ty_n * mk.nw;
         const bool lds = max(nk, nt) <= LDS_WORDS;
         u64 *km = lds ? s_k : reinterpret_cast<u64 *>(p.base + p.kbits_off);
         u64 *tm = lds ? s_t : reinterpret_cast<u64 *>(p.base + p.tbits_off);
@@ -166,7 +166,9 @@
         const int olev = L.level + (L.mode == 1 ? 1 : 0) - (L.mode == 2 ? 1 : 0);
         if (L.level < 0 || L.level >= HG_NEED_LEVELS || olev < 0 || olev >= HG_NEED_LEVELS) return hipErrorInvalidValue;
         const int sh = p.lu[olev] - p.lu[L.level] + olev - L.level;
-        if (p.lu[L.level] < 0 || p.lu[L.level] > 4 || sh < -1 || sh > 1 || (L.th != 8 && L.th != 16)) return hipErrorInvalidValue;
+        if (p.lu[L.level] < 0 || p.lu[L.level] > 4 || sh < -1 || sh > 1 || (L.th != 8 && L.th != 16) ||
+            (L.tw != 0 && L.tw != 16 && L.tw != 32))
+            return hipErrorInvalidValue;
     }
     if (p.lu[0] != 4) return hipErrorInvalidValue;
     hipLaunchKernelGGL(hg_need_kernel, dim3(1), dim3(NT), 0, s, p);
diff --git a/hdr-realtime-video-pipeline_amd/csrc/launchers.h b/hdr-realtime-video-pipeline_amd/csrc/launchers.h
--- a/hdr-realtime-video-pipeline_amd/csrc/launchers.h
+++ b/hdr-realtime-video-pipeline_amd/csrc/launchers.h
@@ -9,8 +9,8 @@
 };
 
 hipError_t conv_igemm_launch(ConvParams p, int cin_t, int bn, int ks, int stride, hipStream_t stream);
-hipError_t conv_glds1_launch(ConvParams p, hipStream_t stream, int n_cu = 0, bool old_form = false);
-hipError_t conv_pglds_launch(ConvParams p, int n_cu, hipStream_t stream);
+hipError_t conv_glds1_launch(ConvParams p, hipStream_t stream, int n_cu = 0, bool old_form = false, bool *list_taken = nullptr);
+hipError_t conv_pglds_launch(ConvParams p, int n_cu, hipStream_t stream, bool *list_taken = nullptr);
 hipError_t conv_prw_launch(ConvParams p, int th, int n_cu, hipStream_t stream, bool *list_taken = nullptr);
 hipError_t conv_pglds_i8_launch(ConvI8Params p, int n_cu, hipStream_t stream);
 hipError_t conv_prw_i8_launch(ConvI8Params p, int th, int n_cu, hipStream_t stream);
@@ -54,7 +54,8 @@
 
 hipError_t conv_c3_launch(const f16 *in, int H, int W, const f16 *wfrag, const float *scale, const float *shift, int cout,
                           int act, f16 *out, f16 *out_pool, int n_cu, hipStream_t s, float pool_q_inv = 0.f, float pool_q_zero = 0.f,
-                          const f16 *w2frag = nullptr, float *part2 = nullptr);
+                          const f16 *w2frag = nullptr, float *part2 = nullptr,
+                          const int *tile_list = nullptr, bool *list_taken = nullptr);
 hipError_t conv_c3_q8_launch(const f16 *in, int H, int W, const int8_t *wq, const float *scale, const float *shift, float q_inv,
                              float q_zoff, int act, f16 *out, int n_cu, hipStream_t s);
 struct QLastArgs {
@@ -95,7 +96,7 @@
     int in_first, skip_first;
     int out_chained;
     int in_chained;
-    int th;
+    int th, tw;
     int list_off;
 };
 struct HgNeedParams {
diff --git a/hdr-realtime-video-pipeline_amd/csrc/le_hg_misc.hip b/hdr-realtime-video-pipeline_amd/csrc/le_hg_misc.hip
--- a/hdr-realtime-video-pipeline_amd/csrc/le_hg_misc.hip
+++ b/hdr-realtime-video-pipeline_amd/csrc/le_hg_misc.hip
@@ -6,6 +6,7 @@
 constexpr int C3_HH = C3_TH + 2, C3_HW = C3_TW + 2;
 constexpr int C3_PW = C3_HW + 2;
 constexpr int C3_NP = (C3_HH * C3_HW + 255) / 256;
+constexpr int C3_LIST_N = 512;
 
 __device__ __forceinline__ f16x8 c3_frag(const f16x4 *s_px, int row, int ky, int l31, int lh)
 {
@@ -46,7 +47,7 @@
                                                       const float *__restrict__ scale, const float *__restrict__ shift,
                                                       int act, f16 *__restrict__ out, f16 *__restrict__ out_pool, float pool_q_inv,
                                                       float pool_q_zero, const f16 *__restrict__ w2frag = nullptr,
-                                                      float *__restrict__ part2 = nullptr)
+                                                      float *__restrict__ part2 = nullptr, const int *__restrict__ tile_list = nullptr)
 {
     static_assert(!DOT || COUT == 64, "the fused conv10 half belongs to HG.conv1");
     constexpr int MT = COUT / 32;
@@ -60,6 +61,9 @@
     if (tid < COUT) { s_ss[tid] = scale[tid]; s_ss[COUT + tid] = shift[tid]; }
     __shared__ __attribute__((aligned(16))) f16x8 s_w2[DOT ? 4 * 64 : 1];
     if constexpr (DOT) s_w2[tid] = reinterpret_cast<const f16x8 *>(w2frag)[tid];
+    const int *const lst = DOT ? tile_list : nullptr;
+    const int nrun = lst ? lst[0] : ntiles;
+    __shared__ int s_list[DOT ? C3_LIST_N : 1];
     f16x8 wf[MT][3];
 #pragma unroll
     for (int i = 0; i < MT; ++i)
@@ -71,19 +75,32 @@
     auto fetch = [&](int t) { c3_fetch(pre, in, H, W, (t / tiles_x) * C3_TH, (t % tiles_x) * C3_TW, tid); };
     const float aslope = act_slope(act);
     int t = blockIdx.x;
-    if (t < ntiles) fetch(t);
+    [[maybe_unused]] int tile = t, tile1 = t + (int)gridDim.x, tile2 = 0, k = 0;
+    if constexpr (DOT) {
+        if (lst) {
+            const int mine = t < nrun ? (nrun - t + (int)gridDim.x - 1) / (int)gridDim.x : 0;
+            for (int j = tid; j < mine; j += 256) s_list[j] = lst[1 + t + j * (int)gridDim.x];
+            if (t < nrun) tile = lst[1 + t];
+            if (t + (int)gridDim.x < nrun) tile1 = lst[1 + t + (int)gridDim.x];
+        }
+    }
+    if (t < nrun) fetch(tile);
     int pbuf = 0;
     if constexpr (DOT) {
-        if (t < ntiles) c3_stage(pre, s_px_all, tid);
-        if (t + (int)gridDim.x < ntiles) fetch(t + gridDim.x);
-    }
-    for (; t < ntiles; t += gridDim.x) {
-    const int ox0 = (t % tiles_x) * C3_TW, oy0 = (t / tiles_x) * C3_TH;
+        if (t < nrun) c3_stage(pre, s_px_all, tid);
+        if (t + (int)gridDim.x < nrun) fetch(tile1);
+    }
+    for (; t < nrun; t += gridDim.x) {
+    const int cur = DOT ? tile : t;
+    const int ox0 = (cur % tiles_x) * C3_TW, oy0 = (cur / tiles_x) * C3_TH;
     if constexpr (DOT) {
         __syncthreads();
         s_px = s_px_all + pbuf * (C3_HH * C3_PW);
-        if (t + (int)gridDim.x < ntiles) c3_stage(pre, s_px_all + (pbuf ^ 1) * (C3_HH * C3_PW), tid);
-        if (t + 2 * (int)gridDim.x < ntiles) fetch(t + 2 * gridDim.x);
+        if (t + (int)gridDim.x < nrun) c3_stage(pre, s_px_all + (pbuf ^ 1) * (C3_HH * C3_PW), tid);
+        if (t + 2 * (int)gridDim.x < nrun) {
+            tile2 = lst ? __builtin_amdgcn_readfirstlane(s_list[k + 2]) : t + 2 * (int)gridDim.x;
+            fetch(tile2);
+        }
         pbuf ^= 1;
     } else {
         __syncthreads();
@@ -195,6 +212,7 @@
                 }
             }
         }
+        ++k; tile = tile1; tile1 = tile2;
         continue;
     }
     __syncthreads();
@@ -522,8 +540,9 @@
 
 hipError_t conv_c3_launch(const f16 *in, int H, int W, const f16 *wfrag, const float *scale, const float *shift, int cout,
                           int act, f16 *out, f16 *out_pool, int n_cu, hipStream_t s, float pool_q_inv, float pool_q_zero,
-                          const f16 *w2frag, float *part2)
-{
+                          const f16 *w2frag, float *part2, const int *tile_list, bool *list_taken)
+{
+    if (list_taken) *list_taken = false;
     if ((w2frag != nullptr) != (part2 != nullptr) || (part2 && (cout != 64 || out || !out_pool))) return hipErrorInvalidValue;
     const int ntiles = ((W + C3_TW - 1) / C3_TW) * ((H + C3_TH - 1) / C3_TH);
     static int occ[3] = {0, 0, 0};
@@ -536,15 +555,17 @@
         per_cu = (e == hipSuccess && nb >= 1) ? nb : 2;
     }
     const dim3 grid(ntiles < per_cu * n_cu ? ntiles : per_cu * n_cu);
+    if (tile_list && (!part2 || (ntiles + (int)grid.x - 1) / (int)grid.x > C3_LIST_N)) tile_list = nullptr;
+    if (list_taken) *list_taken = tile_list != nullptr;
     if (cout == 32)
         hipLaunchKernelGGL(conv_c3_kernel<32>, grid, dim3(256), 0, s, in, H, W, wfrag, scale, shift, act, out, out_pool, pool_q_inv, pool_q_zero,
-                           (const f16 *)nullptr, (float *)nullptr);
+                           (const f16 *)nullptr, (float *)nullptr, (const int *)nullptr);
     else if (cout == 64 && part2)
         hipLaunchKernelGGL((conv_c3_kernel<64, true>), grid, dim3(256), 0, s, in, H, W, wfrag, scale, shift, act, out, out_pool, pool_q_inv, pool_q_zero,
-                           w2frag, part2);
+                           w2frag, part2, tile_list);
     else if (cout == 64)
         hipLaunchKernelGGL(conv_c3_kernel<64>, grid, dim3(256), 0, s, in, H, W, wfrag, scale, shift, act, out, out_pool, pool_q_inv, pool_q_zero,
-                           (const f16 *)nullptr, (float *)nullptr);
+                           (const f16 *)nullptr, (float *)nullptr, (const int *)nullptr);
     else
         return hipErrorInvalidValue;
     return hipGetLastError();
diff --git a/hdr-realtime-video-pipeline_amd/hdrtv_mi355x/lib.py b/hdr-realtime-video-pipeline_amd/hdrtv_mi355x/lib.py
--- a/hdr-realtime-video-pipeline_amd/hdrtv_mi355x/lib.py
+++ b/hdr-realtime-video-pipeline_amd/hdrtv_mi355x/lib.py
@@ -53,6 +53,7 @@
     ("hdrtv_profile_enable", _I, [_VP, _I]),
     ("hdrtv_profile_get", _I, [_VP, _I, C.POINTER(C.c_char_p), C.POINTER(C.c_char_p), C.POINTER(C.c_float),
                                C.POINTER(C.c_double), C.POINTER(C.c_double)]),
+    ("hdrtv_profile_tiles", _I, [_VP, _I, C.POINTER(_I), C.POINTER(_I)]),
     ("hdrtv_set_variant", _I, [_VP, C.c_char_p, _I]),
     ("hdrtv_get_variant", _I, [_VP, C.c_char_p, C.POINTER(_I)]),
     ("hdrtv_last_error", C.c_char_p, [_VP]),
diff --git a/hdr-realtime-video-pipeline_amd/hdrtv_mi355x/processor.py b/hdr-realtime-video-pipeline_amd/hdrtv_mi355x/processor.py
--- a/hdr-realtime-video-pipeline_amd/hdrtv_mi355x/processor.py
+++ b/hdr-realtime-video-pipeline_amd/hdrtv_mi355x/processor.py
@@ -618,6 +618,16 @@
             out.append((layer.value.decode(), kern.value.decode(), ms.value, macs.value, nbytes.value))
         return out
 
+    def profile_tiles(self):
+        n = self._lib.hdrtv_profile_get(self._ctx, -1, None, None, None, None, None)
+        out = []
+        for i in range(max(n, 0)):
+            layer, kern, done, total = C.c_char_p(), C.c_char_p(), C.c_int(), C.c_int()
+            self._chk(self._lib.hdrtv_profile_get(self._ctx, i, C.byref(layer), C.byref(kern), None, None, None), "hdrtv_profile_get")
+            self._chk(self._lib.hdrtv_profile_tiles(self._ctx, i, C.byref(done), C.byref(total)), "hdrtv_profile_tiles")
+            out.append((layer.value.decode(), kern.value.decode(), done.value, total.value))
+        return out
+
     def execution_summary(self, profile=None):
         return summarize_profile(profile if profile is not None else self.profile_read())
 
diff --git a/include/hdrtv_mi355x.h b/include/hdrtv_mi355x.h
--- a/include/hdrtv_mi355x.h
+++ b/include/hdrtv_mi355x.h
@@ -103,6 +103,7 @@
 int hdrtv_profile_enable(hdrtv_ctx *ctx, int on);
 int hdrtv_profile_get(hdrtv_ctx *ctx, int i, const char **layer, const char **kernel, float *ms, double *macs,
                       double *bytes);
+int hdrtv_profile_tiles(hdrtv_ctx *ctx, int i, int *executed, int *total);
 
 int hdrtv_set_variant(hdrtv_ctx *ctx, const char *name, int value);
 int hdrtv_get_variant(hdrtv_ctx *ctx, const char *name, int *value);
```
